# i2Nav-WHU/IC-GVINS

Measured on NVIDIA H100. Metric: frames/sec (KLT+BA) 1280x560 300-feat 10-KF window, higher is better.
Workload: dtype u8/int32 fixed point + f32 (KLT), f64 (BA)

## Files before the change

ic_gvins_b200/csrc/ba.cu:

```cuda
#include <cooperative_groups.h>
#include <math.h>
#include <string.h>

#include "ba_dev.cuh"
#include "geom_core.cuh"

namespace icg {
using namespace bam;
namespace cg = cooperative_groups;

constexpr int BA_CHOL_NB = 8;

__device__ __forceinline__ double *lin_Mp(const BaCaps &C, const BaDev &D, int b, int w) { return D.Mp[b] + (size_t) w * C.K * (C.K - 1) * 210; }
__device__ __forceinline__ double *lin_AW(const BaCaps &C, const BaDev &D, int b, int w) { return D.AW[b] + (size_t) w * C.LP * C.NCA; }
__device__ __forceinline__ double *lin_costf(const BaCaps &C, const BaDev &D, int b, int w) { return D.costf[b] + (size_t) w * C.F; }
__device__ __forceinline__ double *lin_hl(const BaCaps &C, const BaDev &D, int b, int w) { return D.hl[b] + (size_t) w * C.L; }
__device__ __forceinline__ double *lin_gl(const BaCaps &C, const BaDev &D, int b, int w) { return D.gl[b] + (size_t) w * C.L; }
__device__ __forceinline__ double *lin_Hc(const BaCaps &C, const BaDev &D, int b, int w) { return D.Hc[b] + (size_t) w * C.NS * C.NS; }
__device__ __forceinline__ double *lin_gc(const BaCaps &C, const BaDev &D, int b, int w) { return D.gc[b] + (size_t) w * C.NS; }

__device__ __forceinline__ int col_pose(int k) { return 6 * k; }
__device__ __forceinline__ int col_ext(int K) { return 6 * K; }
__device__ __forceinline__ int col_td(int K) { return 6 * K + 6; }
__device__ __forceinline__ int col_mix(int K, int k) { return 6 * K + 7 + 9 * k; }

__device__ __forceinline__ double block_sum(double v, double *s_red);
__device__ __forceinline__ double block_max(double v, double *s_red);
}
#include "ba_lm.cuh"
namespace icg {

__device__ __forceinline__ int jc_off(int a) { return a < 18 ? (a / 6) * 12 + (a % 6) : 36 + 2 * (a - 18); }
__device__ __forceinline__ int jc_row1(int a) { return a < 18 ? 6 : 1; }
__device__ __forceinline__ int tri20(int la, int lb) {
    return la * 20 - la * (la - 1) / 2 + (lb - la);
}
__device__ __forceinline__ void dmma884(double &c0, double &c1, double a, double b) {
    asm volatile("mma.sync.aligned.m8n8k4.row.col.f64.f64.f64.f64 {%0,%1}, {%2}, {%3}, {%0,%1};" : "+d"(c0), "+d"(c1) : "d"(a), "d"(b));
}
__global__ void __launch_bounds__(128, 4) ba_lin_vis(BaCaps C, BaDev D, int at_cand) {
    extern __shared__ double lv_sm[];
    __shared__ int s_ord[128], s_gbeg[BA_MAX_NODES], s_gend[BA_MAX_NODES], s_last, s_p0, s_np;
    double (*s_rec)[LV_LD] = (double (*)[LV_LD]) lv_sm;
    double (*s_frame)[NODE_FRAME_LD] = (double (*)[NODE_FRAME_LD]) (lv_sm + 128 * LV_LD);
    const int w = blockIdx.y;
    const LmState &st = D.st[w];
    if (st.done || !(at_cand ? st.step_valid : st.need_lin)) return;
    const int b = at_cand ? 1 - st.lin_buf : st.lin_buf;
    const double *pose = at_cand ? D.pose_c : D.pose, *xext = at_cand ? D.ext_c : D.ext, *rho = at_cand ? D.rho_c : D.rho;
    const int *vb = D.vb_lm0 + (size_t) w * C.NVB;
    if ((int) blockIdx.x >= vb[C.NVB - 1]) return;
    const WinDims dm = D.dims[w];
    const int tid = threadIdx.x;
    const int *off = D.lm_off + (size_t) w * (C.L + 1);
    const int pA = vb[blockIdx.x], pB = vb[blockIdx.x + 1];
    const int s0 = off[pA], nslot = off[pB] - s0;
    if (tid <= dm.K) node_frame(tid < dm.K ? pose + ((size_t) w * C.K + tid) * 7 : xext + (size_t) w * 8, s_frame[tid]);
    if (tid < BA_MAX_NODES) s_gbeg[tid] = s_gend[tid] = 0;
    if (tid == 0) s_np = 0;
    __syncthreads();
    if (tid < nslot) {
        const int q = s0 + tid;
        double r[2], Ji[12], Jj[12], Je[12], Jr[2], Jt[2], cost = 0;
        const int4 meta = ((const int4 *) D.f_meta_s)[(size_t) w * C.F + q];
        const int i = meta.y, j = meta.z, f = meta.w;
        if (D.f_active[(size_t) w * C.F + f] != 0) {
            const double *ext = xext + (size_t) w * 8;
            reproj_eval_frames(s_frame[i], s_frame[j], s_frame[dm.K], rho[(size_t) w * C.L + meta.x], ext[7],
                               D.f_const_s + ((size_t) w * C.F + q) * 14, dm.reproj_sinv, true, r, Ji, Jj, Je, Jr, Jt);
            if (dm.ext_const)
                for (int k = 0; k < 12; k++) Je[k] = 0;
            if (dm.td_const) Jt[0] = Jt[1] = 0;
            double sq = r[0] * r[0] + r[1] * r[1], sc = 1.0;
            if (dm.reproj_huber)
                huber(sq, cost, sc);
            else
                cost = 0.5 * sq;
            if (sc != 1.0) {
                for (int k = 0; k < 12; k++) Ji[k] *= sc, Jj[k] *= sc, Je[k] *= sc;
                Jr[0] *= sc, Jr[1] *= sc, Jt[0] *= sc, Jt[1] *= sc, r[0] *= sc, r[1] *= sc;
            }
        } else {
            for (int k = 0; k < 12; k++) Ji[k] = Jj[k] = Je[k] = 0;
            Jr[0] = Jr[1] = Jt[0] = Jt[1] = r[0] = r[1] = 0;
        }
        lin_costf(C, D, b, w)[f] = cost;
        double *sr = s_rec[tid];
#pragma unroll
        for (int k = 0; k < 12; k++) sr[k] = Ji[k], sr[12 + k] = Jj[k], sr[24 + k] = Je[k];
        sr[36] = Jt[0], sr[37] = Jt[1], sr[38] = r[0], sr[39] = r[1];
        sr[40] = Jr[0], sr[41] = Jr[1], sr[42] = (double) j, sr[43] = (double) i;
    }
    __syncthreads();
    const int lane = tid & 31, warp = tid >> 5;
    if (nslot > 0) {
        if (tid < nslot) {
            const int *ord = D.vis_ord + (size_t) w * C.F + s0;
            const int v = ord[tid], ob = (int) s_rec[v & 255][42];
            s_ord[tid] = v;
            if (tid == 0 || (int) s_rec[ord[tid - 1] & 255][42] != ob) s_gbeg[ob] = tid;
            if (tid == nslot - 1 || (int) s_rec[ord[tid + 1] & 255][42] != ob) s_gend[ob] = tid + 1;
        }
        __syncthreads();
        const int kk = lane & 3, g = lane >> 2;
        int o[3];
#pragma unroll
        for (int t = 0; t < 3; t++) {
            const int a = 8 * t + g;
            o[t] = a < 20 ? jc_off(a) + (kk & 1) * jc_row1(a) : -1;
        }
        for (int ob = warp; ob < dm.K; ob += 4) {
            const int beg = s_gbeg[ob], end = s_gend[ob];
            if (beg == end) continue;
            double c00[2] = {0, 0}, c01[2] = {0, 0}, c02[2] = {0, 0}, c11[2] = {0, 0}, c12[2] = {0, 0}, c22[2] = {0, 0};
            constexpr int UNR = 2;
            for (int base = beg; base < end; base += 2 * UNR) {
                double x[UNR][3];
#pragma unroll
                for (int u = 0; u < UNR; u++) {
                    const int q = base + 2 * u + (kk >> 1);
                    const bool ok = q < end;
                    const double *rec = s_rec[ok ? s_ord[q] & 255 : 0];
#pragma unroll
                    for (int t = 0; t < 3; t++) x[u][t] = (ok && o[t] >= 0) ? rec[o[t]] : 0.0;
                }
#pragma unroll
                for (int u = 0; u < UNR; u++) {
                    dmma884(c00[0], c00[1], x[u][0], x[u][0]);
                    dmma884(c01[0], c01[1], x[u][0], x[u][1]);
                    dmma884(c02[0], c02[1], x[u][0], x[u][2]);
                    dmma884(c11[0], c11[1], x[u][1], x[u][1]);
                    dmma884(c12[0], c12[1], x[u][1], x[u][2]);
                    dmma884(c22[0], c22[1], x[u][2], x[u][2]);
                }
            }
            double *pp = D.gpart + ((size_t) w * C.GQ + (s_ord[beg] >> 8)) * 210;
            auto put = [&](int ti, int tj, const double *c) {
#pragma unroll
                for (int e = 0; e < 2; e++) {
                    const int la = 8 * ti + g, lb = 8 * tj + 2 * kk + e;
                    if (la <= lb && lb < 20) pp[tri20(la, lb)] = c[e];
                }
            };
            put(0, 0, c00), put(0, 1, c01), put(0, 2, c02), put(1, 1, c11), put(1, 2, c12), put(2, 2, c22);
        }
        __threadfence();
    }
    const int *perm = D.lm_perm + (size_t) w * C.L;
    const int K = dm.K, NCV = 6 * K + 7, NCA = 4 * ((NCV + 1 + 3) / 4);
    const int grp = tid >> 3, sl = tid & 7;
    int o0[3], o1[3];
#pragma unroll
    for (int t = 0; t < 3; t++) {
        const int c = sl + 8 * t;
        o0[t] = c < 19 ? jc_off(c) : 38, o1[t] = c < 19 ? o0[t] + jc_row1(c) : 39;
    }
    for (int pl = pA + grp; pl < pB; pl += 16) {
        const int l = perm[pl], f0 = off[pl] - s0, nf = off[pl + 1] - off[pl];
        double *row = lin_AW(C, D, b, w) + (size_t) l * C.NCA;
        for (int c = sl; c < NCA; c += 8) row[c] = 0.0;
        __syncwarp(0xffu << (tid & 24));
        double acc[3] = {0, 0, 0};
        for (int q = 0; q < nf; q++) {
            const double *rec = s_rec[f0 + q];
            const double r0 = rec[40], r1 = rec[41];
            const int ob = (int) rec[42];
#pragma unroll
            for (int t = 0; t < 3; t++) {
                const int c = sl + 8 * t;
                if (c == 20) {
                    acc[t] += r0 * r0 + r1 * r1;
                } else if (c < 20) {
                    const double v = rec[o0[t]] * r0 + rec[o1[t]] * r1;
                    if (c >= 6 && c < 12)
                        row[col_pose(ob) + c - 6] = v;
                    else
                        acc[t] += v;
                }
            }
        }
        const int ref = nf > 0 ? (int) s_rec[f0][43] : 0;
#pragma unroll
        for (int t = 0; t < 3; t++) {
            const int c = sl + 8 * t;
            if (nf > 0) {
                if (c < 6) row[col_pose(ref) + c] = acc[t];
                else if (c >= 12 && c < 18) row[col_ext(K) + c - 12] = acc[t];
                else if (c == 18) row[col_td(K)] = acc[t];
            }
            if (c == 19) {
                row[NCV] = acc[t];
                lin_gl(C, D, b, w)[l] = acc[t];
            } else if (c == 20) {
                lin_hl(C, D, b, w)[l] = acc[t];
                if (st.first) D.scale_l[(size_t) w * C.L + l] = 1.0 / (1.0 + sqrt(acc[t]));
            }
        }
    }
    if (nslot == 0) return;
    const int rn = (int) s_rec[0][43];
    __syncthreads();
    if (tid == 0) s_last = atomicAdd(D.vis_cnt + (size_t) w * C.K + rn, 1) == D.ref_nrun[(size_t) w * C.K + rn] - 1;
    __syncthreads();
    if (!s_last) return;
    __threadfence();
    if (tid == 0) D.vis_cnt[(size_t) w * C.K + rn] = 0;
    const int PM = C.K * (C.K - 1), P = D.npairs[w];
    const int *pro = D.pair_ro + (size_t) w * PM, *poff = D.part_off + (size_t) w * (PM + 1);
    for (int p = tid; p < P; p += 128)
        if ((pro[p] >> 8) == rn) {
            atomicAdd(&s_np, 1);
            if (p == 0 || (pro[p - 1] >> 8) != rn) s_p0 = p;
        }
    __syncthreads();
    const double *part = D.gpart + (size_t) w * C.GQ * 210;
    double *Mp = lin_Mp(C, D, b, w);
    for (int p = s_p0 + warp; p < s_p0 + s_np; p += 4) {
        const int k0 = poff[p], k1 = poff[p + 1];
        double acc[7];
#pragma unroll
        for (int j = 0; j < 7; j++) acc[j] = lane + 32 * j < 210 ? __ldcg(part + (size_t) k0 * 210 + lane + 32 * j) : 0.0;
        for (int k = k0 + 1; k < k1; k++) {
            double v[7];
#pragma unroll
            for (int j = 0; j < 7; j++) v[j] = lane + 32 * j < 210 ? __ldcg(part + (size_t) k * 210 + lane + 32 * j) : 0.0;
#pragma unroll
            for (int j = 0; j < 7; j++) acc[j] += v[j];
        }
#pragma unroll
        for (int j = 0; j < 7; j++)
            if (lane + 32 * j < 210) Mp[(size_t) p * 210 + lane + 32 * j] = acc[j];
    }
}


__device__ __forceinline__ void gram2_slots(const BaCaps &C, const BaDev &D, int w, int K, short *s_slot) {
    const int PM = C.K * (C.K - 1), P = D.npairs[w];
    const int *pro = D.pair_ro + (size_t) w * PM;
    for (int e = threadIdx.x; e < K * K; e += blockDim.x) s_slot[e] = -1;
    __syncthreads();
    for (int p = threadIdx.x; p < P; p += blockDim.x) s_slot[(pro[p] >> 8) * K + (pro[p] & 255)] = (short) p;
    __syncthreads();
}
__device__ __forceinline__ double gram2_entry(const BaCaps &C, const BaDev &D, int buf, int w, int K, const short *s_slot, int A, int B) {
    const int P = D.npairs[w];
    const double *Mp = lin_Mp(C, D, buf, w);
    const int bA = A < 6 * K ? A / 6 : K, bB = B < 6 * K ? B / 6 : K;
    const int a = A - 6 * bA, b = B - 6 * bB;
    const int ga = 12 + a, gb = 12 + b;
    double sum = 0;
    if (bA == K) {
        const int idx = tri20(ga, gb);
        double s4[4] = {0, 0, 0, 0};
        int p = 0;
        for (; p + 16 <= P; p += 16) {
            double v[16];
#pragma unroll
            for (int u = 0; u < 16; u++) v[u] = Mp[(size_t) (p + u) * 210 + idx];
#pragma unroll
            for (int u = 0; u < 16; u++) s4[u & 3] += v[u];
        }
        for (; p < P; p++) s4[p & 3] += Mp[(size_t) p * 210 + idx];
        sum = (s4[0] + s4[1]) + (s4[2] + s4[3]);
    } else if (bB == K || bB == bA) {
        const int i1 = tri20(a, bB == K ? gb : b), i2 = tri20(6 + a, bB == K ? gb : 6 + b);
        for (int o0 = 0; o0 < K; o0 += 8) {
            double v1[8], v2[8];
#pragma unroll
            for (int u = 0; u < 8; u++) {
                const int o = o0 + u;
                const int p1 = o < K ? s_slot[bA * K + o] : -1, p2 = o < K ? s_slot[o * K + bA] : -1;
                v1[u] = p1 >= 0 ? Mp[(size_t) p1 * 210 + i1] : 0.0;
                v2[u] = p2 >= 0 ? Mp[(size_t) p2 * 210 + i2] : 0.0;
            }
#pragma unroll
            for (int u = 0; u < 8; u++) sum += v1[u], sum += v2[u];
        }
    } else {
        const int p1 = s_slot[bA * K + bB], p2 = s_slot[bB * K + bA];
        if (p1 >= 0) sum += Mp[(size_t) p1 * 210 + tri20(a, 6 + b)];
        if (p2 >= 0) sum += Mp[(size_t) p2 * 210 + tri20(b, 6 + a)];
    }
    return sum;
}

__device__ __forceinline__ double *x_inbox(const BaDev &D, int peer, int w, int from);
__device__ __forceinline__ int tri_idx(int A, int B, int ncv);

__device__ __forceinline__ void schur_store(const BaCaps &C, const BaDev &D, int buf, int w, int K, const short *s_slot, int A, int B, double cw) {
    const int NCV = 6 * K + 7;
    if (A == NCV) return;
    const size_t e = (size_t) w * C.NS * C.NS + (size_t) B * C.NS + A;
    const double hc = !D.S.split && B < NCV ? lin_Hc(C, D, buf, w)[(size_t) B * C.NS + A] : 0.0;
    const double cj = gram2_entry(C, D, buf, w, K, s_slot, A, B);
    if (D.S.split) {
        double *P = x_inbox(D, w % D.world, w, D.rank);
        const int TRI = NCV * (NCV + 1) / 2;
        if (B < NCV) {
            P[tri_idx(A, B, NCV)] = cj - cw;
            if (A == B) P[TRI + A] = cj;
        } else {
            P[TRI + NCV + A] = cj;
            P[TRI + 2 * NCV + A] = cw;
        }
    } else {
        double *V = D.visv + (size_t) w * 3 * C.NCV;
        if (B < NCV) {
            D.Hs[e] = hc + (cj - cw);
            if (A == B) V[A] = cj;
        } else {
            V[NCV + A] = cj, V[2 * NCV + A] = cw;
        }
    }
}

__device__ __forceinline__ void schur_scalars(const BaCaps &C, const BaDev &D, int w, const WinDims &dm, double *s_red) {
    const int tid = threadIdx.x;
    double c = 0, q = 0, gm = 0;
    const double *costf = lin_costf(C, D, 0, w), *gl = lin_gl(C, D, 0, w);
    for (int f = tid; f < dm.F; f += 256) c += costf[f];
    for (int l = tid; l < dm.L; l += 256) {
        const double r = D.rho[(size_t) w * C.L + l];
        q += r * r;
        gm = fmax(gm, fabs(gl[l]));
    }
    c = block_sum(c, s_red);
    q = block_sum(q, s_red);
    gm = block_max(gm, s_red);
    if (tid != 0) return;
    const int NCV = 6 * dm.K + 7, TRI = NCV * (NCV + 1) / 2;
    double *P = x_inbox(D, w % D.world, w, D.rank);
    P[TRI + 3 * NCV] = c, P[TRI + 3 * NCV + 1] = q, P[TRI + 3 * NCV + 2] = gm;
}

__global__ void __cluster_dims__(BA_SPLIT_W, 1, 1) __launch_bounds__(256) ba_schur_dmma(BaCaps C, BaDev D, int ld) {
    extern __shared__ double sA[];
    __shared__ short s_slot[32 * 32];
    __shared__ double s_red[40];
    cg::cluster_group cluster = cg::this_cluster();
    const int w = blockIdx.y, split = blockIdx.x;
    const LmState &st = D.st[w];
    if (st.done) return;
    const WinDims dm = D.dims[w];
    const int NCV = 6 * dm.K + 7, NCA = 4 * ((NCV + 1 + 3) / 4);
    const int T2 = (NCA + 15) / 16, nsuper = T2 * (T2 + 1) / 2;
    const int tid = threadIdx.x, lane = tid & 31, warp = tid >> 5, g = lane >> 2, kk = lane & 3;
    double *sphi = sA + (size_t) SCHUR_RCH * ld;
    const int b = st.lin_buf;
    const double *A = lin_AW(C, D, b, w), *hl = lin_hl(C, D, b, w);
    const double radius = st.radius;
    const int nsteps = (dm.L + 3) / 4;
    const int r_beg = 4 * (int) ((long long) nsteps * split / BA_SPLIT_W), r_end = min(dm.L, 4 * (int) ((long long) nsteps * (split + 1) / BA_SPLIT_W));
    const int npass = (nsuper + SCHUR_PASS - 1) / SCHUR_PASS;
    gram2_slots(C, D, w, dm.K, s_slot);
    for (int pass = 0; pass < npass; pass++) {
        if (pass > 0) cluster.barrier_wait();
        int si[2], sj[2];
        bool on[2];
#pragma unroll
        for (int h2 = 0; h2 < 2; h2++) {
            const int su = (2 * pass + h2) * 8 + warp;
            on[h2] = su < nsuper;
            int a = 0, e = on[h2] ? su : 0;
            while (e >= T2 - a) e -= T2 - a, a++;
            si[h2] = a, sj[h2] = a + e;
        }
        double acc[2][4][2];
#pragma unroll
        for (int h2 = 0; h2 < 2; h2++)
#pragma unroll
            for (int q = 0; q < 4; q++) acc[h2][q][0] = acc[h2][q][1] = 0;
        for (int r0 = r_beg; r0 < r_end; r0 += SCHUR_RCH) {
            const int nr = min(SCHUR_RCH, r_end - r0), nr4 = (nr + 3) & ~3;
            __syncthreads();
            for (int rb = warp; rb < nr4; rb += 8 * 4) {
                double v[4][3];
#pragma unroll
                for (int u = 0; u < 4; u++) {
                    const int rr = rb + 8 * u;
#pragma unroll
                    for (int cchunk = 0; cchunk < 3; cchunk++) {
                        const int c = lane + 32 * cchunk;
                        v[u][cchunk] = (rr < nr && c < NCA) ? A[(size_t) (r0 + rr) * C.NCA + c] : 0.0;
                    }
                }
#pragma unroll
                for (int u = 0; u < 4; u++) {
                    const int rr = rb + 8 * u;
#pragma unroll
                    for (int cchunk = 0; cchunk < 3; cchunk++) {
                        const int c = lane + 32 * cchunk;
                        if (rr < nr4 && c < ld) sA[(size_t) rr * ld + c] = v[u][cchunk];
                    }
                }
                for (int c = lane + 96; c < ld; c += 32)
                    for (int u = 0; u < 4; u++) {
                        const int rr = rb + 8 * u;
                        if (rr < nr4) sA[(size_t) rr * ld + c] = (rr < nr && c < NCA) ? A[(size_t) (r0 + rr) * C.NCA + c] : 0.0;
                    }
            }
            for (int rr = tid; rr < nr4; rr += 256) {
                double ph = 0;
                if (rr < nr) {
                    const int l = r0 + rr;
                    const double sl = D.scale_l[(size_t) w * C.L + l], hs = sl * sl * hl[l];
                    ph = sl * sl / (hs + lm_d2(hs, radius));
                }
                sphi[rr] = ph;
            }
            __syncthreads();
            for (int ks = 0; ks < nr4 / 4; ks++) {
                const double *row = sA + (size_t) (4 * ks + kk) * ld;
                const double ph = sphi[4 * ks + kk];
#pragma unroll
                for (int h2 = 0; h2 < 2; h2++) {
                    if (!on[h2]) continue;
                    const double xb0 = row[16 * sj[h2] + g], xb1 = row[16 * sj[h2] + 8 + g];
                    const double a0 = row[16 * si[h2] + g] * ph, a1 = row[16 * si[h2] + 8 + g] * ph;
                    dmma884(acc[h2][0][0], acc[h2][0][1], a0, xb0);
                    dmma884(acc[h2][1][0], acc[h2][1][1], a0, xb1);
                    dmma884(acc[h2][2][0], acc[h2][2][1], a1, xb0);
                    dmma884(acc[h2][3][0], acc[h2][3][1], a1, xb1);
                }
            }
        }
        __syncthreads();
#pragma unroll
        for (int h2 = 0; h2 < 2; h2++) {
            if (!on[h2]) continue;
#pragma unroll
            for (int q = 0; q < 4; q++)
#pragma unroll
                for (int e = 0; e < 2; e++) sA[(h2 * 8 + warp) * 256 + 64 * q + 32 * e + lane] = acc[h2][q][e];
        }
        cluster.sync();
        const int nslot = min(SCHUR_PASS, nsuper - SCHUR_PASS * pass);
        double cw[SCHUR_PASS / BA_SPLIT_W];
#pragma unroll
        for (int j = 0; j < SCHUR_PASS / BA_SPLIT_W; j++) {
            const int sl = split + BA_SPLIT_W * j;
            double p[BA_SPLIT_W];
#pragma unroll
            for (int k = 0; k < BA_SPLIT_W; k++) p[k] = sl < nslot ? cluster.map_shared_rank(sA, k)[sl * 256 + tid] : 0.0;
            cw[j] = 0;
#pragma unroll
            for (int k = 0; k < BA_SPLIT_W; k++) cw[j] += p[k];
        }
        cluster.barrier_arrive();
        const int q = tid >> 6, r_in = 8 * (q >> 1) + ((tid & 31) >> 2), c_in = 8 * (q & 1) + 2 * (tid & 3) + ((tid >> 5) & 1);
#pragma unroll
        for (int j = 0; j < SCHUR_PASS / BA_SPLIT_W; j++) {
            const int sl = split + BA_SPLIT_W * j;
            if (sl >= nslot) break;
            int a = 0, e = SCHUR_PASS * pass + sl;
            while (e >= T2 - a) e -= T2 - a, a++;
            const int r = 16 * a + r_in, cc = 16 * (a + e) + c_in;
            if (r <= cc && cc <= NCV) schur_store(C, D, b, w, dm.K, s_slot, r, cc, cw[j]);
        }
    }
    if (split == 0 && D.S.split) schur_scalars(C, D, w, dm, s_red);
    cluster.barrier_wait();
}

constexpr double IMU_GB_STD = 7200 / 3600.0 * 3.14159265358979323846 / 180.0;
constexpr double IMU_AB_STD = 2.0e4 * 1.0e-5;

__device__ void imu_factor_warp(const double *blob, const double *U, const double *pose0, const double *mix0, const double *pose1,
                                const double *mix1, bool want_j, double *rw, double *Jw, int lane) {
    __shared__ ImuMid s_mid[16];
    double *raw_r = rw + 15;
    const int wslot = (threadIdx.x >> 5) & 15;
    if (want_j)
        for (int e = lane; e < 450; e += 32) Jw[e] = 0;
    __syncwarp();
    if (lane == 0) {
        ImuMid M;
        imu_residual_raw(blob, pose0, mix0, pose1, mix1, raw_r, M);
        if (want_j) imu_jacobian_raw(blob, M, Jw);
        s_mid[wslot] = M;
    }
    __syncwarp();
    if (want_j && lane < 30) {
        for (int i = 0; i < 15; i++) {
            double s = 0;
            for (int k = i; k < 15; k++) s += U[i * 15 + k] * Jw[k * 30 + lane];
            Jw[i * 30 + lane] = s;
        }
    }
    if (lane < 15) {
        double s = 0;
        for (int k = lane; k < 15; k++) s += U[lane * 15 + k] * raw_r[k];
        rw[lane] = s;
    }
    __syncwarp();
}

__device__ void marg_dx(const BaCaps &C, const BaDev &D, int w, const WinDims &dm, const double *pose, const double *mix, const double *ext, double *dx,
                        int *colmap, int tid, int nthreads) {
    const int *type = D.marg_type + (size_t) w * BA_MARG_MAXB, *node = D.marg_node + (size_t) w * BA_MARG_MAXB;
    const double *x0 = D.marg_x0 + (size_t) w * BA_MARG_MAXB * 9;
    if (tid == 0) {
        int col = 0, xo = 0;
        for (int b = 0; b < dm.marg_nb; b++) {
            int t = type[b], nd = node[b];
            if (t == 0 || t == 2) {
                const double *x = t == 0 ? pose + nd * 7 : ext;
                const double *xl = x0 + xo;
                Q dq = qmul(qinv(pose_q(xl)), pose_q(x));
                V3 a = 2.0 * qv(dq);
                if (dq.w < 0) a = -a;
                for (int k = 0; k < 3; k++) dx[col + k] = x[k] - xl[k];
                dx[col + 3] = a.x, dx[col + 4] = a.y, dx[col + 5] = a.z;
                int base = t == 0 ? col_pose(nd) : col_ext(dm.K);
                for (int k = 0; k < 6; k++) colmap[col + k] = (t == 2 && dm.ext_const) ? -1 : base + k;
                col += 6, xo += 7;
            } else if (t == 1) {
                for (int k = 0; k < 9; k++) dx[col + k] = mix[nd * 9 + k] - x0[xo + k], colmap[col + k] = col_mix(dm.K, nd) + k;
                col += 9, xo += 9;
            } else {
                dx[col] = ext[7] - x0[xo];
                colmap[col] = dm.td_const ? -1 : col_td(dm.K);
                col += 1, xo += 1;
            }
        }
    }
}

__device__ __forceinline__ void red_add(double *p, double v) { asm volatile("red.global.add.f64 [%0], %1;" ::"l"(p), "d"(v) : "memory"); }

__device__ double cam_factors(const BaCaps &C, const BaDev &D, int w, const WinDims &dm, const double *pose, const double *mix, const double *ext,
                              bool lin, int b, double *smem) {
    const int tid = threadIdx.x, lane = tid & 31, warp = tid >> 5, nwarps = blockDim.x >> 5;
    const int K = dm.K, N = 15 * K + 7;
    double *Hc = lin_Hc(C, D, b, w), *gc = lin_gc(C, D, b, w);
    double *s_imu = smem;
    double *s_gnss = s_imu + (size_t) C.K * 480;
    double *s_misc = s_gnss + (size_t) C.G * 24;
    double *s_pp = s_misc, *s_mp = s_misc + 48, *s_dx = s_mp + 16, *s_y = s_dx + C.R, *s_cost = s_y + C.R;
    int *s_colmap = (int *) (s_cost + 8);
    __shared__ double s_total;
#ifdef ICG_BA_PHASE_CLOCKS
    unsigned long long cclk = D.clk ? clock64() : 0ull;
#define CAM_CLK(k)                                                 \
    if (D.clk && lin && w == 0 && tid == 0) {                      \
        const unsigned long long t_ = clock64();                   \
        atomicAdd(&D.clk[16 + (k)], t_ - cclk), atomicAdd(&D.clk[24 + (k)], 1ull); \
        cclk = t_;                                                 \
    }
#else
#define CAM_CLK(k)
#endif
    for (int k = warp; k < dm.n_imu; k += nwarps)
        imu_factor_warp(D.imu_blob + ((size_t) w * C.K + k) * ICG_IMU_BLOB_DOUBLES, D.imu_U + ((size_t) w * C.K + k) * 225, pose + k * 7, mix + k * 9,
                        pose + (k + 1) * 7, mix + (k + 1) * 9, lin, s_imu + (size_t) k * 480, s_imu + (size_t) k * 480 + 30, lane);
    if (tid < dm.n_gnss) {
        const int nd = D.gnss_node[(size_t) w * C.G + tid];
        double *o = s_gnss + tid * 24;
        gnss_eval(pose + nd * 7, D.gnss_blh + ((size_t) w * C.G + tid) * 3, D.gnss_std + ((size_t) w * C.G + tid) * 3, D.lever + (size_t) w * 3, lin, o, o + 3);
        double sq = o[0] * o[0] + o[1] * o[1] + o[2] * o[2], cost, sc = 1.0;
        if (dm.gnss_huber)
            huber(sq, cost, sc);
        else
            cost = 0.5 * sq;
        if (sc != 1.0) {
            for (int e = 0; e < 3; e++) o[e] *= sc;
            if (lin)
                for (int e = 0; e < 18; e++) o[3 + e] *= sc;
        }
        o[21] = cost;
    }
    if (tid == 64 && dm.has_pose_prior) pose_prior_eval(pose, D.pose_prior + (size_t) w * 7, D.pose_prior_sinfo + (size_t) w * 6, lin, s_pp, s_pp + 6);
    if (tid == 96 && dm.has_mix_prior)
        for (int k = 0; k < 9; k++) s_mp[k] = (mix[k] - D.mix_prior[(size_t) w * 9 + k]) / D.mix_prior_std[(size_t) w * 9 + k];
    if (dm.marg_r > 0) marg_dx(C, D, w, dm, pose, mix, ext, s_dx, s_colmap, tid, blockDim.x);
    __syncthreads();
    CAM_CLK(0)
    const double *H0 = D.marg_H0 + (size_t) w * C.R * C.R, *b0 = D.marg_b0 + (size_t) w * C.R;
    if (dm.marg_r > 0) {
        for (int i = tid; i < dm.marg_r; i += blockDim.x) {
            double s = 0;
            for (int k = 0; k < dm.marg_r; k++) s += H0[(size_t) i * dm.marg_r + k] * s_dx[k];
            s_y[i] = s;
        }
    }
    __syncthreads();
    if (tid == 0) {
        double c = 0;
        for (int k = 0; k < dm.n_imu; k++) {
            const double *r = s_imu + (size_t) k * 480;
            double sq = 0;
            for (int e = 0; e < 15; e++) sq += r[e] * r[e];
            c += 0.5 * sq;
        }
        for (int g = 0; g < dm.n_gnss; g++) c += s_gnss[g * 24 + 21];
        if (dm.has_imu_error) {
            const double *m = mix + dm.n_imu * 9;
            double sq = 0;
            for (int e = 0; e < 3; e++) sq += (m[3 + e] / IMU_GB_STD) * (m[3 + e] / IMU_GB_STD) + (m[6 + e] / IMU_AB_STD) * (m[6 + e] / IMU_AB_STD);
            c += 0.5 * sq;
        }
        if (dm.has_pose_prior) {
            double sq = 0;
            for (int e = 0; e < 6; e++) sq += s_pp[e] * s_pp[e];
            c += 0.5 * sq;
        }
        if (dm.has_mix_prior) {
            double sq = 0;
            for (int e = 0; e < 9; e++) sq += s_mp[e] * s_mp[e];
            c += 0.5 * sq;
        }
        if (dm.marg_r > 0) {
            double q = D.marg_c0[w];
            for (int i = 0; i < dm.marg_r; i++) q += (2.0 * b0[i] + s_y[i]) * s_dx[i];
            c += 0.5 * q;
        }
        s_total = c;
    }
    if (!lin) {
        __syncthreads();
        return s_total;
    }
    CAM_CLK(1)
    for (int e = tid; e < N * C.NS; e += blockDim.x) Hc[e] = 0;
    for (int e = tid; e < N; e += blockDim.x) gc[e] = 0;
    __syncthreads();
    CAM_CLK(2)
    if (dm.marg_r > 0) {
        const int r = dm.marg_r;
        for (int e = tid; e < r * r; e += blockDim.x) {
            int i = e / r, j = e - i * r;
            int ci = s_colmap[i], cj = s_colmap[j];
            if (ci >= 0 && cj >= 0) Hc[(size_t) ci * C.NS + cj] = H0[e];
        }
        for (int i = tid; i < r; i += blockDim.x)
            if (s_colmap[i] >= 0) gc[s_colmap[i]] = b0[i] + s_y[i];
    }
    __syncthreads();
    CAM_CLK(3)
    for (int parity = 0; parity < 2; parity++) {
        const int nf = (dm.n_imu - parity + 1) / 2;
        for (int e = tid; e < nf * 930; e += blockDim.x) {
            const int k = parity + 2 * (e / 930), q = e % 930;
            const double *rw = s_imu + (size_t) k * 480, *Jw = rw + 30;
            auto gcol = [&](int c) { return c < 6 ? col_pose(k) + c : c < 15 ? col_mix(K, k) + c - 6 : c < 21 ? col_pose(k + 1) + c - 15 : col_mix(K, k + 1) + c - 21; };
            if (q < 900) {
                int a = q / 30, b = q - a * 30;
                double s = 0;
                for (int m = 0; m < 15; m++) s += Jw[m * 30 + a] * Jw[m * 30 + b];
                red_add(&Hc[(size_t) gcol(a) * C.NS + gcol(b)], s);
            } else {
                int a = q - 900;
                double s = 0;
                for (int m = 0; m < 15; m++) s += Jw[m * 30 + a] * rw[m];
                red_add(&gc[gcol(a)], s);
            }
        }
        __syncthreads();
    }
    CAM_CLK(4)
    for (int e = tid; e < K * 42; e += blockDim.x) {
        const int k = e / 42, q = e % 42;
        double s = 0;
        if (q < 36) {
            const int a = q / 6, b = q % 6;
            for (int g = 0; g < dm.n_gnss; g++)
                if (D.gnss_node[(size_t) w * C.G + g] == k) {
                    const double *J = s_gnss + g * 24 + 3;
                    s += J[a] * J[b] + J[6 + a] * J[6 + b] + J[12 + a] * J[12 + b];
                }
            if (k == 0 && dm.has_pose_prior)
                for (int m = 0; m < 6; m++) s += s_pp[6 + m * 6 + a] * s_pp[6 + m * 6 + b];
            red_add(&Hc[(size_t) (col_pose(k) + a) * C.NS + col_pose(k) + b], s);
        } else {
            const int a = q - 36;
            for (int g = 0; g < dm.n_gnss; g++)
                if (D.gnss_node[(size_t) w * C.G + g] == k) {
                    const double *o = s_gnss + g * 24;
                    s += o[3 + a] * o[0] + o[9 + a] * o[1] + o[15 + a] * o[2];
                }
            if (k == 0 && dm.has_pose_prior)
                for (int m = 0; m < 6; m++) s += s_pp[6 + m * 6 + a] * s_pp[m];
            red_add(&gc[col_pose(k) + a], s);
        }
    }
    if (tid < 9) {
        if (dm.has_imu_error && tid >= 3) {
            const int k = dm.n_imu;
            const double sd = tid < 6 ? IMU_GB_STD : IMU_AB_STD;
            Hc[(size_t) (col_mix(K, k) + tid) * C.NS + col_mix(K, k) + tid] += 1.0 / (sd * sd);
            gc[col_mix(K, k) + tid] += mix[k * 9 + tid] / (sd * sd);
        }
    }
    __syncthreads();
    if (tid < 9 && dm.has_mix_prior) {
        const double sd = D.mix_prior_std[(size_t) w * 9 + tid];
        Hc[(size_t) (col_mix(K, 0) + tid) * C.NS + col_mix(K, 0) + tid] += 1.0 / (sd * sd);
        gc[col_mix(K, 0) + tid] += s_mp[tid] / sd;
    }
    __syncthreads();
    CAM_CLK(5)
#undef CAM_CLK
    return s_total;
}

__global__ void __launch_bounds__(CAM_THREADS) ba_lin_cam(BaCaps C, BaDev D, int at_cand) {
    extern __shared__ double smem[];
    const int w = blockIdx.x;
    LmState &st = D.st[w];
    if (st.done || !(at_cand ? st.step_valid : st.need_lin)) return;
    if (D.S.split && (w % D.world) != D.rank) return;
    const WinDims dm = D.dims[w];
    const int b = at_cand ? 1 - st.lin_buf : st.lin_buf;
    const double *pose = at_cand ? D.pose_c : D.pose, *mix = at_cand ? D.mix_c : D.mix, *ext = at_cand ? D.ext_c : D.ext;
    double c = cam_factors(C, D, w, dm, pose + (size_t) w * C.K * 7, mix + (size_t) w * C.K * 9, ext + (size_t) w * 8, true, b, smem);
    if (threadIdx.x == 0) st.cost_cam[b] = c;
}


__device__ __forceinline__ double block_sum(double v, double *s_red) {
    const int tid = threadIdx.x, lane = tid & 31, warp = tid >> 5;
    for (int o = 16; o > 0; o >>= 1) v += __shfl_down_sync(0xffffffffu, v, o);
    __syncthreads();
    if (lane == 0) s_red[warp] = v;
    __syncthreads();
    double t = 0;
    if (tid == 0) {
        for (int k = 0; k < (int) (blockDim.x >> 5); k++) t += s_red[k];
        s_red[32] = t;
    }
    __syncthreads();
    return s_red[32];
}
__device__ __forceinline__ double block_max(double v, double *s_red) {
    const int tid = threadIdx.x, lane = tid & 31, warp = tid >> 5;
    for (int o = 16; o > 0; o >>= 1) v = fmax(v, __shfl_down_sync(0xffffffffu, v, o));
    __syncthreads();
    if (lane == 0) s_red[warp] = v;
    __syncthreads();
    if (tid == 0) {
        double t = 0;
        for (int k = 0; k < (int) (blockDim.x >> 5); k++) t = fmax(t, s_red[k]);
        s_red[32] = t;
    }
    __syncthreads();
    return s_red[32];
}

__global__ void __launch_bounds__(SOLVE_THREADS, 2) ba_solve(BaCaps C, BaDev D) {
    extern __shared__ double sm[];
    const int w = blockIdx.x, tid = threadIdx.x;
    LmState &st = D.st[w];
    if (st.done) return;
#ifdef ICG_BA_PHASE_CLOCKS
    unsigned long long clk_prev = D.clk ? clock64() : 0ull;
#define SOLVE_CLK(k)                                              \
    if (D.clk && w == 0 && tid == 0) {                            \
        const unsigned long long t_ = clock64();                  \
        atomicAdd(&D.clk[k], t_ - clk_prev), atomicAdd(&D.clk[8 + (k)], 1ull); \
        clk_prev = t_;                                            \
    }
#define SOLVE_CLK_NOW() (D.clk ? clock64() : 0ull)
#define SOLVE_CLK_ADD(k, t0)                                      \
    if (D.clk && w == 0 && tid == 0) atomicAdd(&D.clk[k], clock64() - (t0)), atomicAdd(&D.clk[8 + (k)], 1ull);
#else
#define SOLVE_CLK(k)
#define SOLVE_CLK_NOW() 0ull
#define SOLVE_CLK_ADD(k, t0)
#endif
    const WinDims dm = D.dims[w];
    const int K = dm.K, L = dm.L, NCV = 6 * K + 7, N = 15 * K + 7;
    const int f_first = st.first, f_fresh = st.fresh_lin, f_last = st.last_success, f_iter = st.iter;
    const double f_gmax_old = st.gmax;
    (void) f_gmax_old;
    double *s_red = sm;
    double *s_scale = s_red + 40;
    double *s_g = s_scale + C.NS;
    double *s_rhs = s_g + C.NS;
    double *s_d2 = s_rhs + C.NS;
    double *s_diag = s_d2 + C.NS;
    double *S = s_diag + C.NS;
    const int b = st.lin_buf;
    const double *Hc = lin_Hc(C, D, b, w), *gcam = lin_gc(C, D, b, w), *Hs = D.Hs + (size_t) w * C.NS * C.NS;
    const double *V = D.visv + (size_t) (3 * C.NCV) * w;
    if (tid == 0 && st.need_lin) st.need_lin = 0;
    double *scale_c = D.scale_c + (size_t) w * C.NS;
    const double *hl = lin_hl(C, D, b, w), *gl = lin_gl(C, D, b, w), *scale_l = D.scale_l + (size_t) w * C.L;

    for (int a = tid; a < N; a += SOLVE_THREADS) {
        double g = gcam[a];
        if (a < NCV) g += V[NCV + a];
        s_g[a] = g;
        if (f_first) {
            double h = Hc[(size_t) a * C.NS + a] + (a < NCV ? V[a] : 0.0);
            scale_c[a] = 1.0 / (1.0 + sqrt(h));
        }
    }
    __syncthreads();
    for (int a = tid; a < N; a += SOLVE_THREADS) s_scale[a] = scale_c[a];
    double gmax_now = st.gmax;
    if (f_fresh) {
        double cs = 0, gq = 0;
        const double *costf = lin_costf(C, D, b, w);
        for (int f = tid; f < dm.F; f += SOLVE_THREADS) cs += costf[f];
        for (int l = tid; l < L; l += SOLVE_THREADS) gq = fmax(gq, fabs(gl[l]));
        const double c = block_sum(cs, s_red), gml = block_max(gq, s_red);
        double gm = 0;
        for (int a = tid; a < N; a += SOLVE_THREADS) gm = fmax(gm, fabs(s_g[a]));
        gm = fmax(block_max(gm, s_red), gml);
        gmax_now = gm;
        if (tid == 0) {
            st.x_cost = c + st.cost_cam[b];
            st.gmax = gm;
            if (f_first) st.initial_cost = st.x_cost;
            st.fresh_lin = 0;
        }
        __syncthreads();
    }
    if (f_first) {
        __syncthreads();
        if (tid == 0) st.first = 0;
    }
    {
        const int term = lm_term(f_iter, st.max_iter, f_last, gmax_now, st.radius);
        if (term) {
            __syncthreads();
            if (tid == 0) st.done = term, st.step_valid = 0;
            return;
        }
    }
    __syncthreads();
    if (tid == 0) st.iter++;
    const double radius = st.radius;
    SOLVE_CLK(0)

    constexpr bool async_fill = true;
    if (async_fill) {
        for (int i = tid >> 5; i < N; i += SOLVE_THREADS / 32) {
            const double *src = (i < NCV ? Hs : Hc) + (size_t) i * C.NS;
            const unsigned dst = (unsigned) __cvta_generic_to_shared(S + i * (i + 1) / 2);
            for (int j = tid & 31; j <= i; j += 32)
                asm volatile("cp.async.ca.shared.global [%0], [%1], 8;" ::"r"(dst + 8u * j), "l"(src + j) : "memory");
        }
        asm volatile("cp.async.commit_group;" ::: "memory");
    }
    for (int a = tid; a < N; a += SOLVE_THREADS) {
        double h = Hc[(size_t) a * C.NS + a] + (a < NCV ? V[a] : 0.0);
        double hs = s_scale[a] * s_scale[a] * h;
        s_d2[a] = lm_d2(hs, radius);
        double gw = a < NCV ? V[2 * NCV + a] : 0.0;
        s_rhs[a] = -s_scale[a] * (s_g[a] - gw);
    }
    if (async_fill) asm volatile("cp.async.wait_all;" ::: "memory");
    __syncthreads();
    if (async_fill) {
        for (int i = tid >> 5; i < N; i += SOLVE_THREADS / 32) {
            double *row = S + i * (i + 1) / 2;
            const double si = s_scale[i];
            for (int j = tid & 31; j <= i; j += 32) {
                double v = si * s_scale[j] * row[j];
                if (i == j) v += s_d2[i];
                row[j] = v;
            }
        }
    } else {
        for (int i = tid >> 5; i < N; i += SOLVE_THREADS / 32) {
            constexpr int MAXQ = 16;
            double hv[MAXQ];
            const int nq = i / 32 + 1;
#pragma unroll
            for (int q = 0; q < MAXQ; q++) {
                const int j = (tid & 31) + 32 * q;
                hv[q] = 0;
                if (q < nq && j <= i) hv[q] = (i < NCV ? Hs : Hc)[(size_t) i * C.NS + j];
            }
#pragma unroll
            for (int q = 0; q < MAXQ; q++) {
                const int j = (tid & 31) + 32 * q;
                if (q < nq && j <= i) {
                    double v = s_scale[i] * s_scale[j] * hv[q];
                    if (i == j) v += s_d2[i];
                    S[i * (i + 1) / 2 + j] = v;
                }
            }
        }
    }
    for (int a = tid; a < N; a += SOLVE_THREADS) S[N * (N + 1) / 2 + a] = s_rhs[a];
    __syncthreads();
    SOLVE_CLK(1)
    __shared__ int s_fail;
    if (tid == 0) s_fail = 0;
    __syncthreads();
    const int NR = N + 1;
    for (int J0 = 0; J0 < N; J0 += BA_CHOL_NB) {
        const int nb = min(BA_CHOL_NB, N - J0);
        const int lane = tid & 31, warp = tid >> 5, g = lane >> 2, kk = lane & 3;
        const int ntile = (NR - J0 + 7) / 8;
        const unsigned long long pc0 = SOLVE_CLK_NOW();
        (void) pc0;
        const int cb = J0 + g;
        const double *rb = S + (cb < NR ? cb * (cb + 1) / 2 : 0);
        const bool okb = cb < NR;
        if (warp == 0) {
            if (J0 > 0) {
                const double *ra = rb;
                double acc[8] = {0, 0, 0, 0, 0, 0, 0, 0};
                int k0 = 0;
                for (; k0 + 16 <= J0; k0 += 16) {
                    const double x0 = okb ? ra[k0 + kk] : 0.0, x1 = okb ? ra[k0 + 4 + kk] : 0.0, x2 = okb ? ra[k0 + 8 + kk] : 0.0, x3 = okb ? ra[k0 + 12 + kk] : 0.0;
                    dmma884(acc[0], acc[1], x0, x0);
                    dmma884(acc[2], acc[3], x1, x1);
                    dmma884(acc[4], acc[5], x2, x2);
                    dmma884(acc[6], acc[7], x3, x3);
                }
                for (; k0 + 8 <= J0; k0 += 8) {
                    const double x0 = okb ? ra[k0 + kk] : 0.0, x1 = okb ? ra[k0 + 4 + kk] : 0.0;
                    dmma884(acc[0], acc[1], x0, x0);
                    dmma884(acc[2], acc[3], x1, x1);
                }
                const double c0 = (acc[0] + acc[2]) + (acc[4] + acc[6]), c1 = (acc[1] + acc[3]) + (acc[5] + acc[7]);
                const int i = J0 + g;
                if (i < NR) {
                    const int ca = J0 + 2 * kk;
                    if (ca < J0 + nb && ca <= i) S[i * (i + 1) / 2 + ca] -= c0;
                    if (ca + 1 < J0 + nb && ca + 1 <= i) S[i * (i + 1) / 2 + ca + 1] -= c1;
                }
                __syncwarp();
            }
            double Ld[BA_CHOL_NB][BA_CHOL_NB], dinv[BA_CHOL_NB];
            bool bad = false;
#pragma unroll
            for (int a = 0; a < BA_CHOL_NB; a++)
#pragma unroll
                for (int b = 0; b < BA_CHOL_NB; b++) Ld[a][b] = (a < nb && b <= a) ? S[(J0 + a) * (J0 + a + 1) / 2 + J0 + b] : (a == b ? 1.0 : 0.0);
#pragma unroll
            for (int j = 0; j < BA_CHOL_NB; j++) {
                double d = Ld[j][j];
#pragma unroll
                for (int k = 0; k < j; k++) d -= Ld[j][k] * Ld[j][k];
                if (!(d > 0.0) || !isfinite(d)) bad = true;
                const double di = rsqrt(d);
                dinv[j] = di;
                Ld[j][j] = d * di;
#pragma unroll
                for (int a = j + 1; a < BA_CHOL_NB; a++) {
                    double sum = Ld[a][j];
#pragma unroll
                    for (int k = 0; k < j; k++) sum -= Ld[a][k] * Ld[j][k];
                    Ld[a][j] = sum * di;
                }
            }
            __syncwarp();
            if (bad && lane == 0) s_fail = 1;
#pragma unroll
            for (int a2 = 0; a2 < BA_CHOL_NB; a2++) {
                double *ri = S + (J0 + a2) * (J0 + a2 + 1) / 2 + J0;
#pragma unroll
                for (int b = 0; b <= a2; b++)
                    if (lane == ((a2 * 8 + b) & 31) && a2 < nb) ri[b] = Ld[a2][b];
                if (lane == 8 + a2 && a2 < nb) s_diag[J0 + a2] = dinv[a2];
            }
            SOLVE_CLK_ADD(6, pc0)
        } else if (J0 > 0 && warp != 4) {
            constexpr int TPW = 4, NWARP = 6;
            const int wslot = warp < 4 ? warp - 1 : warp - 2;
            for (int t0 = 1 + wslot; t0 < ntile; t0 += TPW * NWARP) {
                const double *ra[TPW];
                bool oka[TPW];
                double acc[TPW][4];
#pragma unroll
                for (int u = 0; u < TPW; u++) {
                    const int ia = J0 + 8 * (t0 + u * NWARP) + g;
                    oka[u] = (t0 + u * NWARP) < ntile && ia < NR;
                    ra[u] = S + (oka[u] ? ia * (ia + 1) / 2 : 0);
                    acc[u][0] = acc[u][1] = acc[u][2] = acc[u][3] = 0;
                }
                for (int k0 = 0; k0 + 8 <= J0; k0 += 8) {
                    const double b0 = okb ? rb[k0 + kk] : 0.0, b1 = okb ? rb[k0 + 4 + kk] : 0.0;
                    double a0[TPW], a1[TPW];
#pragma unroll
                    for (int u = 0; u < TPW; u++) a0[u] = oka[u] ? ra[u][k0 + kk] : 0.0, a1[u] = oka[u] ? ra[u][k0 + 4 + kk] : 0.0;
#pragma unroll
                    for (int u = 0; u < TPW; u++) {
                        dmma884(acc[u][0], acc[u][1], a0[u], b0);
                        dmma884(acc[u][2], acc[u][3], a1[u], b1);
                    }
                }
#pragma unroll
                for (int u = 0; u < TPW; u++) {
                    const double c0 = acc[u][0] + acc[u][2], c1 = acc[u][1] + acc[u][3];
                    const int i = J0 + 8 * (t0 + u * NWARP) + g;
                    if (oka[u]) {
                        const int ca = J0 + 2 * kk;
                        if (ca < J0 + nb && ca <= i) S[i * (i + 1) / 2 + ca] -= c0;
                        if (ca + 1 < J0 + nb && ca + 1 <= i) S[i * (i + 1) / 2 + ca + 1] -= c1;
                    }
                }
            }
        }
        __syncthreads();
        const unsigned long long pc1 = SOLVE_CLK_NOW();
        (void) pc1;
        if (s_fail) break;
        for (int i = J0 + nb + tid; i < NR; i += SOLVE_THREADS) {
            double *ri = S + i * (i + 1) / 2 + J0;
            double x[BA_CHOL_NB];
#pragma unroll
            for (int c = 0; c < BA_CHOL_NB; c++) x[c] = c < nb ? ri[c] : 0.0;
#pragma unroll
            for (int c = 0; c < BA_CHOL_NB; c++) {
                if (c < nb) {
                    const double *lc = S + (J0 + c) * (J0 + c + 1) / 2 + J0;
                    double sum = x[c];
#pragma unroll
                    for (int k = 0; k < c; k++) sum -= x[k] * lc[k];
                    x[c] = sum * s_diag[J0 + c];
                }
            }
#pragma unroll
            for (int c = 0; c < BA_CHOL_NB; c++)
                if (c < nb) ri[c] = x[c];
        }
        __syncthreads();
        SOLVE_CLK_ADD(7, pc1)
    }
    __syncthreads();
    bool valid = !s_fail;
    SOLVE_CLK(2)
    if (valid) {
        double *y = S + N * (N + 1) / 2;
        const int lane = tid & 31;
        for (int J0 = ((N - 1) / BA_CHOL_NB) * BA_CHOL_NB; J0 >= 0; J0 -= BA_CHOL_NB) {
            const int nb = min(BA_CHOL_NB, N - J0);
            if (tid < 32) {
                double x[BA_CHOL_NB];
#pragma unroll
                for (int c = BA_CHOL_NB - 1; c >= 0; c--) {
                    x[c] = 0.0;
                    if (c < nb) {
                        double sum = y[J0 + c];
#pragma unroll
                        for (int k = BA_CHOL_NB - 1; k > c; k--)
                            if (k < nb) sum -= S[(J0 + k) * (J0 + k + 1) / 2 + J0 + c] * x[k];
                        x[c] = sum * s_diag[J0 + c];
                    }
                }
#pragma unroll
                for (int c = 0; c < BA_CHOL_NB; c++)
                    if (c == lane && c < nb) s_rhs[J0 + c] = x[c];
            }
            __syncthreads();
            for (int i = tid; i < J0; i += SOLVE_THREADS) {
                double acc = y[i];
#pragma unroll
                for (int c = BA_CHOL_NB - 1; c >= 0; c--)
                    if (c < nb) acc -= S[(J0 + c) * (J0 + c + 1) / 2 + i] * s_rhs[J0 + c];
                y[i] = acc;
            }
            __syncthreads();
        }
    }
    __syncthreads();
    SOLVE_CLK(3)
    double *step_l = D.step_l + (size_t) w * C.L;
    const double *AW = lin_AW(C, D, b, w);
    double part = 0;
    bool finite = true;
    double *R2 = D.red2 + (size_t) w * 4;
    if (!valid) {
        if (tid == 0) {
            st.chol_ok = 0, st.step_valid = 0;
            R2[0] = 0, R2[1] = 0, R2[2] = 1;
        }
        return;
    }
    for (int a = tid; a < N; a += SOLVE_THREADS) {
        double sp = s_rhs[a];
        finite = finite && isfinite(sp);
        part += -0.5 * sp * (s_scale[a] * s_g[a]) + 0.5 * s_d2[a] * sp * sp;
    }
    double *s_sx = s_diag;
    __syncthreads();
    for (int a = tid; a < NCV; a += SOLVE_THREADS) s_sx[a] = s_scale[a] * s_rhs[a];
    __syncthreads();
    {
        const int lane = tid & 31, warp = tid >> 5;
        constexpr int LB = 8;
        const int lu = ((lane >> 4) & 1) * 4 + ((lane >> 3) & 1) * 2 + ((lane >> 2) & 1);
        for (int l0 = LB * warp; l0 < L; l0 += LB * (SOLVE_THREADS / 32)) {
            const int l = l0 + lu;
            const bool lok = l < L;
            const double sl = lok ? scale_l[l] : 0.0, hh = lok ? hl[l] : 0.0, gg = lok ? gl[l] : 0.0;
            double d[LB];
#pragma unroll
            for (int u = 0; u < LB; u++) d[u] = 0;
            for (int c = lane; c < NCV; c += 32) {
                const double sx = s_sx[c];
#pragma unroll
                for (int u = 0; u < LB; u++) d[u] += (l0 + u < L ? AW[(size_t) (l0 + u) * C.NCA + c] : 0.0) * sx;
            }
            const double hs = sl * sl * hh, d2 = lm_d2(hs, radius), den = hs + d2, sg = sl * gg;
            double e4[4], e2[2];
            {
                const bool hi = lane & 16;
#pragma unroll
                for (int u = 0; u < 4; u++) {
                    const double keep = hi ? d[u + 4] : d[u], send = hi ? d[u] : d[u + 4];
                    e4[u] = keep + __shfl_xor_sync(0xffffffffu, send, 16);
                }
            }
            {
                const bool hi = lane & 8;
#pragma unroll
                for (int u = 0; u < 2; u++) {
                    const double keep = hi ? e4[u + 2] : e4[u], send = hi ? e4[u] : e4[u + 2];
                    e2[u] = keep + __shfl_xor_sync(0xffffffffu, send, 8);
                }
            }
            double mine;
            {
                const bool hi = lane & 4;
                const double keep = hi ? e2[1] : e2[0], send = hi ? e2[0] : e2[1];
                mine = keep + __shfl_xor_sync(0xffffffffu, send, 4);
            }
            mine += __shfl_xor_sync(0xffffffffu, mine, 2);
            mine += __shfl_xor_sync(0xffffffffu, mine, 1);
            if ((lane & 3) == 0 && lok) {
                double sp = (-sg - sl * mine) / den;
                finite = finite && isfinite(sp);
                step_l[l] = sp;
                part += -0.5 * sp * sg + 0.5 * d2 * sp * sp;
            }
        }
    }
    __syncthreads();
    SOLVE_CLK(4)
    const double mcc = block_sum(part, s_red);
    const double nfin = block_sum(finite ? 0.0 : 1.0, s_red);
    const double *pose = D.pose + (size_t) w * C.K * 7, *mix = D.mix + (size_t) w * C.K * 9, *ext = D.ext + (size_t) w * 8, *rho = D.rho + (size_t) w * C.L;
    double *pose_c = D.pose_c + (size_t) w * C.K * 7, *mix_c = D.mix_c + (size_t) w * C.K * 9, *ext_c = D.ext_c + (size_t) w * 8, *rho_c = D.rho_c + (size_t) w * C.L;
    double sn = 0;
    for (int k = tid; k <= K; k += SOLVE_THREADS) {
        const bool is_ext = (k == K);
        const double *x = is_ext ? ext : pose + k * 7;
        double *xc = is_ext ? ext_c : pose_c + k * 7;
        if (is_ext && dm.ext_const) {
            for (int e = 0; e < 7; e++) xc[e] = x[e];
        } else {
            const int c0 = is_ext ? col_ext(K) : col_pose(k);
            double d[6];
            for (int e = 0; e < 6; e++) d[e] = s_rhs[c0 + e] * s_scale[c0 + e];
            pose_plus(x, d, xc);
            for (int e = 0; e < 7; e++) sn += (x[e] - xc[e]) * (x[e] - xc[e]);
        }
    }
    for (int e = tid; e < K * 9; e += SOLVE_THREADS) {
        int k = e / 9, q = e - 9 * k, c = col_mix(K, k) + q;
        double v = mix[e] + s_rhs[c] * s_scale[c];
        mix_c[e] = v;
        sn += (mix[e] - v) * (mix[e] - v);
    }
    if (tid == 0) {
        if (dm.td_const) {
            ext_c[7] = ext[7];
        } else {
            double v = ext[7] + s_rhs[col_td(K)] * s_scale[col_td(K)];
            ext_c[7] = v;
            sn += (ext[7] - v) * (ext[7] - v);
        }
    }
    for (int l = tid; l < L; l += SOLVE_THREADS) {
        double v = rho[l] + step_l[l] * scale_l[l];
        rho_c[l] = v;
        sn += (rho[l] - v) * (rho[l] - v);
    }
    sn = block_sum(sn, s_red);
    if (tid == 0) {
// ... 258 lines not shown
```

ic_gvins_b200/csrc/ba_dev.cuh:

```cuda
#pragma once
#include "ba_math.cuh"
#include "ba_slide.cuh"
#include "common.cuh"

namespace icg {

constexpr int BA_SPLIT_W = 4;
constexpr int BA_MARG_MAXB = 72;
constexpr int BA_MAX_NODES = 32;

struct BaCaps {
    int NW, K, L, F, G, R;
    int NCV, N, NS, NCA, RJ, LP, NVB;
    int GQ;
};

struct WinDims {
    int K, L, F, n_imu, n_gnss, marg_r, marg_nb;
    int ext_const, td_const, reproj_huber, gnss_huber, has_imu_error, has_pose_prior, has_mix_prior;
    double reproj_sinv;
};

struct LmState {
    double radius, decrease_factor, x_cost, x_norm, cand_cost, model_cost_change, step_norm, gmax, initial_cost;
    double cost_cam[2];
    int iter, n_success, n_invalid, done, need_lin, last_success, first, step_valid, fresh_lin, max_iter, chol_ok;
    int lin_buf;
};

struct ShardDev {
    int split;
    int PK, BS, RV;
    double *peer[8];
    size_t off_inbox, off_bcast, off_scal, off_flagA, off_flagB, off_flagC;
    size_t off_flagX, off_post, off_exp;
    double *redv;
    int *err;
    double *slm;
    int *slm_cnt;
};

struct BaDev {
    ShardDev S;
    WinDims *dims;
    LmState *st;
    double *pose, *mix, *ext, *rho;
    double *pose_c, *mix_c, *ext_c, *rho_c;
    double *pose_0, *mix_0, *ext_0, *rho_0;
    uint8_t *f_active_0;
    double *gnss_std_0;
    uint8_t *f_active;
    int *lm_off;
    int *lm_perm;
    int *vb_lm0;
    int *ref_nrun;
    int *f_meta_s;
    double *f_const_s;
    int *vis_ord;
    int *part_off, *pair_ro, *npairs;
    double *gpart;
    int *vis_cnt;
    double *Mp[2];
    double *AW[2];
    double *costf[2];
    double *hl[2], *gl[2];
    double *Hc[2], *gc[2];
    double *scale_l, *scale_c;
    double *Hs;
    double *visv;
    double *imu_blob, *imu_U;
    int *gnss_node;
    double *gnss_blh, *gnss_std, *lever;
    double *pose_prior, *pose_prior_sinfo, *mix_prior, *mix_prior_std;
    int *marg_type, *marg_node;
    double *marg_x0, *marg_H0, *marg_b0, *marg_c0;
    double *cost_part;
    double *red2;
    int rank, world;
    double *step_c, *step_l;
    double *Sglobal;
    unsigned long long *clk;
};

constexpr int LV_LD = 45;
constexpr size_t LV_SMEM = sizeof(double) * (128 * LV_LD + (BA_MAX_NODES + 1) * bam::NODE_FRAME_LD);
constexpr int SCHUR_RCH = 80;
constexpr int SCHUR_PASS = 16;
constexpr int CAM_THREADS = 320;
constexpr int SOLVE_THREADS = 256;

constexpr int SPLIT_CLUSTER = 4;
constexpr int SPLIT_HDR = 16;
constexpr int SPLIT_SCAL = 8;
constexpr int SPLIT_BS_ROWS = 32;
constexpr int STEP_SLICES = 4;
constexpr int MEXP_ROW = 16;
enum { XF_SUM = 0, XF_EXPORT = 1, XF_DONE = 2 };

__host__ __device__ inline size_t split_S_stride(const BaCaps &C) { return (size_t) (C.N + 1) * (C.N + 2) / 2 + (size_t) C.NS; }

constexpr int DSM_CL = 4;
static_assert(SOLVE_THREADS == 256 && DSM_CL == SPLIT_CLUSTER, "ba_solve_cam_dsm: warp r assembles row r of a tile row; one launch geometry for both forms");
__host__ __device__ constexpr int dsm_ntiles(int NR) { return (NR + 7) / 8; }
__host__ inline size_t dsm_smem_doubles(const BaCaps &C) {
    const int nt = dsm_ntiles(C.N + 1);
    int mx = 0;
    for (int cr = 0; cr < DSM_CL; cr++) {
        int s = 0;
        for (int T = cr; T < nt; T += DSM_CL) s += T;
        mx = s > mx ? s : mx;
    }
    return 40 + 8 * (size_t) nt * 8 + 64 + 8 + 8 * DSM_CL + 8 + 8 + (size_t) nt * 64 * 3 + (size_t) mx * 64;
}

constexpr int MARG_THREADS = 512;
constexpr int MARG_MAP_HDR = 8;

struct MargDev {
    int *map;
    int map_stride;
    double *H0, *b0;
    double *G1, *V1;
    double *G2, *V2;
    double *lam1, *lam2;
    double *Z;
    double *Hp, *bp;
    double *J0, *e0;
    int *flags;
    int n0cap, mcap, rcap;
};

constexpr int MARG_PAIR_MAXN = 160;
constexpr int MARG_CTA_MAXN = 118;
constexpr int MARG_CTA_THREADS = 512;
constexpr int MARG_CLUSTER_MAXN = 320;
constexpr int MARG_CLUSTER_CTAS = 8;
constexpr int MARG_CLUSTER_THREADS = 640;
constexpr int MARG_CLUSTER_SLOT = 3 * (MARG_CLUSTER_MAXN / 2);
__host__ __device__ constexpr int marg_cluster_rows(int n) { return (n + MARG_CLUSTER_CTAS - 1) / MARG_CLUSTER_CTAS; }
__host__ __device__ constexpr size_t marg_cluster_smem(int n) {
    return sizeof(double) * (2 * (size_t) marg_cluster_rows(n) * n + 2 * (size_t) MARG_CLUSTER_SLOT);
}

__global__ void ba_lin_vis(BaCaps C, BaDev D, int at_cand);
__global__ void ba_schur_dmma(BaCaps C, BaDev D, int ld);
__global__ void ba_lin_cam(BaCaps C, BaDev D, int at_cand);
__global__ void ba_solve(BaCaps C, BaDev D);
__global__ void ba_cost_cam(BaCaps C, BaDev D, int nblk_vis);
__global__ void ba_cost(BaCaps C, BaDev D, int nblk_vis);
__global__ void ba_accept(BaCaps C, BaDev D);
__global__ void ba_reset_state(BaDev D, LmState *save, int n, int max_iter);
__global__ void ba_chi2_cull(BaCaps C, BaDev D, int *counters);
__global__ void ba_set_gnss_huber(BaDev D, int n, int v);
__global__ void ba_residual_costs_kernel(BaCaps C, BaDev D, double *reproj_cost, double *gnss_cost);
__global__ void ba_reproj_eval_kernel(const double *in, double *out, int frames);
__global__ void ba_imu_eval_kernel(const double *blob, const double *U, const double *x, double *out);
__global__ void ba_small_factor_eval_kernel(int kind, const double *in, double *out);
__global__ void ba_marg_factor_eval_kernel(const double *in, double *out);
__global__ void ba_lm_ref_fill(const WinDims *dims, const SlideWin *win, const int *map, const double *old, const double *fc, const int *lm_off,
                               const int *lm_perm, double *out, int Lc, int Fc);

__global__ void ba_signal(BaDev D, unsigned long long epoch);
__global__ void ba_reduce(BaCaps C, BaDev D, unsigned long long epoch);
__global__ void ba_solve_cam(BaCaps C, BaDev D, unsigned long long epoch);
__global__ void ba_solve_cam_dsm(BaCaps C, BaDev D, unsigned long long epoch);
__global__ void ba_step_lm(BaCaps C, BaDev D, unsigned long long epoch);
__global__ void ba_exchange(BaCaps C, BaDev D, int n, int nblk_vis, unsigned long long epoch);
__global__ void ba_accept_split(BaCaps C, BaDev D, unsigned long long epoch);
__global__ void ba_xflag(BaDev D, int kind, unsigned long long epoch);
__global__ void ba_xsum(BaCaps C, BaDev D, int *v, int stride, int n, int nv, int op, int par, unsigned long long epoch);
__global__ void ba_marg_export(BaCaps C, BaDev D, const int *sel, const int *sel_off, const uint8_t *fmask, unsigned long long prev);
__global__ void ba_marg_heads(BaCaps C, BaDev D, int n_own, long long *heads, unsigned long long epoch);
__global__ void ba_marg_gather(BaCaps C, BaDev D, const long long *heads, const int *dst_row, double *dst);
__global__ void ba_marg_fill(BaCaps Cm, BaDev Dm, BaCaps C, BaDev D, const double *rows, const int *row0, const int *fidx);

__global__ void marg_prepare(BaDev D, MargDev M, int n, int restore);
__global__ void marg_assemble(BaCaps C, BaDev D, MargDev M);
__global__ void marg_jacobi(MargDev M, int which);
__global__ void marg_jacobi_pair(MargDev M, int which);
__global__ void marg_jacobi_cta(MargDev M, int which);
__global__ void marg_jacobi_cluster(MargDev M, int which);
__global__ void marg_schur(MargDev M);
__global__ void marg_finish(MargDev M);

}
```

ic_gvins_b200/csrc/ba_handle.cu:

```cuda
#include <unistd.h>

#include <string>
#include <thread>

#include "ba_handle.cuh"
#include "preint.cuh"

using namespace icg;

int dmalloc(icg_ba *h, double **p, size_t n) {
    if (cudaMalloc(p, sizeof(double) * n) != cudaSuccess) {
        set_error("icg_ba_create: cudaMalloc of %zu doubles failed", n);
        return ICG_ENOMEM;
    }
    cudaMemsetAsync(*p, 0, sizeof(double) * n, h->stream);
    h->dev_only.push_back(*p);
    return ICG_OK;
}

static int cam_threads(const icg_ba *h) { return h->D.world >= 4 ? CAM_THREADS : 160; }

static const char *PROF_NAMES[16] = {"(gap/other)", "lin_vis", "lin_lm", "lin at candidate", "","schur_dmma (+ epilogue)", "join lin_cam + lin_done",
                                     "signal", "solve", "cost (+cost_cam)", "exchange", "accept", "reduce", "join gram chain", "step_lm", ""};
static void prof_mark(icg_ba *h, int tag) {
    if (!h->prof) return;
    if (h->prof_used == h->prof_ev.size()) {
        cudaEvent_t e;
        cudaEventCreate(&e);
        h->prof_ev.push_back(e);
        h->prof_tag.push_back(0);
    }
    h->prof_tag[h->prof_used] = tag;
    cudaEventRecord(h->prof_ev[h->prof_used++], h->stream);
}
static void prof_collect(icg_ba *h) {
    if (!h->prof) return;
    if (h->prof_used && h->prof_skip > 0) {
        h->prof_skip--;
        h->prof_used = 0;
        return;
    }
    for (size_t i = 1; i < h->prof_used; i++) {
        float ms = 0;
        if (cudaEventElapsedTime(&ms, h->prof_ev[i - 1], h->prof_ev[i]) == cudaSuccess) {
            h->prof_ms[h->prof_tag[i]] += ms;
            h->prof_cnt[h->prof_tag[i]]++;
        }
    }
    h->prof_used = 0;
}
static void prof_print(icg_ba *h) {
    if (!h->prof) return;
    double tot = 0;
    for (int t = 0; t < 16; t++) tot += h->prof_ms[t];
    fprintf(stderr, "[icg_ba profile] handle %p, %d windows: stage totals over all recorded LM sequences (ms, mean us, share)\n", (void *) h, h->cur_windows);
    for (int t = 0; t < 16; t++)
        if (h->prof_cnt[t])
            fprintf(stderr, "  %-28s %9.3f ms  %8.1f us  %5.1f %%\n", PROF_NAMES[t], h->prof_ms[t], 1e3 * h->prof_ms[t] / h->prof_cnt[t], 100.0 * h->prof_ms[t] / tot);
    if (h->D.clk) {
        unsigned long long ck[48];
        if (cudaMemcpy(ck, h->D.clk, sizeof(ck), cudaMemcpyDeviceToHost) == cudaSuccess) {
            static const char *cn[6] = {"factor evaluation", "prior product + cost", "zero H_c", "prior blocks", "IMU J^T J", "GNSS / prior diagonals"};
            fprintf(stderr, "[icg_ba profile] ba_lin_cam phases of window 0 (SM cycles per call, mean):\n");
            for (int k = 0; k < 6; k++)
                if (ck[24 + k]) fprintf(stderr, "  %-28s %9.0f cycles\n", cn[k], (double) ck[16 + k] / (double) ck[24 + k]);
            if (h->D.S.split) {
                static const char *sn_l2[6] = {"per panel: stage B operand", "per panel: warp 0 tile + factor", "per panel: tiles + barrier 1", "per panel: row solve + barrier 2", "whole factorisation", ""};
                static const char *sn_dsm[6] = {"assembly", "per panel: warp 0 tile + factor", "per panel: until block barrier", "per panel: row solve + cl. barrier", "whole factorisation", "backward substitution"};
                const char **sn = h->solve_cam_dsm ? sn_dsm : sn_l2;
                fprintf(stderr, "[icg_ba profile] %s phases of window 0 (SM cycles, mean):\n", h->solve_cam_dsm ? "ba_solve_cam_dsm" : "ba_solve_cam");
                for (int k = 0; k < 6; k++)
                    if (ck[8 + k]) fprintf(stderr, "  %-34s %9.0f cycles\n", sn[k], (double) ck[k] / (double) ck[8 + k]);
                static const char *sn2[5] = {"(unused)", "(unused)", "per panel: warp 0 diagonal-tile update", "per panel: warp 0 loads + 8x8 factorisation", "per panel: warp 0 write-back"};
                for (int k = 0; k < 5 && h->solve_cam_dsm; k++)
                    if (ck[40 + k]) fprintf(stderr, "  %-50s %9.0f cycles\n", sn2[k], (double) ck[32 + k] / (double) ck[40 + k]);
            }
            static const char *nm[8] = {"gradient / cost / tests", "assembly", "Cholesky", "camera back-substitution", "landmark back-substitution", "candidate + reductions",
                                        "  per panel: warp 0 tile+factor", "  per panel: row solve phase"};
            if (!h->D.S.split) fprintf(stderr, "[icg_ba profile] ba_solve phases of window 0 (SM cycles per call, mean):\n");
            for (int k = 0; k < 8 && !h->D.S.split; k++)
                if (ck[8 + k]) fprintf(stderr, "  %-28s %9.0f cycles\n", nm[k], (double) ck[k] / (double) ck[8 + k]);
        }
    }
}

void retire(icg_ba *h, void *d, void *hp) {
    if (h->D.world > 1) {
        if (d) h->retired_d.push_back(d);
        if (hp) h->retired_h.push_back(hp);
        return;
    }
    if (d) cudaFree(d);
    if (hp) cudaFreeHost(hp);
}

static void split_release(icg_ba *h) {
    if (h->stream) cudaStreamSynchronize(h->stream);
    for (void *p : h->retired_d) cudaFree(p);
    for (void *p : h->retired_h) cudaFreeHost(p);
    for (icg_ba *m : h->retired_mx) icg_ba_destroy(m);
    h->retired_d.clear(), h->retired_h.clear(), h->retired_mx.clear();
    for (int r = 0; r < 8; r++)
        if (h->ipc_opened[r]) cudaIpcCloseMemHandle(h->ipc_opened[r]), h->ipc_opened[r] = nullptr;
    if (h->xbuf) cudaFree(h->xbuf), h->xbuf = nullptr;
    if (h->D.S.redv) cudaFree(h->D.S.redv), h->D.S.redv = nullptr;
    if (h->D.S.err) cudaFree(h->D.S.err), h->D.S.err = nullptr;
    if (h->D.S.slm) cudaFree(h->D.S.slm), h->D.S.slm = nullptr;
    if (h->D.S.slm_cnt) cudaFree(h->D.S.slm_cnt), h->D.S.slm_cnt = nullptr;
    if (h->D.Sglobal) cudaFree(h->D.Sglobal), h->D.Sglobal = nullptr;
    h->D.S.split = 0;
}

static int preload_group_kernels() {
    const void *k[] = {(const void *) ba_accept, (const void *) ba_accept_split, (const void *) ba_chi2_cull, (const void *) ba_cost, (const void *) ba_cost_cam,
                       (const void *) ba_exchange, (const void *) ba_lin_cam, (const void *) ba_lin_vis, (const void *) ba_marg_export, (const void *) ba_marg_fill,
                       (const void *) ba_marg_gather, (const void *) ba_marg_heads, (const void *) ba_reduce, (const void *) ba_reset_state,
                       (const void *) ba_schur_dmma, (const void *) ba_set_gnss_huber, (const void *) ba_signal, (const void *) ba_solve, (const void *) ba_solve_cam,
                       (const void *) ba_solve_cam_dsm, (const void *) ba_step_lm, (const void *) ba_xflag, (const void *) ba_xsum, (const void *) marg_assemble,
                       (const void *) marg_finish, (const void *) marg_jacobi, (const void *) marg_jacobi_cluster, (const void *) marg_jacobi_cta,
                       (const void *) marg_jacobi_pair, (const void *) marg_prepare, (const void *) marg_schur};
    cudaFuncAttributes a;
    for (const void *f : k) ICG_CUDA(cudaFuncGetAttributes(&a, f));
    ICG_CUDA(preload_update_cull());
    ICG_CUDA(preload_slide());
    ICG_CUDA(preload_preint_resident());
    return ICG_OK;
}

static int split_setup(icg_ba *h, int rank, int world) {
    if (world < 1 || world > 8 || rank < 0 || rank >= world) {
        set_error("split pipeline: rank %d / world %d out of range (<= 8 GPUs of one box)", rank, world);
        return ICG_EINVAL;
    }
    ICG_CUDA(cudaSetDevice(h->device));
    ICG_CUDA(cudaStreamSynchronize(h->stream));
    split_release(h);
    const BaCaps &C = h->C;
    ShardDev &S = h->D.S;
    const size_t NW = C.NW, G = world;
    const size_t TRI = (size_t) C.NCV * (C.NCV + 1) / 2;
    S.PK = (int) ((TRI + 3 * (size_t) C.NCV + 4 + 3) & ~(size_t) 3);
    S.BS = (SPLIT_HDR + C.NS + 3) & ~3;
    S.RV = (3 * C.NCV + 4 + 3) & ~3;
    const size_t NWo = (NW + G - 1) / G;
    size_t off = 0;
    S.off_inbox = off, off += NWo * G * S.PK;
    S.off_bcast = off, off += NW * S.BS;
    S.off_scal = off, off += NW * G * SPLIT_SCAL;
    S.off_flagA = off, off += 8;
    S.off_flagB = off, off += (NW + 3) & ~(size_t) 3;
    S.off_flagC = off, off += (NW * G + 3) & ~(size_t) 3;
    S.off_flagX = off, off += 3 * 8;
    S.off_post = off, off += 2 * NW * G * SPLIT_SCAL;
    S.off_exp = off;
    if (world > 1) off += 2 * NW + NW * (size_t) C.F * MEXP_ROW;
    h->xbuf_doubles = off;
    h->xs_calls = 0, h->exp_epoch = 0;
    if (world > 1) {
        const int rc = preload_group_kernels();
        if (rc != ICG_OK) return rc;
        if (!h->xs_v.d && h->xs_v.alloc(16) != ICG_OK) {
            set_error("split pipeline: allocation of the exchange word failed");
            return ICG_ENOMEM;
        }
    }
    if (cudaMalloc(&h->xbuf, sizeof(double) * off) != cudaSuccess || cudaMalloc(&S.redv, sizeof(double) * NW * S.RV) != cudaSuccess ||
        cudaMalloc(&S.err, sizeof(int) * 4) != cudaSuccess || cudaMalloc(&S.slm, sizeof(double) * NW * STEP_SLICES * 8) != cudaSuccess ||
        cudaMalloc(&S.slm_cnt, sizeof(int) * NW) != cudaSuccess ||
        cudaMalloc(&h->D.Sglobal, sizeof(double) * NWo * split_S_stride(C)) != cudaSuccess) {
        set_error("split pipeline: allocation of the exchange buffers failed (%zu doubles)", off);
        return ICG_ENOMEM;
    }
    ICG_CUDA(cudaMemset(h->xbuf, 0, sizeof(double) * off));
    ICG_CUDA(cudaMemset(S.redv, 0, sizeof(double) * NW * S.RV));
    ICG_CUDA(cudaMemset(S.err, 0, sizeof(int) * 4));
    ICG_CUDA(cudaMemset(S.slm, 0, sizeof(double) * NW * STEP_SLICES * 8));
    ICG_CUDA(cudaMemset(S.slm_cnt, 0, sizeof(int) * NW));
    for (int r = 0; r < 8; r++) S.peer[r] = nullptr;
    S.peer[rank] = h->xbuf;
    S.split = 1;
    h->D.rank = rank, h->D.world = world;
    h->x_world = world;
    h->epoch = 0;
    {
        const size_t ldbp = ((size_t) (C.N + 15) / 16) * 16 + 8;
        const size_t bs = (size_t) SPLIT_BS_ROWS * (C.NS + 1), base = 8 * ldbp + 64;
        h->smem_solve_cam = sizeof(double) * (40 + 4 * (size_t) C.NS + std::max(bs, base));
    }
    h->smem_step_lm = sizeof(double) * (40 + (size_t) C.NS);
    h->smem_solve_cam_dsm = sizeof(double) * dsm_smem_doubles(C);
    h->solve_cam_dsm = h->smem_solve_cam_dsm <= 227 * 1024 && C.N <= 32 * 11;
    if (h->solve_cam_dsm) ICG_CUDA(raise_dynamic_smem((const void *) ba_solve_cam_dsm, h->smem_solve_cam_dsm));
    ICG_CUDA(raise_dynamic_smem((const void *) ba_solve_cam, (size_t) (h->smem_solve_cam)));
    ICG_CUDA(cudaFuncSetAttribute(ba_solve_cam, cudaFuncAttributeNonPortableClusterSizeAllowed, 0));
    ICG_CUDA(raise_dynamic_smem((const void *) ba_step_lm, (size_t) (h->smem_step_lm)));
    return ICG_OK;
}

static int ba_create_body(icg_ba *h, int max_windows, int max_K, int max_L, int max_F, int max_gnss, int max_marg_r, void *stream) {
    if (stream) {
        h->stream = (cudaStream_t) stream;
    } else {
        ICG_CUDA(cudaStreamCreateWithFlags(&h->stream, cudaStreamNonBlocking));
        h->own_stream = true;
    }
    {
        int prio_lo = 0, prio_hi = 0;
        ICG_CUDA(cudaDeviceGetStreamPriorityRange(&prio_lo, &prio_hi));
        ICG_CUDA(cudaStreamCreateWithPriority(&h->stream_cam, cudaStreamNonBlocking, prio_hi));
    }
    ICG_CUDA(cudaEventCreateWithFlags(&h->ev_fork, cudaEventDisableTiming));
    ICG_CUDA(cudaEventCreateWithFlags(&h->ev_join, cudaEventDisableTiming));
    h->prof = getenv("ICG_BA_PROFILE") != nullptr;
    if (h->prof) {
        double *ck = nullptr;
        if (dmalloc(h, &ck, 48) != ICG_OK) return ICG_ENOMEM;
        h->D.clk = (unsigned long long *) ck;
    }
    if (getenv("ICG_BA_PROFILE_SKIP")) h->prof_skip = atoi(getenv("ICG_BA_PROFILE_SKIP"));
    BaCaps &C = h->C;
    max_L = std::max(1, max_L), max_F = std::max(1, max_F);
    C.NW = max_windows, C.K = max_K, C.L = max_L, C.F = max_F, C.G = std::max(1, max_gnss), C.R = std::max(1, max_marg_r);
    C.NCV = 6 * max_K + 7, C.N = 15 * max_K + 7, C.NS = (C.N + 3) & ~3, C.NCA = 4 * ((C.NCV + 1 + 3) / 4);
    C.RJ = (2 * max_F + 31) & ~31, C.LP = (max_L + 31) & ~31;
    C.NVB = (max_F + 127 - max_K) / (128 - max_K) + max_L / 128 + 4 + max_K;
    C.GQ = std::max(1, std::min(max_F, (C.NVB - 2) * (max_K - 1)));
    h->nblk_vis = (max_F + 255) / 256;
    const size_t NW = max_windows;
#define HD(field, count)                                                       \
    if (h->field.alloc(count) != ICG_OK) {                                     \
        set_error("icg_ba_create: allocation of " #field " failed");           \
        return ICG_ENOMEM;                                                     \
    }
    HD(dims, NW) HD(st, NW) HD(pose, NW * C.K * 7) HD(mix, NW * C.K * 9) HD(ext, NW * 8) HD(rho, NW * C.L)
    HD(imu_blob, NW * C.K * ICG_IMU_BLOB_DOUBLES) HD(imu_U, NW * C.K * 225) HD(gnss_blh, NW * C.G * 3) HD(gnss_std, NW * C.G * 3) HD(lever, NW * 3)
    HD(pose_prior, NW * 7) HD(pose_prior_sinfo, NW * 6) HD(mix_prior, NW * 9) HD(mix_prior_std, NW * 9) HD(marg_x0, NW * BA_MARG_MAXB * 9)
    HD(marg_H0, NW * C.R * C.R) HD(marg_b0, NW * C.R) HD(marg_c0, NW)
    HD(lm_off, NW * (C.L + 1)) HD(lm_perm, NW * C.L) HD(lm_fidx, NW * C.F) HD(gnss_node, NW * C.G) HD(marg_type, NW * BA_MARG_MAXB) HD(marg_node, NW * BA_MARG_MAXB) HD(f_active, NW * C.F)
    HD(scratch, 1024) HD(st_save, NW) HD(cull_counters, 2 * NW) HD(f_meta_s, NW * C.F * 4) HD(vb_lm0, NW * C.NVB) HD(ref_nrun, NW * C.K) HD(f_const_s, NW * C.F * 14)
    HD(part_off, NW * ((size_t) C.K * (C.K - 1) + 1)) HD(pair_ro, NW * (size_t) C.K * (C.K - 1)) HD(vis_ord, NW * C.F) HD(npairs, NW)
#undef HD
    ICG_CUDA(cudaMemsetAsync(h->st.d, 0, sizeof(LmState) * NW, h->stream));
    BaDev &D = h->D;
    D.rank = 0, D.world = 1;
    D.dims = h->dims.d, D.st = h->st.d, D.pose = h->pose.d, D.mix = h->mix.d, D.ext = h->ext.d, D.rho = h->rho.d;
    D.f_active = h->f_active.d;
    D.part_off = h->part_off.d, D.pair_ro = h->pair_ro.d, D.vis_ord = h->vis_ord.d, D.npairs = h->npairs.d;
    D.f_meta_s = h->f_meta_s.d, D.vb_lm0 = h->vb_lm0.d, D.ref_nrun = h->ref_nrun.d, D.f_const_s = h->f_const_s.d;
    D.lm_off = h->lm_off.d, D.lm_perm = h->lm_perm.d, D.imu_blob = h->imu_blob.d, D.imu_U = h->imu_U.d;
    D.gnss_node = h->gnss_node.d, D.gnss_blh = h->gnss_blh.d, D.gnss_std = h->gnss_std.d, D.lever = h->lever.d;
    D.pose_prior = h->pose_prior.d, D.pose_prior_sinfo = h->pose_prior_sinfo.d, D.mix_prior = h->mix_prior.d, D.mix_prior_std = h->mix_prior_std.d;
    D.marg_type = h->marg_type.d, D.marg_node = h->marg_node.d, D.marg_x0 = h->marg_x0.d, D.marg_H0 = h->marg_H0.d, D.marg_b0 = h->marg_b0.d, D.marg_c0 = h->marg_c0.d;
    int rc = ICG_OK;
#define DM(field, count) \
    if (rc == ICG_OK) rc = dmalloc(h, &D.field, count);
    DM(pose_c, NW * C.K * 7) DM(mix_c, NW * C.K * 9) DM(ext_c, NW * 8) DM(rho_c, NW * C.L)
    DM(pose_0, NW * C.K * 7) DM(mix_0, NW * C.K * 9) DM(ext_0, NW * 8) DM(rho_0, NW * C.L)
    DM(AW[0], NW * C.NCA * C.LP) DM(Mp[0], NW * (size_t) C.K * (C.K - 1) * 210) DM(visv, NW * 3 * C.NCV)
    DM(gpart, NW * (size_t) C.GQ * 210) DM(costf[0], NW * C.F) DM(hl[0], NW * C.L) DM(gl[0], NW * C.L) DM(scale_l, NW * C.L) DM(scale_c, NW * C.NS)
    DM(Hc[0], NW * C.NS * C.NS) DM(gc[0], NW * C.NS) DM(Hs, NW * C.NS * C.NS) DM(cost_part, NW * (h->nblk_vis + 1)) DM(red2, NW * 4) DM(step_c, NW * C.NS) DM(step_l, NW * C.L)
#undef DM
    if (rc == ICG_OK) rc = dmalloc(h, &D.gnss_std_0, NW * C.G * 3);
    if (rc == ICG_OK) {
        double *cnt = nullptr;
        rc = dmalloc(h, &cnt, (NW * C.K + 1) / 2);
        D.vis_cnt = (int *) cnt;
    }
    if (rc == ICG_OK) {
        double *fa0 = nullptr;
        rc = dmalloc(h, &fa0, (NW * C.F + 7) / 8 + 1);
        D.f_active_0 = (uint8_t *) fa0;
    }
    if (rc == ICG_OK) rc = dmalloc(h, &h->lm_ref, NW * C.L * 7);
    if (rc == ICG_OK) rc = dmalloc(h, &h->lm_ref_alt, NW * C.L * 7);
    if (rc != ICG_OK) return rc;
    h->smem_cam = sizeof(double) * ((size_t) C.K * 480 + (size_t) C.G * 24 + 48 + 16 + 2 * (size_t) C.R + 8) + sizeof(int) * (size_t) C.R + 64;
    size_t vec = sizeof(double) * (40 + 5 * (size_t) C.NS);
    size_t packed = sizeof(double) * ((size_t) (C.N + 1) * (C.N + 2) / 2);
    h->use_global_S = (vec + packed > 220 * 1024) ? 1 : 0;
    h->smem_solve = vec + (h->use_global_S ? 0 : packed);
    D.Sglobal = nullptr;
    memset(&D.S, 0, sizeof(D.S));
    if (h->use_global_S) {
        rc = split_setup(h, 0, 1);
        if (rc != ICG_OK) return rc;
    } else {
        ICG_CUDA(raise_dynamic_smem((const void *) ba_solve, (size_t) (h->smem_solve)));
    }
    h->ld_schur = 16 * ((C.NCA + 15) / 16) + 8;
    h->smem_schur = sizeof(double) * std::max((size_t) SCHUR_RCH * h->ld_schur + SCHUR_RCH, (size_t) SCHUR_PASS * 256);
    ICG_CUDA(raise_dynamic_smem((const void *) ba_schur_dmma, (size_t) (h->smem_schur)));
    ICG_CUDA(cudaFuncSetAttribute(ba_schur_dmma, cudaFuncAttributePreferredSharedMemoryCarveout, cudaSharedmemCarveoutMaxShared));
    ICG_CUDA(raise_dynamic_smem((const void *) ba_lin_cam, (size_t) (h->smem_cam)));
    ICG_CUDA(raise_dynamic_smem((const void *) ba_cost_cam, (size_t) (h->smem_cam)));
    ICG_CUDA(raise_dynamic_smem((const void *) ba_lin_vis, LV_SMEM));
    ICG_CUDA(cudaStreamSynchronize(h->stream));
    h->cur_windows = 0;
    return ICG_OK;
}

cudaError_t launch_lm_ref_fill(icg_ba *h, int n, const SlideWin *win, const int *map, const double *old, double *out) {
    const int gx = std::max(1, std::min(8, (h->C.L + 255) / 256));
    ba_lm_ref_fill<<<dim3(gx, n), 256, 0, h->stream>>>(h->D.dims, win, map, old, h->D.f_const_s, h->D.lm_off, h->D.lm_perm, out, h->C.L, h->C.F);
    count_launch();
    return cudaGetLastError();
}

#define PK_FAIL(code, ...)                          \
    do {                                            \
        char eb_[512];                              \
        snprintf(eb_, sizeof(eb_), __VA_ARGS__);    \
        err = eb_;                                  \
        return code;                                \
    } while (0)
static int pack_window(icg_ba *h, int w, const icg_ba_problem &p, bool values, std::string &err) {
        const BaCaps &C = h->C;
        if (p.K < 2 || p.K > C.K || p.L < 0 || p.L > C.L || p.F < 0 || p.F > C.F || p.n_imu < 0 || p.n_imu > p.K - 1 || p.n_gnss < 0 || p.n_gnss > C.G ||
            p.marg_r < 0 || p.marg_r > C.R || p.marg_nblocks < 0 || p.marg_nblocks > 2 * C.K + 2 || !p.pose || !p.mix || !p.ext || (p.L > 0 && !p.invdepth) ||
            (p.F > 0 && (!p.f_lm || !p.f_ref || !p.f_obs || !p.f_const))) {
            PK_FAIL(ICG_EINVAL, "icg_ba_upload: window %d exceeds the handle's capacity or has null parameter arrays (K=%d L=%d F=%d gnss=%d marg_r=%d)", w, p.K, p.L, p.F,
                      p.n_gnss, p.marg_r);
        }
        WinDims &d = h->dims.h[w];
        d.K = p.K, d.L = p.L, d.F = p.F, d.n_imu = p.n_imu, d.n_gnss = p.n_gnss, d.marg_r = p.marg_r, d.marg_nb = p.marg_nblocks;
        d.ext_const = p.ext_const != 0, d.td_const = p.td_const != 0, d.reproj_huber = p.reproj_huber != 0, d.gnss_huber = p.gnss_huber != 0;
        d.has_imu_error = p.has_imu_error != 0, d.has_pose_prior = p.has_pose_prior != 0, d.has_mix_prior = p.has_mix_prior != 0;
        d.reproj_sinv = 1.0 / p.reproj_std;
        if (values) {
            memcpy(h->pose.h + (size_t) w * C.K * 7, p.pose, sizeof(double) * 7 * p.K);
            memcpy(h->mix.h + (size_t) w * C.K * 9, p.mix, sizeof(double) * 9 * p.K);
        }
        memcpy(h->ext.h + (size_t) w * 8, p.ext, sizeof(double) * 8);
        if (values && p.L > 0) memcpy(h->rho.h + (size_t) w * C.L, p.invdepth, sizeof(double) * p.L);
        for (int f = 0; f < p.F; f++) {
            if (p.f_lm[f] < 0 || p.f_lm[f] >= p.L || p.f_ref[f] < 0 || p.f_ref[f] >= p.K || p.f_obs[f] < 0 || p.f_obs[f] >= p.K || p.f_ref[f] == p.f_obs[f]) {
                PK_FAIL(ICG_EINVAL, "icg_ba_upload: window %d factor %d has invalid indices", w, f);
            }
        }
        std::vector<int> refof(p.L, -1);
        {
            std::vector<unsigned> seen((size_t) p.L, 0u);
            for (int f = 0; f < p.F; f++) {
                const int l = p.f_lm[f];
                if (refof[l] < 0) refof[l] = p.f_ref[f];
                if (refof[l] != p.f_ref[f] || (seen[l] >> p.f_obs[f]) & 1u) {
                    PK_FAIL(ICG_EINVAL, "icg_ba_upload: window %d factor %d: landmark %d has two reference nodes or two observations in node %d", w, f, l, p.f_obs[f]);
                }
                seen[l] |= 1u << p.f_obs[f];
            }
        }
        if (p.f_active)
            memcpy(h->f_active.h + (size_t) w * C.F, p.f_active, p.F);
        else
            memset(h->f_active.h + (size_t) w * C.F, 1, p.F);
        int *perm = h->lm_perm.h + (size_t) w * C.L;
        std::vector<int> pos_of(p.L);
        {
            std::vector<int> kcur(p.K + 2, 0);
            for (int l = 0; l < p.L; l++) kcur[(refof[l] < 0 ? p.K : refof[l]) + 1]++;
            for (int k = 0; k <= p.K; k++) kcur[k + 1] += kcur[k];
            for (int l = 0; l < p.L; l++) pos_of[l] = kcur[refof[l] < 0 ? p.K : refof[l]]++, perm[pos_of[l]] = l;
        }
        int *off = h->lm_off.h + (size_t) w * (C.L + 1), *fidx = h->lm_fidx.h + (size_t) w * C.F;
        for (int l = 0; l <= p.L; l++) off[l] = 0;
        for (int f = 0; f < p.F; f++) off[pos_of[p.f_lm[f]] + 1]++;
        for (int l = 0; l < p.L; l++) off[l + 1] += off[l];
        int *vbh = h->vb_lm0.h + (size_t) w * C.NVB, *meta = h->f_meta_s.h + (size_t) w * C.F * 4;
        int nrun = 0;
        {
            std::vector<int> cur(off, off + p.L);
            for (int f = 0; f < p.F; f++) fidx[cur[pos_of[p.f_lm[f]]]++] = f;
            int *nrun_of = h->ref_nrun.h + (size_t) w * C.K;
            for (int k = 0; k < C.K; k++) nrun_of[k] = 0;
            int l0 = 0;
            while (l0 < p.L) {
                const int ref = refof[perm[l0]];
                int l1 = l0;
                while (l1 < p.L && refof[perm[l1]] == ref && off[l1 + 1] - off[l0] <= 128) l1++;
                if (l1 == l0 || nrun >= C.NVB - 2) PK_FAIL(ICG_EINVAL, "icg_ba_upload: window %d: landmark %d has more than 128 factors or the run table overflows", w, perm[l0]);
                if (ref >= 0) nrun_of[ref]++;
                vbh[nrun++] = l0;
                l0 = l1;
            }
            vbh[nrun] = p.L;
            vbh[C.NVB - 1] = nrun;
            double *fcs = h->f_const_s.h + (size_t) w * C.F * 14;
            for (int q = 0; q < p.F; q++) {
                const int f = fidx[q];
                meta[4 * q] = p.f_lm[f], meta[4 * q + 1] = p.f_ref[f], meta[4 * q + 2] = p.f_obs[f], meta[4 * q + 3] = f;
                if (values) memcpy(fcs + (size_t) q * 14, p.f_const + (size_t) f * 14, sizeof(double) * 14);
            }
        }
        {
            const int PM = C.K * (C.K - 1);
            int *poff = h->part_off.h + (size_t) w * (PM + 1), *pro = h->pair_ro.h + (size_t) w * PM, *ord = h->vis_ord.h + (size_t) w * C.F;
            std::vector<int> slot((size_t) p.K * p.K, -1);
            for (int f = 0; f < p.F; f++) slot[(size_t) p.f_ref[f] * p.K + p.f_obs[f]] = 0;
            int P = 0;
            for (int key = 0; key < p.K * p.K; key++)
                if (slot[key] == 0) slot[key] = P, pro[P++] = ((key / p.K) << 8) | (key % p.K);
            std::vector<int> npart(P, 0);
            for (int r = 0; r < nrun; r++) {
                unsigned seen = 0u;
                for (int q = off[vbh[r]]; q < off[vbh[r + 1]]; q++) seen |= 1u << meta[4 * q + 2];
                for (int k = 0; k < p.K; k++)
                    if ((seen >> k) & 1u) npart[slot[(size_t) refof[perm[vbh[r]]] * p.K + k]]++;
            }
            poff[0] = 0;
            for (int i = 0; i < P; i++) poff[i + 1] = poff[i] + npart[i];
            std::vector<int> cur(poff, poff + P), start(p.K), pidx(p.K);
            for (int r = 0; r < nrun; r++) {
                const int a = off[vbh[r]], b = off[vbh[r + 1]];
                if (a == b) continue;
                const int ref = meta[4 * a + 1];
                std::fill(start.begin(), start.end(), 0);
                for (int q = a; q < b; q++) start[meta[4 * q + 2]]++;
                for (int k = 0, t = 0; k < p.K; k++) {
                    const int c = start[k];
                    start[k] = t, t += c;
                    if (c) pidx[k] = cur[slot[(size_t) ref * p.K + k]]++;
                }
                for (int q = a; q < b; q++) {
                    const int k = meta[4 * q + 2];
                    ord[a + start[k]++] = (q - a) | (pidx[k] << 8);
                }
            }
            h->npairs.h[w] = P;
        }
        for (int k = 0; values && k < p.n_imu; k++) {
            const double *b = p.imu_blob + (size_t) k * ICG_IMU_BLOB_DOUBLES;
            memcpy(h->imu_blob.h + ((size_t) w * C.K + k) * ICG_IMU_BLOB_DOUBLES, b, sizeof(double) * ICG_IMU_BLOB_DOUBLES);
            if (!host_imu_sqrt_info(b + 252, h->imu_U.h + ((size_t) w * C.K + k) * 225)) {
                PK_FAIL(ICG_EINVAL, "icg_ba_upload: window %d IMU factor %d has a non positive-definite covariance", w, k);
            }
        }
        for (int g = 0; g < p.n_gnss; g++) {
            if (p.gnss_node[g] < 0 || p.gnss_node[g] >= p.K) {
                PK_FAIL(ICG_EINVAL, "icg_ba_upload: window %d GNSS factor %d has an invalid node", w, g);
            }
            h->gnss_node.h[(size_t) w * C.G + g] = p.gnss_node[g];
        }
        if (values && p.n_gnss) {
            memcpy(h->gnss_blh.h + (size_t) w * C.G * 3, p.gnss_blh, sizeof(double) * 3 * p.n_gnss);
            memcpy(h->gnss_std.h + (size_t) w * C.G * 3, p.gnss_std, sizeof(double) * 3 * p.n_gnss);
        }
        memcpy(h->lever.h + (size_t) w * 3, p.lever, sizeof(double) * 3);
        if (p.has_pose_prior) {
            memcpy(h->pose_prior.h + (size_t) w * 7, p.pose_prior, sizeof(double) * 7);
            for (int k = 0; k < 6; k++) h->pose_prior_sinfo.h[(size_t) w * 6 + k] = 1.0 / p.pose_prior_std[k];
        }
        if (p.has_mix_prior) {
            memcpy(h->mix_prior.h + (size_t) w * 9, p.mix_prior, sizeof(double) * 9);
            memcpy(h->mix_prior_std.h + (size_t) w * 9, p.mix_prior_std, sizeof(double) * 9);
        }
        if (p.marg_r > 0) {
            const int r = p.marg_r;
            int tot = 0, cols = 0;
            for (int b = 0; b < p.marg_nblocks; b++) {
                int t = p.marg_block_type[b];
                if (t < 0 || t > 3 || ((t == 0 || t == 1) && (p.marg_block_node[b] < 0 || p.marg_block_node[b] >= p.K))) {
                    PK_FAIL(ICG_EINVAL, "icg_ba_upload: window %d marginalization block %d invalid", w, b);
                }
                tot += (t == 0 || t == 2) ? 7 : t == 1 ? 9 : 1;
                cols += (t == 0 || t == 2) ? 6 : t == 1 ? 9 : 1;
                h->marg_type.h[(size_t) w * BA_MARG_MAXB + b] = t;
                h->marg_node.h[(size_t) w * BA_MARG_MAXB + b] = p.marg_block_node[b];
            }
            if (cols != r || tot > BA_MARG_MAXB * 9) {
                PK_FAIL(ICG_EINVAL, "icg_ba_upload: window %d marginalization prior size mismatch (blocks give %d columns, marg_r=%d)", w, cols, r);
            }
            memcpy(h->marg_x0.h + (size_t) w * BA_MARG_MAXB * 9, p.marg_x0, sizeof(double) * tot);
            if (!values) return ICG_OK;
            double *H0 = h->marg_H0.h + (size_t) w * C.R * C.R, *b0 = h->marg_b0.h + (size_t) w * C.R;
            for (int i = 0; i < r; i++) {
                for (int j = i; j < r; j++) {
                    double s = 0;
                    for (int k = 0; k < r; k++) s += p.marg_J0[(size_t) k * r + i] * p.marg_J0[(size_t) k * r + j];
                    H0[(size_t) i * r + j] = H0[(size_t) j * r + i] = s;
                }
                double s = 0;
                for (int k = 0; k < r; k++) s += p.marg_J0[(size_t) k * r + i] * p.marg_e0[k];
                b0[i] = s;
            }
            double c0 = 0;
            for (int k = 0; k < r; k++) c0 += p.marg_e0[k] * p.marg_e0[k];
            h->marg_c0.h[w] = c0;
        }
            return ICG_OK;
}
#undef PK_FAIL

int pack_windows(icg_ba *h, int n, const icg_ba_problem *P, bool values) {
    const int nthreads = std::max(1, std::min({n / 4, 16, (int) std::thread::hardware_concurrency()}));
    std::vector<int> rcs(nthreads, ICG_OK);
    std::vector<std::string> errs(nthreads);
    auto worker = [&](int t) {
        for (int w = t; w < n; w += nthreads) {
            const int rc = pack_window(h, w, P[w], values, errs[t]);
            if (rc != ICG_OK) {
                rcs[t] = rc;
                return;
            }
        }
    };
    std::vector<std::thread> th;
    for (int t = 1; t < nthreads; t++) th.emplace_back(worker, t);
    worker(0);
    for (auto &x : th) x.join();
    for (int t = 0; t < nthreads; t++)
        if (rcs[t] != ICG_OK) {
            set_error("%s", errs[t].c_str());
            return rcs[t];
        }
    return ICG_OK;
}

int upload_structure(icg_ba *h, int n) {
    const BaCaps &C = h->C;
    cudaStream_t s = h->stream;
    const size_t nn = (size_t) n, PM = (size_t) C.K * (C.K - 1);
#define UP(field, stride) ICG_CUDA(h->field.up(s, nn * (size_t) (stride)))
    UP(dims, 1); UP(ext, 8);
    UP(f_active, C.F);
    UP(f_meta_s, C.F * 4); UP(vb_lm0, C.NVB); UP(lm_off, C.L + 1); UP(lm_perm, C.L); UP(ref_nrun, C.K); UP(part_off, PM + 1); UP(pair_ro, PM); UP(vis_ord, C.F);
    UP(npairs, 1); UP(gnss_node, C.G); UP(lever, 3);
    UP(pose_prior, 7); UP(pose_prior_sinfo, 6); UP(mix_prior, 9); UP(mix_prior_std, 9);
    UP(marg_type, BA_MARG_MAXB); UP(marg_node, BA_MARG_MAXB); UP(marg_x0, BA_MARG_MAXB * 9);
#undef UP
    return ICG_OK;
}

int keep_pristine(icg_ba *h, int n) {
    const BaCaps &C = h->C;
    const BaDev &D = h->D;
    cudaStream_t s = h->stream;
    ICG_CUDA(cudaMemcpyAsync(D.pose_0, D.pose, sizeof(double) * (size_t) n * C.K * 7, cudaMemcpyDeviceToDevice, s));
    ICG_CUDA(cudaMemcpyAsync(D.mix_0, D.mix, sizeof(double) * (size_t) n * C.K * 9, cudaMemcpyDeviceToDevice, s));
    ICG_CUDA(cudaMemcpyAsync(D.ext_0, D.ext, sizeof(double) * (size_t) n * 8, cudaMemcpyDeviceToDevice, s));
    ICG_CUDA(cudaMemcpyAsync(D.rho_0, D.rho, sizeof(double) * (size_t) n * C.L, cudaMemcpyDeviceToDevice, s));
    ICG_CUDA(cudaMemcpyAsync(D.f_active_0, D.f_active, (size_t) n * C.F, cudaMemcpyDeviceToDevice, s));
    ICG_CUDA(cudaMemcpyAsync(D.gnss_std_0, D.gnss_std, sizeof(double) * (size_t) n * C.G * 3, cudaMemcpyDeviceToDevice, s));
    return ICG_OK;
}

static int alloc_lin_buf2(icg_ba *h) {
    BaDev &D = h->D;
    if (D.Mp[1]) return ICG_OK;
    const BaCaps &C = h->C;
    const size_t NW = C.NW;
    int rc = ICG_OK;
#define DM(field, count) \
    if (rc == ICG_OK) rc = dmalloc(h, &D.field, count);
    DM(AW[1], NW * C.NCA * C.LP) DM(Mp[1], NW * (size_t) C.K * (C.K - 1) * 210) DM(costf[1], NW * C.F) DM(hl[1], NW * C.L) DM(gl[1], NW * C.L)
    DM(Hc[1], NW * C.NS * C.NS) DM(gc[1], NW * C.NS)
#undef DM
    return rc;
}

static int launch_solve_cam(icg_ba *h, int n, unsigned long long epoch) {
    const ClusterLaunch L((unsigned) (n * SPLIT_CLUSTER), SOLVE_THREADS, h->solve_cam_dsm ? h->smem_solve_cam_dsm : h->smem_solve_cam, h->stream,
                          SPLIT_CLUSTER);
    if (h->solve_cam_dsm) ICG_CUDA(cudaLaunchKernelEx(&L.cfg, ba_solve_cam_dsm, h->C, h->D, epoch));
    else ICG_CUDA(cudaLaunchKernelEx(&L.cfg, ba_solve_cam, h->C, h->D, epoch));
    return ICG_OK;
}

static int enqueue_lm_split(icg_ba *h, int max_num_iterations) {
    const BaCaps &C = h->C;
    const BaDev &D = h->D;
    const int n = h->cur_windows;
    cudaStream_t s = h->stream;
    for (int r = 0; r < D.world; r++)
        if (!D.S.peer[r]) {
            set_error("landmark-sharded solve: peer %d is not connected (icg_ba_shard_connect)", r);
            return ICG_EINVAL;
        }
    const dim3 g_vis(C.NVB - 2, n), g_cost(h->nblk_vis, n), g_nn(((C.NCV + 1) * (C.NCV + 1) + 255) / 256, n);
    for (int it = 0; it <= max_num_iterations; it++) {
        const unsigned long long epoch = ++h->epoch;
        ICG_CUDA(cudaEventRecord(h->ev_fork, s));
        ICG_CUDA(cudaStreamWaitEvent(h->stream_cam, h->ev_fork, 0));
        ba_lin_cam<<<n, cam_threads(h), h->smem_cam, h->stream_cam>>>(C, D, 0);
        ICG_CUDA(cudaEventRecord(h->ev_join, h->stream_cam));
        prof_mark(h, 0);
        ba_lin_vis<<<g_vis, 128, LV_SMEM, s>>>(C, D, 0);
        prof_mark(h, 1);
        ba_schur_dmma<<<dim3(BA_SPLIT_W, n), 256, h->smem_schur, s>>>(C, D, h->ld_schur);
        prof_mark(h, 5);
        ba_signal<<<1, 32, 0, s>>>(D, epoch);
        prof_mark(h, 7);
        ICG_CUDA(cudaStreamWaitEvent(s, h->ev_join, 0));
        prof_mark(h, 6);
        ba_reduce<<<g_nn, 256, 0, s>>>(C, D, epoch);
        prof_mark(h, 12);
        int rc = launch_solve_cam(h, n, epoch);
        if (rc != ICG_OK) return rc;
        prof_mark(h, 8);
        ba_step_lm<<<dim3(n, STEP_SLICES), SOLVE_THREADS, h->smem_step_lm, s>>>(C, D, epoch);
        prof_mark(h, 14);
        count_launch(7);
        if (it == max_num_iterations) break;
        ICG_CUDA(cudaEventRecord(h->ev_fork, s));
        ICG_CUDA(cudaStreamWaitEvent(h->stream_cam, h->ev_fork, 0));
        ba_cost_cam<<<n, cam_threads(h), h->smem_cam, h->stream_cam>>>(C, D, h->nblk_vis);
        ICG_CUDA(cudaEventRecord(h->ev_join, h->stream_cam));
        ba_cost<<<g_cost, 256, 0, s>>>(C, D, h->nblk_vis);
        ICG_CUDA(cudaStreamWaitEvent(s, h->ev_join, 0));
        prof_mark(h, 9);
        ba_exchange<<<(n + 63) / 64, 64, 0, s>>>(C, D, n, h->nblk_vis, epoch);
        prof_mark(h, 10);
        ba_accept_split<<<n, 128, 0, s>>>(C, D, epoch);
        prof_mark(h, 11);
        count_launch(4);
    }
    ICG_CHECK_LAUNCH();
    return ICG_OK;
}

static int enqueue_lm(icg_ba *h, int max_num_iterations) {
    if (h->D.S.split) return enqueue_lm_split(h, max_num_iterations);
    int rc = alloc_lin_buf2(h);
    if (rc != ICG_OK) return rc;
    const BaCaps &C = h->C;
    const BaDev &D = h->D;
    const int n = h->cur_windows;
    cudaStream_t s = h->stream;
    const dim3 g_vis(C.NVB - 2, n);
    auto enqueue_lin = [&](int at_cand) -> int {
        ICG_CUDA(cudaEventRecord(h->ev_fork, s));
        ICG_CUDA(cudaStreamWaitEvent(h->stream_cam, h->ev_fork, 0));
        ba_lin_cam<<<n, cam_threads(h), h->smem_cam, h->stream_cam>>>(C, D, at_cand);
        ICG_CUDA(cudaEventRecord(h->ev_join, h->stream_cam));
        prof_mark(h, 0);
        ba_lin_vis<<<g_vis, 128, LV_SMEM, s>>>(C, D, at_cand);
        prof_mark(h, at_cand ? 3 : 1);
        ICG_CUDA(cudaStreamWaitEvent(s, h->ev_join, 0));
        prof_mark(h, at_cand ? 3 : 6);
        count_launch(2);
        return ICG_OK;
    };
    rc = enqueue_lin(0);
    if (rc != ICG_OK) return rc;
    for (int it = 0; it <= max_num_iterations; it++) {
        ba_schur_dmma<<<dim3(BA_SPLIT_W, n), 256, h->smem_schur, s>>>(C, D, h->ld_schur);
        prof_mark(h, 5);
        ba_solve<<<n, SOLVE_THREADS, h->smem_solve, s>>>(C, D);
        prof_mark(h, 8);
        count_launch(2);
        if (it == max_num_iterations) break;
        rc = enqueue_lin(1);
        if (rc != ICG_OK) return rc;
        ba_accept<<<n, 128, sizeof(double) * 8 * h->nblk_vis, s>>>(C, D);
        prof_mark(h, 11);
        count_launch();
    }
    ICG_CHECK_LAUNCH();
    return ICG_OK;
}

static int restore_params(icg_ba *h) {
    const BaCaps &C = h->C;
    const BaDev &D = h->D;
    const int n = h->cur_windows;
    cudaStream_t s = h->stream;
    ICG_CUDA(cudaMemcpyAsync(D.pose, D.pose_0, sizeof(double) * (size_t) n * C.K * 7, cudaMemcpyDeviceToDevice, s));
    ICG_CUDA(cudaMemcpyAsync(D.mix, D.mix_0, sizeof(double) * (size_t) n * C.K * 9, cudaMemcpyDeviceToDevice, s));
    ICG_CUDA(cudaMemcpyAsync(D.ext, D.ext_0, sizeof(double) * (size_t) n * 8, cudaMemcpyDeviceToDevice, s));
    ICG_CUDA(cudaMemcpyAsync(D.rho, D.rho_0, sizeof(double) * (size_t) n * C.L, cudaMemcpyDeviceToDevice, s));
    ICG_CUDA(cudaMemcpyAsync(D.f_active, D.f_active_0, (size_t) n * C.F, cudaMemcpyDeviceToDevice, s));
    ICG_CUDA(cudaMemcpyAsync(D.gnss_std, D.gnss_std_0, sizeof(double) * (size_t) n * C.G * 3, cudaMemcpyDeviceToDevice, s));
    ICG_CUDA(h->dims.up(s, n));
    return ICG_OK;
}

static void fill_summary(const LmState &st, icg_ba_summary &o) {
    o.iterations = st.iter, o.num_successful_steps = st.n_success;
    o.termination = st.done == 2 ? 1 : st.done == 3 ? 2 : 0;
    o.reserved = 0;
    o.initial_cost = st.initial_cost, o.final_cost = st.x_cost, o.final_radius = st.radius;
}

int shard_timed_out(icg_ba *h, const char *what) {
    if (icg_ba_shard_error(h) == 0) return ICG_OK;
    set_error("%s: a peer exchange of the shard group timed out (a rank did not make the same call)", what);
    return ICG_ECUDA;
}

int shard_xsum(icg_ba *h, int *v, int stride, int n, int nv, int op) {
    const unsigned long long epoch = ++h->epoch;
    const int par = (int) (h->xs_calls++ & 1);
    ba_xsum<<<1, 256, 0, h->stream>>>(h->C, h->D, v, stride, n, nv, op, par, epoch);
    ICG_CHECK_LAUNCH();
    count_launch();
    return ICG_OK;
}

int shard_xmax(icg_ba *h, int *v3, const char *fn) {
    int rc = hd_reserve(h, h->xs_v, 8, fn);
    if (rc != ICG_OK) return rc;
    memcpy(h->xs_v.h, v3, 3 * sizeof(int));
    ICG_CUDA(h->xs_v.up(h->stream, 3));
    rc = shard_xsum(h, h->xs_v.d, 3, 1, 3, 1);
    if (rc != ICG_OK) return rc;
    ICG_CUDA(h->xs_v.down(h->stream, 3));
    ICG_CUDA(cudaStreamSynchronize(h->stream));
    rc = shard_timed_out(h, fn);
    if (rc != ICG_OK) return rc;
    memcpy(v3, h->xs_v.h, 3 * sizeof(int));
    return ICG_OK;
}

int shard_agree(icg_ba *h, bool rejected, int fp, const char *fn) {
    int mx[3] = {rejected ? h->D.rank + 1 : 0, rejected ? 0 : fp, rejected ? 0 : -fp};
    const int rc = shard_xmax(h, mx, fn);
    if (rc != ICG_OK || rejected) return rc != ICG_OK ? rc : ICG_EINVAL;
    if (mx[0]) {
        set_error("%s: rank %d of the shard group rejected the call (see that rank's error); no rank changed its handle", fn, mx[0] - 1);
        return ICG_EINVAL;
    }
    if (mx[1] != -mx[2]) {
        set_error("%s: the ranks' camera sides differ (node, IMU and GNSS rows and maps, the prior's source and the integration's inputs must be "
                  "the same on every rank); no rank changed its handle", fn);
        return ICG_EINVAL;
    }
    return ICG_OK;
}

struct ShardBlob {
    uint64_t magic, pid, ptr, doubles;
    int32_t rank, world, device, pad;
    cudaIpcMemHandle_t ipc;
};
static_assert(sizeof(ShardBlob) <= ICG_SHARD_BLOB_BYTES, "ShardBlob size");

static int small_factor_eval(icg_ba *h, int kind, const double *in, int nin, double *out, int nout) {
    ICG_CUDA(cudaSetDevice(h->device));
    memcpy(h->scratch.h, in, sizeof(double) * nin);
    ICG_CUDA(cudaMemcpyAsync(h->scratch.d, h->scratch.h, sizeof(double) * nin, cudaMemcpyHostToDevice, h->stream));
    ba_small_factor_eval_kernel<<<1, 1, 0, h->stream>>>(kind, h->scratch.d, h->scratch.d + 128);
    count_launch();
    ICG_CUDA(cudaMemcpyAsync(h->scratch.h + 128, h->scratch.d + 128, sizeof(double) * nout, cudaMemcpyDeviceToHost, h->stream));
    ICG_CUDA(cudaStreamSynchronize(h->stream));
    memcpy(out, h->scratch.h + 128, sizeof(double) * nout);
    return ICG_OK;
}

extern "C" {

int icg_imu_preintegrate(const double *state16, const double *iewn3, const double *gravity3, const double *noise5, const double *imu, int n, double *blob,
                         double *end_state10) {
    if (!state16 || !gravity3 || !noise5 || !imu || !blob || n < 1) {
        set_error("icg_imu_preintegrate: bad arguments");
        return ICG_EINVAL;
    }
    gc::preintegrate_core(state16, iewn3, gravity3, noise5, imu, n, blob, end_state10);
    return ICG_OK;
}

int icg_ba_create(icg_ba **out, int max_windows, int max_K, int max_L, int max_F, int max_gnss, int max_marg_r, int device, void *stream) {
    if (!out || max_windows < 1 || max_K < 2 || max_K > 32 || max_L < 0 || max_F < 0 || max_gnss < 0 || max_marg_r < 0) {
        set_error("icg_ba_create: bad arguments");
        return ICG_EINVAL;
    }
    int ndev = 0;
    if (cudaGetDeviceCount(&ndev) != cudaSuccess || ndev == 0) {
        set_error("icg_ba_create: no CUDA device (this library has no CPU fallback)");
        return ICG_ENODEVICE;
    }
    if (device < 0 || device >= ndev) {
        set_error("icg_ba_create: device %d out of range", device);
        return ICG_EINVAL;
    }
    ICG_CUDA(cudaSetDevice(device));
    cudaDeviceProp prop;
    ICG_CUDA(cudaGetDeviceProperties(&prop, device));
    if (prop.major != 9 || prop.minor != 0) {
        set_error("icg_ba_create: device is sm_%d%d; this library is built for sm_90a only", prop.major, prop.minor);
        return ICG_ENODEVICE;
    }
    icg_ba *h = new icg_ba();
    h->device = device;
    const int rc_init = ba_create_body(h, max_windows, max_K, max_L, max_F, max_gnss, max_marg_r, stream);
    if (rc_init != ICG_OK) {
        icg_ba_destroy(h);
        return rc_init;
    }
    *out = h;
    return ICG_OK;
}

void icg_ba_destroy(icg_ba *h) {
    if (!h) return;
    cudaSetDevice(h->device);
    if (h->stream) cudaStreamSynchronize(h->stream);
    prof_collect(h);
    prof_print(h);
    for (cudaEvent_t e : h->prof_ev) cudaEventDestroy(e);
    split_release(h);
    if (h->mx_h) icg_ba_destroy(h->mx_h);
    if (h->mx_rows) cudaFree(h->mx_rows);
    for (double *p : {h->M.H0, h->M.b0, h->M.G1, h->M.V1, h->M.lam1, h->M.Z})
        if (p) cudaFree(p);
    if (h->slide_old) cudaFree(h->slide_old);
    for (double *p : {h->store_d[0], h->store_d[1], h->cut_rows})
        if (p) cudaFree(p);
    if (h->ins_ev) cudaEventDestroy(h->ins_ev);
    if (h->fc_alt) cudaFree(h->fc_alt);
    if (h->slide_ev) cudaEventDestroy(h->slide_ev);
    for (void *p : h->dev_only) cudaFree(p);
    if (h->stream_cam) cudaStreamSynchronize(h->stream_cam), cudaStreamDestroy(h->stream_cam);
    if (h->ev_fork) cudaEventDestroy(h->ev_fork);
    if (h->ev_join) cudaEventDestroy(h->ev_join);
    if (h->own_stream && h->stream) cudaStreamDestroy(h->stream);
    delete h;
}

int icg_ba_upload(icg_ba *h, int n, const icg_ba_problem *P) {
    if (!h || !P || n < 1 || n > h->C.NW) {
        set_error("icg_ba_upload: bad arguments (n=%d, capacity %d)", n, h ? h->C.NW : 0);
        return ICG_EINVAL;
    }
    ICG_CUDA(cudaSetDevice(h->device));
    const BaCaps &C = h->C;
    h->marg_res_n = 0;
    h->cull_res_n = 0;
    h->lists_n = 0;
    h->store_valid = false;
    int rc = pack_windows(h, n, P, true);
    if (rc != ICG_OK) return rc;
    rc = upload_structure(h, n);
    if (rc != ICG_OK) return rc;
    cudaStream_t s = h->stream;
    const size_t nn = (size_t) n;
#define UP(field, stride) ICG_CUDA(h->field.up(s, nn * (size_t) (stride)))
    UP(pose, C.K * 7); UP(mix, C.K * 9); UP(rho, C.L); UP(f_const_s, C.F * 14); UP(imu_blob, C.K * ICG_IMU_BLOB_DOUBLES); UP(imu_U, C.K * 225);
    UP(gnss_blh, C.G * 3); UP(gnss_std, C.G * 3); UP(marg_H0, (size_t) C.R * C.R); UP(marg_b0, C.R); UP(marg_c0, 1);
#undef UP
    ICG_CUDA(launch_lm_ref_fill(h, n, nullptr, nullptr, nullptr, h->lm_ref));
    rc = keep_pristine(h, n);
    if (rc != ICG_OK) return rc;
    h->cur_windows = n;
    return ICG_OK;
}

int icg_ba_run(icg_ba *h, int max_num_iterations, int restart) {
    if (!h || h->cur_windows < 1 || max_num_iterations < 0) {
        set_error("icg_ba_run: no problems uploaded");
        return ICG_EINVAL;
    }
    ICG_CUDA(cudaSetDevice(h->device));
    const int n = h->cur_windows;
    if (restart) {
        int rc = restore_params(h);
        if (rc != ICG_OK) return rc;
    }
    ba_reset_state<<<(n + 127) / 128, 128, 0, h->stream>>>(h->D, nullptr, n, max_num_iterations);
    count_launch();
    return enqueue_lm(h, max_num_iterations);
// ... 419 lines not shown
```

ic_gvins_b200/csrc/ba_split.cuh:

```cuda
#pragma once
#include <cooperative_groups.h>

namespace icg {
namespace cg = cooperative_groups;

__device__ __forceinline__ unsigned long long ld_acquire_sys(const unsigned long long *p) {
    unsigned long long v;
    asm volatile("ld.acquire.sys.global.u64 %0, [%1];" : "=l"(v) : "l"(p) : "memory");
    return v;
}
__device__ __forceinline__ void st_release_sys(unsigned long long *p, unsigned long long v) {
    asm volatile("st.release.sys.global.u64 [%0], %1;" ::"l"(p), "l"(v) : "memory");
}
__device__ __forceinline__ void wait_flag(const unsigned long long *f, unsigned long long epoch, int *err) {
    const long long t0 = clock64();
    while (ld_acquire_sys(f) < epoch) {
        if (clock64() - t0 > 4000000000ll) {
            atomicExch(err, 1);
            break;
        }
        __nanosleep(64);
    }
}

__device__ __forceinline__ double *x_inbox(const BaDev &D, int peer, int w, int from) {
    const ShardDev &S = D.S;
    return S.peer[peer] + S.off_inbox + ((size_t) (w / D.world) * D.world + from) * S.PK;
}
__device__ __forceinline__ double *x_bcast(const BaDev &D, int peer, int w) { return D.S.peer[peer] + D.S.off_bcast + (size_t) w * D.S.BS; }
__device__ __forceinline__ double *x_scal(const BaDev &D, int peer, int w, int from) {
    return D.S.peer[peer] + D.S.off_scal + ((size_t) w * D.world + from) * SPLIT_SCAL;
}
__device__ __forceinline__ unsigned long long *x_flagA(const BaDev &D, int peer, int from) {
    return (unsigned long long *) (D.S.peer[peer] + D.S.off_flagA) + from;
}
__device__ __forceinline__ unsigned long long *x_flagB(const BaDev &D, int peer, int w) {
    return (unsigned long long *) (D.S.peer[peer] + D.S.off_flagB) + w;
}
__device__ __forceinline__ unsigned long long *x_flagC(const BaDev &D, int peer, int w, int from) {
    return (unsigned long long *) (D.S.peer[peer] + D.S.off_flagC) + (size_t) w * D.world + from;
}
__device__ __forceinline__ int tri_idx(int A, int B, int ncv) { return A * ncv - A * (A - 1) / 2 + (B - A); }

__global__ void ba_signal(BaDev D, unsigned long long epoch) {
    const int q = threadIdx.x;
    if (q >= D.world) return;
    __threadfence_system();
    st_release_sys(x_flagA(D, q, D.rank), epoch);
}

__global__ void __launch_bounds__(256) ba_reduce(BaCaps C, BaDev D, unsigned long long epoch) {
    const int w = blockIdx.y, tid = threadIdx.x;
    if (w % D.world != D.rank) return;
    if (D.st[w].done) return;
    const int K = D.dims[w].K, NCV = 6 * K + 7, nn = NCV + 1, TRI = NCV * (NCV + 1) / 2;
    if ((int) blockIdx.x * 256 >= nn * nn) return;
    if (tid < D.world) wait_flag(x_flagA(D, D.rank, tid), epoch, D.S.err);
    __syncthreads();
    const int t = blockIdx.x * 256 + tid;
    if (t >= nn * nn) return;
    const int A = t / nn, B = t - A * nn;
    if (B < A) return;
    const double *P0 = x_inbox(D, D.rank, w, 0);
    const size_t PK = D.S.PK;
    auto rsum = [&](int e) {
        double s = 0;
        for (int r = 0; r < D.world; r++) s += __ldcg(P0 + (size_t) r * PK + e);
        return s;
    };
    double *rv = D.S.redv + (size_t) w * D.S.RV;
    if (A < NCV && B < NCV) {
        D.Hs[(size_t) w * C.NS * C.NS + (size_t) B * C.NS + A] = lin_Hc(C, D, 0, w)[(size_t) B * C.NS + A] + rsum(tri_idx(A, B, NCV));
        if (A == B) rv[A] = rsum(TRI + A);
    } else if (A < NCV) {
        rv[NCV + A] = rsum(TRI + NCV + A);
        rv[2 * NCV + A] = rsum(TRI + 2 * NCV + A);
    } else {
        rv[3 * NCV] = rsum(TRI + 3 * NCV);
        rv[3 * NCV + 1] = rsum(TRI + 3 * NCV + 1);
        double m = 0;
        for (int r = 0; r < D.world; r++) m = fmax(m, __ldcg(P0 + (size_t) r * PK + TRI + 3 * NCV + 2));
        rv[3 * NCV + 2] = m;
    }
}


__device__ __forceinline__ void split_col(const BaCaps &C, const BaDev &D, int w, int NCV, int a, const LmState &s0, double &g, double &sc, double &d2,
                                          double &rh) {
    const double *rv = D.S.redv + (size_t) w * D.S.RV;
    const double gv = lin_gc(C, D, 0, w)[a] + (a < NCV ? rv[NCV + a] : 0.0);
    const double h = lin_Hc(C, D, 0, w)[(size_t) a * C.NS + a] + (a < NCV ? rv[a] : 0.0);
    const double sv = s0.first ? 1.0 / (1.0 + sqrt(h)) : D.scale_c[(size_t) w * C.NS + a];
    g = gv, sc = sv, d2 = lm_d2(sv * sv * h, s0.radius), rh = -sv * (gv - (a < NCV ? rv[2 * NCV + a] : 0.0));
}

__device__ __forceinline__ void split_hdr(double *BC, int term, bool valid, double x_cost, double gmax, double init, double mcc) {
    BC[0] = (double) term, BC[1] = valid ? 1.0 : 0.0, BC[2] = x_cost, BC[3] = gmax, BC[4] = init, BC[5] = mcc;
}

__device__ __forceinline__ void split_bcast(const BaDev &D, int w, int N, bool valid, double nfin, const double *x, const double *s_scale, double x_cost,
                                            double gmax, double init, double mcc, unsigned long long epoch) {
    const int tid = threadIdx.x;
    for (int q = 0; q < D.world; q++) {
        double *BC = x_bcast(D, q, w);
        if (valid)
            for (int a = tid; a < N; a += SOLVE_THREADS) BC[SPLIT_HDR + a] = x[a] * s_scale[a];
        if (tid == 0) split_hdr(BC, 0, valid && nfin == 0.0, x_cost, gmax, init, mcc);
    }
    __threadfence_system();
    __syncthreads();
    for (int q = tid; q < D.world; q += SOLVE_THREADS) st_release_sys(x_flagB(D, q, w), epoch);
}

__global__ void __launch_bounds__(SOLVE_THREADS) ba_solve_cam(BaCaps C, BaDev D, unsigned long long epoch) {
    extern __shared__ double sm[];
    cg::cluster_group cluster = cg::this_cluster();
    const int CL = (int) cluster.num_blocks(), cr = (int) cluster.block_rank();
    const int w = blockIdx.x / CL, tid = threadIdx.x, lane = tid & 31, warp = tid >> 5;
    if (w % D.world != D.rank) return;
    LmState &st = D.st[w];
    if (st.done) return;
    const WinDims dm = D.dims[w];
    const int K = dm.K, NCV = 6 * K + 7, N = 15 * K + 7, NR = N + 1;
    const int CT = CL * SOLVE_THREADS, ctid = cr * SOLVE_THREADS + tid, cwarp = ctid >> 5, ncwarps = CT / 32;
    const LmState s0 = st;
    double *s_red = sm;
    double *s_scale = s_red + 40;
    double *s_g = s_scale + C.NS;
    double *s_rhs = s_g + C.NS;
    double *s_d2 = s_rhs + C.NS;
    double *s_blk = s_d2 + C.NS;
    double *S = D.Sglobal + (size_t) (w / D.world) * split_S_stride(C);
    const double *Hc = lin_Hc(C, D, 0, w), *Hs = D.Hs + (size_t) w * C.NS * C.NS;
    for (int a = tid; a < N; a += SOLVE_THREADS) split_col(C, D, w, NCV, a, s0, s_g[a], s_scale[a], s_d2[a], s_rhs[a]);
    __syncthreads();
    double x_cost = s0.x_cost, gmax = s0.gmax;
    if (s0.fresh_lin) {
        const double *rv = D.S.redv + (size_t) w * D.S.RV;
        double gm = 0;
        for (int a = tid; a < N; a += SOLVE_THREADS) gm = fmax(gm, fabs(s_g[a]));
        gmax = fmax(block_max(gm, s_red), rv[3 * NCV + 2]);
        x_cost = rv[3 * NCV] + s0.cost_cam[0];
    }
    const int term = lm_term(s0.iter, s0.max_iter, s0.last_success, gmax, s0.radius);
    cluster.sync();
    if (cr == 0 && tid == 0) lm_begin(st, x_cost, gmax, s0.first ? x_cost : s0.initial_cost, term);
    if (cr == 0 && s0.first)
        for (int a = tid; a < N; a += SOLVE_THREADS) D.scale_c[(size_t) w * C.NS + a] = s_scale[a];
    if (term) {
        if (cr == 0) {
            __syncthreads();
            for (int q = tid; q < D.world; q += SOLVE_THREADS) {
                split_hdr(x_bcast(D, q, w), term, false, x_cost, gmax, s0.first ? x_cost : s0.initial_cost, 0.0);
                __threadfence_system();
                st_release_sys(x_flagB(D, q, w), epoch);
            }
        }
        return;
    }
    for (int i = cwarp; i < N; i += ncwarps) {
        const double *src = (i < NCV ? Hs : Hc) + (size_t) i * C.NS;
        double *dst = S + (size_t) i * (i + 1) / 2;
        const double si = s_scale[i];
        for (int j = lane; j <= i; j += 32) {
            double v = si * s_scale[j] * src[j];
            if (i == j) v += s_d2[i];
            dst[j] = v;
        }
    }
    for (int a = ctid; a < N; a += CT) S[(size_t) N * (N + 1) / 2 + a] = s_rhs[a];
    cluster.sync();
    double *dinvg = S + (size_t) (C.N + 1) * (C.N + 2) / 2;
    double *s_b = s_blk;
    const int ldbp = ((C.N + 15) / 16) * 16 + 8;
    int fail = 0;
#ifdef ICG_BA_PHASE_CLOCKS
#define CAMS_CLK(k, t0)                                                                                             \
    if (D.clk && w == 0 && ctid == 0) atomicAdd(&D.clk[k], clock64() - (t0)), atomicAdd(&D.clk[8 + (k)], 1ull);
#define CAMS_NOW() clock64()
#else
#define CAMS_CLK(k, t0)
#define CAMS_NOW() 0ull
#endif
    const unsigned long long tc_all = CAMS_NOW();
    (void) tc_all;
    for (int J0 = 0; J0 < N; J0 += BA_CHOL_NB) {
        const int nb = min(BA_CHOL_NB, N - J0);
        const int g = lane >> 2, kk = lane & 3;
        const int ntile = (NR - J0 + 7) / 8;
        const unsigned long long tc0 = CAMS_NOW();
        (void) tc0;
        if (J0 > 0) {
            for (int e = tid; e < 8 * J0; e += SOLVE_THREADS) {
                const int r = e / J0, c = e - r * J0, row = J0 + r;
                s_b[r * ldbp + c] = row < NR ? S[(size_t) row * (row + 1) / 2 + c] : 0.0;
            }
            __syncthreads();
        }
        CAMS_CLK(0, tc0)
        const unsigned long long tc1 = CAMS_NOW();
        (void) tc1;
        auto tile_update = [&](int tI) {
            const int ia = J0 + 8 * tI + g;
            const bool oka = ia < NR;
            const double *ra = S + (oka ? (size_t) ia * (ia + 1) / 2 : 0);
            const double *sb = s_b + g * ldbp;
            double c0 = 0, c1 = 0, d0 = 0, d1 = 0, e0 = 0, e1 = 0, f0 = 0, f1 = 0;
            for (int k0 = 0; k0 < J0; k0 += 64) {
                double a[16];
#pragma unroll
                for (int u = 0; u < 16; u++) a[u] = (oka && k0 + 4 * u < J0) ? ra[k0 + 4 * u + kk] : 0.0;
#pragma unroll
                for (int u = 0; u < 16; u += 4) {
                    if (k0 + 4 * u < J0) {
                        const double b0 = sb[k0 + 4 * u + kk], b1 = k0 + 4 * u + 4 < J0 ? sb[k0 + 4 * u + 4 + kk] : 0.0;
                        const double b2 = k0 + 4 * u + 8 < J0 ? sb[k0 + 4 * u + 8 + kk] : 0.0, b3 = k0 + 4 * u + 12 < J0 ? sb[k0 + 4 * u + 12 + kk] : 0.0;
                        dmma884(c0, c1, a[u], b0);
                        dmma884(d0, d1, a[u + 1], b1);
                        dmma884(e0, e1, a[u + 2], b2);
                        dmma884(f0, f1, a[u + 3], b3);
                    }
                }
            }
            c0 += d0 + (e0 + f0), c1 += d1 + (e1 + f1);
            if (oka) {
                const int ca = J0 + 2 * kk;
                double *ri = S + (size_t) ia * (ia + 1) / 2;
                if (ca < J0 + nb && ca <= ia) ri[ca] -= c0;
                if (ca + 1 < J0 + nb && ca + 1 <= ia) ri[ca + 1] -= c1;
            }
        };
        if (cwarp == 0) {
            double *s_jj = s_b + 8 * ldbp;
            {
                const int ia = J0 + g;
                const bool oka = ia < NR;
                const int ca = J0 + 2 * kk;
                double v0 = 0, v1 = 0;
                if (oka && ca <= ia && ca < J0 + nb) v0 = S[(size_t) ia * (ia + 1) / 2 + ca];
                if (oka && ca + 1 <= ia && ca + 1 < J0 + nb) v1 = S[(size_t) ia * (ia + 1) / 2 + ca + 1];
                if (J0 > 0) {
                    const double *sa = s_b + g * ldbp;
                    double c0 = 0, c1 = 0, d0 = 0, d1 = 0, e0 = 0, e1 = 0, f0 = 0, f1 = 0;
                    int k0 = 0;
                    for (; k0 + 16 <= J0; k0 += 16) {
                        const double x0 = sa[k0 + kk], x1 = sa[k0 + 4 + kk], x2 = sa[k0 + 8 + kk], x3 = sa[k0 + 12 + kk];
                        dmma884(c0, c1, x0, x0);
                        dmma884(d0, d1, x1, x1);
                        dmma884(e0, e1, x2, x2);
                        dmma884(f0, f1, x3, x3);
                    }
                    for (; k0 + 4 <= J0; k0 += 4) {
                        const double x0 = sa[k0 + kk];
                        dmma884(c0, c1, x0, x0);
                    }
                    v0 -= c0 + d0 + (e0 + f0), v1 -= c1 + d1 + (e1 + f1);
                }
                s_jj[g * 8 + 2 * kk] = v0, s_jj[g * 8 + 2 * kk + 1] = v1;
                if (oka && ia >= J0 + nb) {
                    if (ca < J0 + nb) S[(size_t) ia * (ia + 1) / 2 + ca] = v0;
                    if (ca + 1 < J0 + nb) S[(size_t) ia * (ia + 1) / 2 + ca + 1] = v1;
                }
                __syncwarp();
            }
            double Ld[BA_CHOL_NB][BA_CHOL_NB], dinv[BA_CHOL_NB];
            bool bad = false;
#pragma unroll
            for (int a = 0; a < BA_CHOL_NB; a++)
#pragma unroll
                for (int b = 0; b < BA_CHOL_NB; b++) Ld[a][b] = (a < nb && b <= a) ? s_jj[a * 8 + b] : (a == b ? 1.0 : 0.0);
#pragma unroll
            for (int j = 0; j < BA_CHOL_NB; j++) {
                double d = Ld[j][j];
#pragma unroll
                for (int k = 0; k < j; k++) d -= Ld[j][k] * Ld[j][k];
                if (!(d > 0.0) || !isfinite(d)) bad = true;
                const double di = rsqrt(d);
                dinv[j] = di;
                Ld[j][j] = d * di;
#pragma unroll
                for (int a = j + 1; a < BA_CHOL_NB; a++) {
                    double sum = Ld[a][j];
#pragma unroll
                    for (int k = 0; k < j; k++) sum -= Ld[a][k] * Ld[j][k];
                    Ld[a][j] = sum * di;
                }
            }
            __syncwarp();
#pragma unroll
            for (int a2 = 0; a2 < BA_CHOL_NB; a2++) {
                double *ri = S + (size_t) (J0 + a2) * (J0 + a2 + 1) / 2 + J0;
#pragma unroll
                for (int b = 0; b <= a2; b++)
                    if (lane == ((a2 * 8 + b) & 31) && a2 < nb) ri[b] = Ld[a2][b];
                if (lane == 8 + a2 && a2 < nb) dinvg[J0 + a2] = bad ? -1.0 : dinv[a2];
            }
            CAMS_CLK(1, tc1)
        } else if (J0 > 0) {
            for (int tI = cwarp; tI < ntile; tI += ncwarps - 1) tile_update(tI);
        }
        cluster.sync();
        CAMS_CLK(2, tc1)
        const unsigned long long tc2 = CAMS_NOW();
        (void) tc2;
        fail = dinvg[J0] < 0.0;
        if (fail) break;
        for (int i = J0 + nb + ctid; i < NR; i += CT) {
            double *ri = S + (size_t) i * (i + 1) / 2 + J0;
            double x[BA_CHOL_NB], Lb[BA_CHOL_NB * (BA_CHOL_NB - 1) / 2], dv[BA_CHOL_NB];
#pragma unroll
            for (int c = 0; c < BA_CHOL_NB; c++) {
                x[c] = c < nb ? ri[c] : 0.0;
                dv[c] = c < nb ? dinvg[J0 + c] : 1.0;
#pragma unroll
                for (int k = 0; k < c; k++) Lb[c * (c - 1) / 2 + k] = c < nb ? S[(size_t) (J0 + c) * (J0 + c + 1) / 2 + J0 + k] : 0.0;
            }
#pragma unroll
            for (int c = 0; c < BA_CHOL_NB; c++) {
                double sum = x[c];
#pragma unroll
                for (int k = 0; k < c; k++) sum -= x[k] * Lb[c * (c - 1) / 2 + k];
                x[c] = sum * dv[c];
            }
#pragma unroll
            for (int c = 0; c < BA_CHOL_NB; c++)
                if (c < nb) ri[c] = x[c];
        }
        cluster.sync();
        CAMS_CLK(3, tc2)
    }
    CAMS_CLK(4, tc_all)
    if (cr != 0) return;
    const bool valid = !fail;
    double *y = s_rhs;
    __syncthreads();
    if (valid) {
        for (int a = tid; a < N; a += SOLVE_THREADS) y[a] = S[(size_t) N * (N + 1) / 2 + a];
        __syncthreads();
        const int ldb = C.NS + 1;
        for (int j1 = N; j1 > 0; j1 -= SPLIT_BS_ROWS) {
            const int j0 = max(0, j1 - SPLIT_BS_ROWS), nr = j1 - j0;
            for (int e = tid; e < nr * j1; e += SOLVE_THREADS) {
                const int r = e / j1, c = e - r * j1;
                const int row = j0 + r;
                s_blk[r * ldb + c] = c <= row ? S[(size_t) row * (row + 1) / 2 + c] : 0.0;
            }
            __syncthreads();
            if (warp == 0) {
                double xv = lane < nr ? y[j0 + lane] : 0.0;
                for (int r = nr - 1; r >= 0; r--) {
                    const double xj = __shfl_sync(0xffffffffu, xv, r) / s_blk[r * ldb + j0 + r];
                    if (lane == r) xv = xj;
                    if (lane < r) xv -= s_blk[r * ldb + j0 + lane] * xj;
                }
                if (lane < nr) y[j0 + lane] = xv;
            }
            __syncthreads();
            for (int c = tid; c < j0; c += SOLVE_THREADS) {
                double acc = y[c];
                for (int r = 0; r < nr; r++) acc -= s_blk[r * ldb + c] * y[j0 + r];
                y[c] = acc;
            }
            __syncthreads();
        }
    }
    double part = 0;
    bool finite = true;
    if (valid)
        for (int a = tid; a < N; a += SOLVE_THREADS) {
            const double sp = y[a];
            finite = finite && isfinite(sp);
            part += -0.5 * sp * (s_scale[a] * s_g[a]) + 0.5 * s_d2[a] * sp * sp;
        }
    const double mcc = block_sum(part, s_red);
    const double nfin = block_sum(finite ? 0.0 : 1.0, s_red);
    split_bcast(D, w, N, valid, nfin, y, s_scale, x_cost, gmax, s0.first ? x_cost : s0.initial_cost, mcc, epoch);
}

__host__ __device__ inline int dsm_tile_off(int cr, int m) { return m * cr + 2 * m * (m - 1); }

__device__ __forceinline__ unsigned mapa_u32(unsigned addr, unsigned rank) {
    unsigned r;
    asm volatile("mapa.shared::cluster.u32 %0, %1, %2;" : "=r"(r) : "r"(addr), "r"(rank));
    return r;
}
__device__ __forceinline__ void dsm_mbar_init(unsigned bar, unsigned count) { asm volatile("mbarrier.init.shared::cta.b64 [%0], %1;" ::"r"(bar), "r"(count) : "memory"); }
__device__ __forceinline__ void dsm_mbar_arrive_local(unsigned bar) { asm volatile("mbarrier.arrive.release.cta.shared::cta.b64 _, [%0];" ::"r"(bar) : "memory"); }
__device__ __forceinline__ void dsm_mbar_arrive_expect_tx_remote(unsigned bar_cluster, unsigned tx) {
    asm volatile("mbarrier.arrive.expect_tx.release.cluster.shared::cluster.b64 _, [%0], %1;" ::"r"(bar_cluster), "r"(tx) : "memory");
}
__device__ __forceinline__ void st_async_f64(unsigned dst_cluster, double a, unsigned bar_cluster) {
    asm volatile("st.async.weak.shared::cluster.mbarrier::complete_tx::bytes.f64 [%0], %1, [%2];" ::"r"(dst_cluster), "d"(a), "r"(bar_cluster) : "memory");
}
__device__ __forceinline__ bool dsm_mbar_try_wait(unsigned bar, unsigned parity) {
    unsigned ok;
    asm volatile("{\n\t.reg .pred p;\n\tmbarrier.try_wait.parity.acquire.cluster.shared::cta.b64 p, [%1], %2;\n\tselp.u32 %0, 1, 0, p;\n\t}" : "=r"(ok) : "r"(bar), "r"(parity) : "memory");
    return ok != 0;
}
__device__ __forceinline__ void dsm_mbar_wait(unsigned bar, unsigned parity, volatile int *s_dead, int *err) {
    if (dsm_mbar_try_wait(bar, parity)) return;
    const long long t0 = clock64();
    while (!dsm_mbar_try_wait(bar, parity)) {
        if (*s_dead) return;
        if (clock64() - t0 > 400000000ll) {
            *s_dead = 1;
            atomicExch(err, 1);
            return;
        }
    }
}

__global__ void __launch_bounds__(SOLVE_THREADS, 1) ba_solve_cam_dsm(BaCaps C, BaDev D, unsigned long long epoch) {
    extern __shared__ double sm[];
    cg::cluster_group cluster = cg::this_cluster();
    constexpr int CL = DSM_CL;
    const int cr = (int) cluster.block_rank();
    const int w = blockIdx.x / CL, tid = threadIdx.x, lane = tid & 31, warp = tid >> 5;
    if (w % D.world != D.rank) return;
    LmState &st = D.st[w];
    if (st.done) return;
    const WinDims dm = D.dims[w];
    const int K = dm.K, NCV = 6 * K + 7, N = 15 * K + 7, NR = N + 1;
    const int ntc = dsm_ntiles(C.N + 1), VL = ntc * 8;
    const int nt = dsm_ntiles(NR), npan = (N + 7) / 8;
    const int Tn = N >> 3, rn = N & 7;
    const LmState s0 = st;
    double *s_red = sm;
    double *s_scale = s_red + 40;
    double *s_g = s_scale + VL;
    double *s_rhs = s_g + VL;
    double *s_d2 = s_rhs + VL;
    double *s_y = s_d2 + VL;
    double *s_contrib = s_y + VL;
    double *s_x = s_contrib + VL;
    double *s_dinv = s_x + VL;
    double *s_Lf = s_dinv + VL;
    double *s_dv = s_Lf + 64;
    double *s_inbox = s_dv + 8;
    double *s_xT = s_inbox + 8 * CL;
    int *s_fail = (int *) (s_xT + 8);
    unsigned long long *s_bar = (unsigned long long *) (s_xT + 12);
    double *s_dg = s_xT + 16;
    double *s_P = s_dg + (size_t) ntc * 64;
    double *s_tiles = s_P + (size_t) 2 * ntc * 64;
    const double *Hc = lin_Hc(C, D, 0, w), *Hs = D.Hs + (size_t) w * C.NS * C.NS;
    for (int a = tid; a < VL; a += SOLVE_THREADS) {
        double g = 0, sc = 0, d2 = 0, rh = 0;
        if (a < N) split_col(C, D, w, NCV, a, s0, g, sc, d2, rh);
        s_g[a] = g, s_scale[a] = sc, s_d2[a] = d2, s_rhs[a] = rh;
        s_y[a] = 0, s_contrib[a] = 0, s_x[a] = 0, s_dinv[a] = 0;
    }
    if (tid < 8 * CL) s_inbox[tid] = 0;
    if (tid == 0) {
        s_fail[0] = 0, s_fail[1] = 0;
        dsm_mbar_init(smem_u32(s_bar), CL - 1);
        asm volatile("fence.mbarrier_init.release.cluster;" ::: "memory");
    }
    __syncthreads();
    double x_cost = s0.x_cost, gmax = s0.gmax;
    if (s0.fresh_lin) {
        const double *rv = D.S.redv + (size_t) w * D.S.RV;
        double gm = 0;
        for (int a = tid; a < N; a += SOLVE_THREADS) gm = fmax(gm, fabs(s_g[a]));
        gmax = fmax(block_max(gm, s_red), rv[3 * NCV + 2]);
        x_cost = rv[3 * NCV] + s0.cost_cam[0];
    }
    const int term = lm_term(s0.iter, s0.max_iter, s0.last_success, gmax, s0.radius);
    cluster.sync();
    if (cr == 0 && tid == 0) lm_begin(st, x_cost, gmax, s0.first ? x_cost : s0.initial_cost, term);
    if (cr == 0 && s0.first)
        for (int a = tid; a < N; a += SOLVE_THREADS) D.scale_c[(size_t) w * C.NS + a] = s_scale[a];
    if (term) {
        if (cr == 0) {
            __syncthreads();
            for (int q = tid; q < D.world; q += SOLVE_THREADS) {
                split_hdr(x_bcast(D, q, w), term, false, x_cost, gmax, s0.first ? x_cost : s0.initial_cost, 0.0);
                __threadfence_system();
                st_release_sys(x_flagB(D, q, w), epoch);
            }
        }
        return;
    }
#ifdef ICG_BA_PHASE_CLOCKS
#define DSM_CLK(k, t0)                                                                                             \
    if (D.clk && w == 0 && cr == 0 && tid == 0) atomicAdd(&D.clk[k], clock64() - (t0)), atomicAdd(&D.clk[8 + (k)], 1ull);
#define DSM_CLK2(k, t0)                                                                                            \
    if (D.clk && w == 0 && cr == 0 && tid == 0) atomicAdd(&D.clk[32 + (k)], clock64() - (t0)), atomicAdd(&D.clk[40 + (k)], 1ull);
#define DSM_NOW() clock64()
#else
#define DSM_CLK(k, t0)
#define DSM_CLK2(k, t0)
#define DSM_NOW() 0ull
#endif
    const unsigned long long tq0 = DSM_NOW();
    (void) tq0;
    for (int m = 0, T = cr; T < nt; m += 2, T += 2 * CL) {
        constexpr int NCH = (15 * 22 + 7 + 31) / 32;
        double v[2][NCH];
#pragma unroll
        for (int h = 0; h < 2; h++) {
            const int Th = T + h * CL, i = 8 * Th + warp, ncol = 8 * Th;
            const double *src = (i < NCV ? Hs : Hc) + (size_t) (i < N ? i : 0) * C.NS;
#pragma unroll
            for (int u = 0; u < NCH; u++) {
                const int j = 32 * u + lane;
                v[h][u] = (Th < nt && j < ncol && i < N) ? __ldcg(src + j) : 0.0;
            }
        }
#pragma unroll
        for (int h = 0; h < 2; h++) {
            const int Th = T + h * CL, i = 8 * Th + warp, ncol = 8 * Th;
            if (Th >= nt) continue;
            double *trow = s_tiles + (size_t) dsm_tile_off(cr, m + h) * 64 + warp * 8;
            const double si = i < N ? s_scale[i] : 0.0;
#pragma unroll
            for (int u = 0; u < NCH; u++) {
                const int j = 32 * u + lane;
                if (j < ncol) trow[(j >> 3) * 64 + (j & 7)] = i < N ? si * s_scale[j] * v[h][u] : (i == N ? s_rhs[j] : 0.0);
            }
        }
    }
    {
        constexpr int NDG = (dsm_ntiles(15 * 22 + 8) * 64 + SOLVE_THREADS - 1) / SOLVE_THREADS;
        double v[NDG];
#pragma unroll
        for (int u = 0; u < NDG; u++) {
            const int e = tid + u * SOLVE_THREADS, T = e >> 6, r = (e >> 3) & 7, c = e & 7, i = 8 * T + r, j = 8 * T + c;
            v[u] = (e < nt * 64 && c <= r && i < N) ? __ldcg((i < NCV ? Hs : Hc) + (size_t) i * C.NS + j) : 0.0;
        }
#pragma unroll
        for (int u = 0; u < NDG; u++) {
            const int e = tid + u * SOLVE_THREADS, T = e >> 6, r = (e >> 3) & 7, c = e & 7, i = 8 * T + r, j = 8 * T + c;
            if (e >= nt * 64) continue;
            double x = 0;
            if (c <= r) {
                if (i < N) x = s_scale[i] * s_scale[j] * v[u] + (i == j ? s_d2[i] : 0.0);
                else if (i == N && j < N) x = s_rhs[j];
            }
            s_dg[e] = x;
        }
    }
    volatile int *s_dead = s_fail + 1;
    __syncthreads();
    DSM_CLK(0, tq0)
    const int wi = warp < 4 ? warp - 1 : warp - 2;
    const bool worker = warp != 0 && warp != 4;
    int fail = 0;
    const unsigned long long tc_all = DSM_NOW();
    (void) tc_all;
    for (int J = 0; J < npan; J++) {
        const int nb = min(8, N - 8 * J);
        const double *PJ = s_P + (size_t) ((J - 1) & 1) * ntc * 64;
        if (J > 0 && tid < 8 && Tn > J - 1) s_y[8 * (J - 1) + tid] = PJ[(size_t) Tn * 64 + rn * 8 + tid];
        const unsigned long long tc1 = DSM_NOW();
        (void) tc1;
        if (J > 0 && worker) {
            const int Jp = J - 1;
            auto run = [&](double a0, double a1, bool diag, const double *pb, double *pc, int n) {
                for (; n > 0; n -= 4, pb += 256, pc += 256) {
                    double2 bq[4], cq[4];
#pragma unroll
                    for (int u = 0; u < 4; u++)
                        if (u < n) bq[u] = *(const double2 *) (pb + 64 * u), cq[u] = *(double2 *) (pc + 64 * u);
#pragma unroll
                    for (int u = 0; u < 4; u++)
                        if (u < n) dmma884(cq[u].x, cq[u].y, diag ? -bq[u].x : a0, bq[u].x);
#pragma unroll
                    for (int u = 0; u < 4; u++)
                        if (u < n) dmma884(cq[u].x, cq[u].y, diag ? -bq[u].y : a1, bq[u].y);
#pragma unroll
                    for (int u = 0; u < 4; u++)
                        if (u < n) *(double2 *) (pc + 64 * u) = cq[u];
                }
            };
            auto run2 = [&](double a10, double a11, double a20, double a21, const double *pb, double *pc1, double *pc2, int n) {
                for (; n > 0; n -= 4, pb += 256, pc1 += 256, pc2 += 256) {
                    double2 bq[4], c1[4], c2[4];
#pragma unroll
                    for (int u = 0; u < 4; u++)
                        if (u < n) bq[u] = *(const double2 *) (pb + 64 * u), c1[u] = *(double2 *) (pc1 + 64 * u), c2[u] = *(double2 *) (pc2 + 64 * u);
#pragma unroll
                    for (int u = 0; u < 4; u++)
                        if (u < n) dmma884(c1[u].x, c1[u].y, a10, bq[u].x), dmma884(c2[u].x, c2[u].y, a20, bq[u].x);
#pragma unroll
                    for (int u = 0; u < 4; u++)
                        if (u < n) dmma884(c1[u].x, c1[u].y, a11, bq[u].y), dmma884(c2[u].x, c2[u].y, a21, bq[u].y);
#pragma unroll
                    for (int u = 0; u < 4; u++)
                        if (u < n) *(double2 *) (pc1 + 64 * u) = c1[u], *(double2 *) (pc2 + 64 * u) = c2[u];
                }
            };
            if (wi < 5) {
                const int m_lo = (Jp + 2 - cr + CL - 1) / CL, m_hi = cr < nt ? (nt - 1 - cr) / CL : -1;
                for (int i = wi; m_lo + i <= m_hi - i; i += 5) {
                    const int m1 = m_lo + i, m2 = m_hi - i, T1 = cr + CL * m1, T2 = cr + CL * m2;
                    const double2 pa1 = *(const double2 *) (PJ + (size_t) T1 * 64 + 2 * lane);
                    double *t1 = s_tiles + (size_t) dsm_tile_off(cr, m1) * 64 + 2 * lane;
                    const double *pb0 = PJ + (size_t) (Jp + 1) * 64 + 2 * lane;
                    if (m1 == m2) {
                        run(-pa1.x, -pa1.y, false, pb0, t1 + (size_t) (Jp + 1) * 64, T1 - (Jp + 1));
                    } else {
                        const double2 pa2 = *(const double2 *) (PJ + (size_t) T2 * 64 + 2 * lane);
                        double *t2 = s_tiles + (size_t) dsm_tile_off(cr, m2) * 64 + 2 * lane;
                        run2(-pa1.x, -pa1.y, -pa2.x, -pa2.y, pb0, t1 + (size_t) (Jp + 1) * 64, t2 + (size_t) (Jp + 1) * 64, T1 - (Jp + 1));
                        run(-pa2.x, -pa2.y, false, PJ + (size_t) T1 * 64 + 2 * lane, t2 + (size_t) T1 * 64, T2 - T1);
                    }
                }
            } else {
                run(0.0, 0.0, true, PJ + (size_t) (Jp + 2) * 64 + 2 * lane, s_dg + (size_t) (Jp + 2) * 64 + 2 * lane, nt - (Jp + 2));
            }
        }
        if (warp == 0) {
            const unsigned long long tf0 = DSM_NOW();
            (void) tf0;
            double *dg = s_dg + (size_t) J * 64;
            if (J > 0) {
                const double2 p = *(const double2 *) (PJ + (size_t) J * 64 + 2 * lane);
                double2 c = *(double2 *) (dg + 2 * lane);
                dmma884(c.x, c.y, -p.x, p.x);
                dmma884(c.x, c.y, -p.y, p.y);
                *(double2 *) (dg + 2 * lane) = c;
                __syncwarp();
            }
            DSM_CLK2(2, tf0)
            const unsigned long long tf1 = DSM_NOW();
            (void) tf1;
            double Ld[8][8], dinv[8];
            bool bad = false;
#pragma unroll
            for (int a = 0; a < 8; a++)
#pragma unroll
                for (int b = 0; b < 8; b++) Ld[a][b] = (a < nb && b <= a) ? dg[a * 8 + b] : (a == b ? 1.0 : 0.0);
#pragma unroll
            for (int j = 0; j < 8; j++) {
                double d = Ld[j][j];
#pragma unroll
                for (int k = 0; k < j; k++) d -= Ld[j][k] * Ld[j][k];
                if (!(d > 0.0) || !isfinite(d)) bad = true;
                const double di = rsqrt(d);
                dinv[j] = di;
                Ld[j][j] = d * di;
#pragma unroll
                for (int a = j + 1; a < 8; a++) {
                    double sum = Ld[a][j];
#pragma unroll
                    for (int k = 0; k < j; k++) sum -= Ld[a][k] * Ld[j][k];
                    Ld[a][j] = sum * di;
                }
            }
#ifdef ICG_BA_PHASE_CLOCKS
            if (Ld[7][7] == 12345.678) bad = true;
#endif
            DSM_CLK2(3, tf1)
            const unsigned long long tf2 = DSM_NOW();
            (void) tf2;
            __syncwarp();
#pragma unroll
            for (int a2 = 0; a2 < 8; a2++) {
#pragma unroll
                for (int b = 0; b <= a2; b++)
                    if (lane == ((a2 * 8 + b) & 31) && a2 < nb) dg[a2 * 8 + b] = Ld[a2][b];
                if (lane == 8 + a2) s_dv[a2] = dinv[a2];
                if (lane == 16 + a2 && a2 < nb) s_dinv[8 * J + a2] = dinv[a2];
            }
            if (lane == 0 && bad) s_fail[0] = 1;
            DSM_CLK2(4, tf2)
            DSM_CLK(1, tf0)
        }
        __syncthreads();
        DSM_CLK(2, tc1)
        const unsigned long long tc2 = DSM_NOW();
        (void) tc2;
        fail = s_fail[0];
        if (fail) break;
        {
            const int m0 = (J + 1 - cr + CL - 1) / CL;
            const int m = m0 + (tid >> 3), r = tid & 7, T = cr + CL * m;
            if (T < nt) {
                double *tp = s_tiles + ((size_t) dsm_tile_off(cr, m) + J) * 64 + r * 8;
                const double *s_Ljj = s_dg + (size_t) J * 64;
                double x[8];
#pragma unroll
                for (int c = 0; c < 8; c += 2) {
                    const double2 t2 = *(const double2 *) (tp + c);
                    x[c] = t2.x, x[c + 1] = t2.y;
                }
#pragma unroll
                for (int c = 0; c < 8; c++) {
                    double sum = x[c];
#pragma unroll
                    for (int k = 0; k < c; k++) sum -= x[k] * s_Ljj[c * 8 + k];
                    x[c] = sum * s_dv[c];
                }
                double *dstP = s_P + (size_t) (J & 1) * ntc * 64 + (size_t) T * 64 + r * 8;
#pragma unroll
                for (int c = 0; c < 8; c += 2) *(double2 *) (tp + c) = make_double2(x[c], x[c + 1]);
#pragma unroll
                for (int q = 0; q < CL; q++) {
                    double *rp = cluster.map_shared_rank(dstP, q);
#pragma unroll
                    for (int c = 0; c < 8; c += 2) *(double2 *) (rp + c) = make_double2(x[c], x[c + 1]);
                }
            }
            cluster.sync();
        }
        DSM_CLK(3, tc2)
    }
    DSM_CLK(4, tc_all)
    const bool valid = !fail;
    const unsigned long long tb0 = DSM_NOW();
    (void) tb0;
    if (valid) {
        {
            const int J = npan - 1;
            if (tid < 8 && Tn > J) s_y[8 * J + tid] = s_P[(size_t) (J & 1) * ntc * 64 + (size_t) Tn * 64 + rn * 8 + tid];
        }
        if (rn > 0 && tid == 0) {
            double x[8];
            for (int c = 0; c < rn; c++) {
                double sum = s_dg[(size_t) Tn * 64 + rn * 8 + c];
                for (int k = 0; k < c; k++) sum -= x[k] * s_dg[(size_t) Tn * 64 + c * 8 + k];
                x[c] = sum * s_dv[c];
                s_y[8 * Tn + c] = x[c];
            }
        }
        __syncthreads();
        double *rX0 = cluster.map_shared_rank(s_x, 0);
        for (int T = npan - 1; T >= 0; T--) {
            if (cr == T % CL) {
                const int nbT = min(8, N - 8 * T), m = T / CL;
                const double *trow = s_tiles + (size_t) dsm_tile_off(cr, m) * 64;
                const int c0 = max(0, 8 * (T - 3)), ncrit = 8 * T - c0;
                if (warp == 0) {
                    const int c = lane & 7, col = c0 + lane;
                    double lcol[8], tcr[8], acc = 0;
#pragma unroll
                    for (int r = 0; r < 8; r++) lcol[r] = s_dg[(size_t) T * 64 + r * 8 + c];
                    if (lane < ncrit) {
                        const double *tp = trow + (col >> 3) * 64 + (col & 7);
#pragma unroll
                        for (int r = 0; r < 8; r++) tcr[r] = tp[r * 8];
                        acc = s_contrib[col];
                    } else {
#pragma unroll
                        for (int r = 0; r < 8; r++) tcr[r] = 0;
                    }
                    const int nmiss = max(0, 3 - (npan - 1 - T));
                    if (lane < nmiss) dsm_mbar_arrive_local(smem_u32(s_bar));
                    dsm_mbar_wait(smem_u32(s_bar), ((npan - 1 - T) / CL) & 1, s_dead, D.S.err);
                    double v = 0;
                    if (lane < nbT) {
                        v = s_y[8 * T + c] - s_contrib[8 * T + c];
#pragma unroll
                        for (int q = 0; q < CL; q++)
                            if (q != cr) v -= s_inbox[q * 8 + c];
                    }
#pragma unroll
                    for (int r = 7; r >= 0; r--) {
                        const double xr = __shfl_sync(0xffffffffu, v, r) * s_dinv[8 * T + r];
                        if (lane == r) v = xr;
                        else if (lane < r) v -= lcol[r] * xr;
                    }
                    if (lane < 8) s_xT[lane] = v, rX0[8 * T + lane] = v;
#pragma unroll
                    for (int r = 0; r < 8; r++) acc += tcr[r] * __shfl_sync(0xffffffffu, v, r);
                    if (lane < ncrit) {
                        s_contrib[col] = acc;
                        const int q = (col >> 3) % CL;
                        const unsigned abar = mapa_u32(smem_u32(s_bar), q);
                        st_async_f64(mapa_u32(smem_u32(s_inbox + cr * 8 + (col & 7)), q), acc, abar);
                        if ((col & 7) == 0) dsm_mbar_arrive_expect_tx_remote(abar, 64u);
                    }
                }
                __syncthreads();
                for (int col = tid; col < c0; col += SOLVE_THREADS) {
                    const double *tp = trow + (col >> 3) * 64 + (col & 7);
                    double acc = s_contrib[col];
#pragma unroll
                    for (int r = 0; r < 8; r++) acc += tp[r * 8] * s_xT[r];
                    s_contrib[col] = acc;
                }
                __syncthreads();
            }
        }
    }
    cluster.sync();
    DSM_CLK(5, tb0)
    if (cr != 0) return;
    double part = 0;
    bool finite = true;
    if (valid)
        for (int a = tid; a < N; a += SOLVE_THREADS) {
            const double sp = s_x[a];
            finite = finite && isfinite(sp);
            part += -0.5 * sp * (s_scale[a] * s_g[a]) + 0.5 * s_d2[a] * sp * sp;
        }
    const double mcc = block_sum(part, s_red);
    const double nfin = block_sum(finite ? 0.0 : 1.0, s_red);
    split_bcast(D, w, N, valid, nfin, s_x, s_scale, x_cost, gmax, s0.first ? x_cost : s0.initial_cost, mcc, epoch);
}

__global__ void __launch_bounds__(SOLVE_THREADS) ba_step_lm(BaCaps C, BaDev D, unsigned long long epoch) {
    extern __shared__ double sm[];
    __shared__ int s_last;
    const int w = blockIdx.x, sl_id = blockIdx.y, tid = threadIdx.x;
    LmState &st = D.st[w];
    const WinDims dm = D.dims[w];
    const int K = dm.K, L = dm.L, NCV = 6 * K + 7, N = 15 * K + 7;
    const bool owner = (w % D.world) == D.rank;
    double *s_red = sm, *s_dl = s_red + 40;
    if (st.done) return;
    const double *BC = x_bcast(D, D.rank, w);
    if (tid == 0) wait_flag(x_flagB(D, D.rank, w), epoch, D.S.err);
    __syncthreads();
    const int term = (int) __ldcg(BC + 0), valid = (int) __ldcg(BC + 1);
    double *R3 = D.red2 + (size_t) w * 4;
    if (!owner && tid == 0 && sl_id == 0) lm_begin(st, __ldcg(BC + 2), __ldcg(BC + 3), __ldcg(BC + 4), term);
    if (term) return;
    if (!valid) {
        if (tid == 0 && sl_id == 0) {
            st.chol_ok = 0, st.step_valid = 0;
            R3[0] = 0, R3[1] = 0, R3[2] = 1, R3[3] = 0;
        }
        return;
    }
    for (int a = tid; a < N; a += SOLVE_THREADS) s_dl[a] = __ldcg(BC + SPLIT_HDR + a);
    __syncthreads();
    const double radius = st.radius;
    const double *hl = lin_hl(C, D, 0, w), *gl = lin_gl(C, D, 0, w), *scale_l = D.scale_l + (size_t) w * C.L;
    double *step_l = D.step_l + (size_t) w * C.L;
    const double *AW = lin_AW(C, D, 0, w);
// ... 254 lines not shown
```

Baseline: 24590.

## Store camera Hessian as block-tridiagonal band plus prior index instead of dense

Replaces the dense NS x NS camera Hessian Hc with a compact block-tridiagonal band of 15x15 node blocks. The marginalization prior H0 is now read through an inverse column map instead of being scattered into Hc. Diagonal blocks are accumulated in shared memory rather than with global atomics. The solve and split paths gather entries through hc_ptr lookups and no longer add Hc into Hs during the Schur store. This cuts zeroing, atomic traffic and memory footprint, in exchange for more indexing logic and scattered cp.async gathers when a prior is present.

```diff
diff --git a/ic_gvins_b200/csrc/ba.cu b/ic_gvins_b200/csrc/ba.cu
--- a/ic_gvins_b200/csrc/ba.cu
+++ b/ic_gvins_b200/csrc/ba.cu
@@ -16,13 +16,42 @@
 __device__ __forceinline__ double *lin_costf(const BaCaps &C, const BaDev &D, int b, int w) { return D.costf[b] + (size_t) w * C.F; }
 __device__ __forceinline__ double *lin_hl(const BaCaps &C, const BaDev &D, int b, int w) { return D.hl[b] + (size_t) w * C.L; }
 __device__ __forceinline__ double *lin_gl(const BaCaps &C, const BaDev &D, int b, int w) { return D.gl[b] + (size_t) w * C.L; }
-__device__ __forceinline__ double *lin_Hc(const BaCaps &C, const BaDev &D, int b, int w) { return D.Hc[b] + (size_t) w * C.NS * C.NS; }
+__device__ __forceinline__ double *lin_Hband(const BaCaps &C, const BaDev &D, int b, int w) { return D.Hc_band[b] + (size_t) w * hc_band_stride(C.K); }
+__device__ __forceinline__ int *lin_Hinv(const BaCaps &C, const BaDev &D, int b, int w) { return D.Hc_inv[b] + (size_t) w * C.NS; }
 __device__ __forceinline__ double *lin_gc(const BaCaps &C, const BaDev &D, int b, int w) { return D.gc[b] + (size_t) w * C.NS; }
 
 __device__ __forceinline__ int col_pose(int k) { return 6 * k; }
 __device__ __forceinline__ int col_ext(int K) { return 6 * K; }
 __device__ __forceinline__ int col_td(int K) { return 6 * K + 6; }
 __device__ __forceinline__ int col_mix(int K, int k) { return 6 * K + 7 + 9 * k; }
+
+__device__ __forceinline__ int hc_node(int K, int c) {
+    if (c < 6 * K) return (c / 6) << 4 | (c % 6);
+    if (c < 6 * K + 7) return -1;
+    const int m = c - 6 * K - 7;
+    return (m / 9) << 4 | (6 + m % 9);
+}
+__device__ __forceinline__ const double *hc_ptr_in(const double *band, const int *inv, const double *H0, int CK, int K, int r, int i, int j) {
+    const int ni = hc_node(K, i), nj = hc_node(K, j);
+    if (ni >= 0 && nj >= 0) {
+        const int ki = ni >> 4, kj = nj >> 4, ai = ni & 15, aj = nj & 15;
+        if (ki == kj) return band + ki * HC_BLK + ai * HC_NODE + aj;
+        if (ki == kj + 1) return band + (CK + kj) * HC_BLK + ai * HC_NODE + aj;
+        if (kj == ki + 1) return band + (CK + ki) * HC_BLK + aj * HC_NODE + ai;
+    }
+    if (r > 0) {
+        const int pi = inv[i], pj = pi >= 0 ? inv[j] : -1;
+        if (pj >= 0) return H0 + pi * r + pj;
+    }
+    return nullptr;
+}
+__device__ __forceinline__ const double *hc_ptr(const BaCaps &C, const BaDev &D, int b, int w, int K, int r, int i, int j) {
+    return hc_ptr_in(lin_Hband(C, D, b, w), lin_Hinv(C, D, b, w), D.marg_H0 + (size_t) w * C.R * C.R, C.K, K, r, i, j);
+}
+__device__ __forceinline__ double hc_at(const BaCaps &C, const BaDev &D, int b, int w, int K, int r, int i, int j) {
+    const double *p = hc_ptr(C, D, b, w, K, r, i, j);
+    return p ? *p : 0.0;
+}
 
 __device__ __forceinline__ double block_sum(double v, double *s_red);
 __device__ __forceinline__ double block_max(double v, double *s_red);
@@ -291,7 +320,6 @@
     const int NCV = 6 * K + 7;
     if (A == NCV) return;
     const size_t e = (size_t) w * C.NS * C.NS + (size_t) B * C.NS + A;
-    const double hc = !D.S.split && B < NCV ? lin_Hc(C, D, buf, w)[(size_t) B * C.NS + A] : 0.0;
     const double cj = gram2_entry(C, D, buf, w, K, s_slot, A, B);
     if (D.S.split) {
         double *P = x_inbox(D, w % D.world, w, D.rank);
@@ -306,7 +334,7 @@
     } else {
         double *V = D.visv + (size_t) w * 3 * C.NCV;
         if (B < NCV) {
-            D.Hs[e] = hc + (cj - cw);
+            D.Hs[e] = cj - cw;
             if (A == B) V[A] = cj;
         } else {
             V[NCV + A] = cj, V[2 * NCV + A] = cw;
@@ -532,12 +560,14 @@
                               bool lin, int b, double *smem) {
     const int tid = threadIdx.x, lane = tid & 31, warp = tid >> 5, nwarps = blockDim.x >> 5;
     const int K = dm.K, N = 15 * K + 7;
-    double *Hc = lin_Hc(C, D, b, w), *gc = lin_gc(C, D, b, w);
+    double *Hband = lin_Hband(C, D, b, w), *gc = lin_gc(C, D, b, w);
     double *s_imu = smem;
     double *s_gnss = s_imu + (size_t) C.K * 480;
     double *s_misc = s_gnss + (size_t) C.G * 24;
     double *s_pp = s_misc, *s_mp = s_misc + 48, *s_dx = s_mp + 16, *s_y = s_dx + C.R, *s_cost = s_y + C.R;
-    int *s_colmap = (int *) (s_cost + 8);
+    double *s_hd = s_cost + 8;
+    int *s_colmap = (int *) (s_hd + (size_t) C.K * HC_BLK);
+    int *s_inv = s_colmap + C.R;
     __shared__ double s_total;
 #ifdef ICG_BA_PHASE_CLOCKS
     unsigned long long cclk = D.clk ? clock64() : 0ull;
@@ -621,8 +651,10 @@
         return s_total;
     }
     CAM_CLK(1)
-    for (int e = tid; e < N * C.NS; e += blockDim.x) Hc[e] = 0;
+    for (int e = tid; e < K * HC_BLK; e += blockDim.x) s_hd[e] = 0;
     for (int e = tid; e < N; e += blockDim.x) gc[e] = 0;
+    if (dm.marg_r > 0)
+        for (int c = tid; c < N; c += blockDim.x) s_inv[c] = -1;
     __syncthreads();
     CAM_CLK(2)
     if (dm.marg_r > 0) {
@@ -630,12 +662,21 @@
         for (int e = tid; e < r * r; e += blockDim.x) {
             int i = e / r, j = e - i * r;
             int ci = s_colmap[i], cj = s_colmap[j];
-            if (ci >= 0 && cj >= 0) Hc[(size_t) ci * C.NS + cj] = H0[e];
+            const int ni = ci >= 0 ? hc_node(K, ci) : -1, nj = cj >= 0 ? hc_node(K, cj) : -1;
+            if (ni >= 0 && nj >= 0 && (ni >> 4) == (nj >> 4)) s_hd[(ni >> 4) * HC_BLK + (ni & 15) * HC_NODE + (nj & 15)] = H0[e];
         }
         for (int i = tid; i < r; i += blockDim.x)
-            if (s_colmap[i] >= 0) gc[s_colmap[i]] = b0[i] + s_y[i];
-    }
-    __syncthreads();
+            if (s_colmap[i] >= 0) gc[s_colmap[i]] = b0[i] + s_y[i], s_inv[s_colmap[i]] = i;
+    }
+    __syncthreads();
+    if (dm.marg_r > 0) {
+        int *inv = lin_Hinv(C, D, b, w);
+        for (int c = tid; c < N; c += blockDim.x) inv[c] = s_inv[c];
+    }
+    auto prior_at = [&](int ci, int cj) {
+        const int pi = dm.marg_r > 0 ? s_inv[ci] : -1, pj = pi >= 0 ? s_inv[cj] : -1;
+        return pj >= 0 ? H0[(size_t) pi * dm.marg_r + pj] : 0.0;
+    };
     CAM_CLK(3)
     for (int parity = 0; parity < 2; parity++) {
         const int nf = (dm.n_imu - parity + 1) / 2;
@@ -644,10 +685,14 @@
             const double *rw = s_imu + (size_t) k * 480, *Jw = rw + 30;
             auto gcol = [&](int c) { return c < 6 ? col_pose(k) + c : c < 15 ? col_mix(K, k) + c - 6 : c < 21 ? col_pose(k + 1) + c - 15 : col_mix(K, k + 1) + c - 21; };
             if (q < 900) {
-                int a = q / 30, b = q - a * 30;
+                const int a = q / 30, b = q - a * 30, na = a >= 15, nb = b >= 15;
+                if (!na && nb) continue;
                 double s = 0;
                 for (int m = 0; m < 15; m++) s += Jw[m * 30 + a] * Jw[m * 30 + b];
-                red_add(&Hc[(size_t) gcol(a) * C.NS + gcol(b)], s);
+                if (na == nb)
+                    s_hd[(k + na) * HC_BLK + (a - 15 * na) * HC_NODE + b - 15 * nb] += s;
+                else
+                    Hband[(C.K + k) * HC_BLK + (a - 15) * HC_NODE + b] = prior_at(gcol(a), gcol(b)) + s;
             } else {
                 int a = q - 900;
                 double s = 0;
@@ -658,6 +703,11 @@
         __syncthreads();
     }
     CAM_CLK(4)
+    for (int e = dm.n_imu * HC_BLK + tid; e < (K - 1) * HC_BLK; e += blockDim.x) {
+        const int k = e / HC_BLK, a = (e - k * HC_BLK) / HC_NODE, c = e - k * HC_BLK - a * HC_NODE;
+        Hband[(C.K + k) * HC_BLK + a * HC_NODE + c] =
+            prior_at(a < 6 ? col_pose(k + 1) + a : col_mix(K, k + 1) + a - 6, c < 6 ? col_pose(k) + c : col_mix(K, k) + c - 6);
+    }
     for (int e = tid; e < K * 42; e += blockDim.x) {
         const int k = e / 42, q = e % 42;
         double s = 0;
@@ -670,7 +720,7 @@
                 }
             if (k == 0 && dm.has_pose_prior)
                 for (int m = 0; m < 6; m++) s += s_pp[6 + m * 6 + a] * s_pp[6 + m * 6 + b];
-            red_add(&Hc[(size_t) (col_pose(k) + a) * C.NS + col_pose(k) + b], s);
+            s_hd[k * HC_BLK + a * HC_NODE + b] += s;
         } else {
             const int a = q - 36;
             for (int g = 0; g < dm.n_gnss; g++)
@@ -687,17 +737,18 @@
         if (dm.has_imu_error && tid >= 3) {
             const int k = dm.n_imu;
             const double sd = tid < 6 ? IMU_GB_STD : IMU_AB_STD;
-            Hc[(size_t) (col_mix(K, k) + tid) * C.NS + col_mix(K, k) + tid] += 1.0 / (sd * sd);
+            s_hd[k * HC_BLK + (6 + tid) * (HC_NODE + 1)] += 1.0 / (sd * sd);
             gc[col_mix(K, k) + tid] += mix[k * 9 + tid] / (sd * sd);
         }
     }
     __syncthreads();
     if (tid < 9 && dm.has_mix_prior) {
         const double sd = D.mix_prior_std[(size_t) w * 9 + tid];
-        Hc[(size_t) (col_mix(K, 0) + tid) * C.NS + col_mix(K, 0) + tid] += 1.0 / (sd * sd);
+        s_hd[(6 + tid) * (HC_NODE + 1)] += 1.0 / (sd * sd);
         gc[col_mix(K, 0) + tid] += s_mp[tid] / sd;
     }
     __syncthreads();
+    for (int e = tid; e < K * HC_BLK; e += blockDim.x) Hband[e] = s_hd[e];
     CAM_CLK(5)
 #undef CAM_CLK
     return s_total;
@@ -744,6 +795,53 @@
     }
     __syncthreads();
     return s_red[32];
+}
+
+__device__ __noinline__ void solve_fill_mix(const double *band, const int *inv, const double *H0, int CK, int K, int marg_r, double *S) {
+    const int tid = threadIdx.x, NCV = 6 * K + 7, N = 15 * K + 7;
+    for (int e = NCV * (NCV + 1) / 2 + tid; e < N * (N + 1) / 2; e += SOLVE_THREADS) S[e] = 0.0;
+    __syncthreads();
+    const unsigned s0 = (unsigned) __cvta_generic_to_shared(S);
+    for (int e = tid; e < (N - NCV) * 36; e += SOLVE_THREADS) {
+        const int i = NCV + e / 36, s = e % 36, k = (i - NCV) / 9;
+        const int j = s < 18 ? 6 * (k - 1) + s : col_mix(K, k - 1) + s - 18;
+        if (s < 18 ? (j >= 0 && j < 6 * K) : (k > 0 || s >= 27) && j <= i)
+            asm volatile("cp.async.ca.shared.global [%0], [%1], 8;" ::"r"(s0 + 8u * (i * (i + 1) / 2 + j)), "l"(hc_ptr_in(band, inv, H0, CK, K, 0, i, j)) : "memory");
+    }
+    if (marg_r > 0) {
+        const double *band_end = band + hc_band_stride(CK);
+        for (int i = NCV + (tid >> 5); i < N; i += SOLVE_THREADS / 32) {
+            if (inv[i] < 0) continue;
+            for (int j = tid & 31; j <= i; j += 32) {
+                const double *src = hc_ptr_in(band, inv, H0, CK, K, marg_r, i, j);
+                if (src && (src < band || src >= band_end))
+                    asm volatile("cp.async.ca.shared.global [%0], [%1], 8;" ::"r"(s0 + 8u * (i * (i + 1) / 2 + j)), "l"(src) : "memory");
+            }
+        }
+    }
+}
+
+__device__ __noinline__ void solve_scale_vis(double *S, const double *s_scale, const double *s_d2, const double *s_hv, const double *band,
+                                             const int *inv, const double *H0, int CK, int K, int marg_r) {
+    const int tid = threadIdx.x, NCV = 6 * K + 7;
+    for (int i = tid >> 5; i < NCV; i += SOLVE_THREADS / 32) {
+        double *row = S + i * (i + 1) / 2;
+        const double si = s_scale[i];
+        const int ki = i < 6 * K ? i / 6 : -2;
+        for (int j = tid & 31; j <= i; j += 32) {
+            const int kj = j / 6;
+            double hc = 0.0;
+            if (ki - kj <= 1 && ki >= 0)
+                hc = s_hv[(ki == kj ? ki : CK + kj) * 36 + (i - 6 * ki) * 6 + j - 6 * kj];
+            else if (marg_r > 0) {
+                const double *p = hc_ptr_in(band, inv, H0, CK, K, marg_r, i, j);
+                hc = p ? *p : 0.0;
+            }
+            double v = si * s_scale[j] * (hc + row[j]);
+            if (i == j) v += s_d2[i];
+            row[j] = v;
+        }
+    }
 }
 
 __global__ void __launch_bounds__(SOLVE_THREADS, 2) ba_solve(BaCaps C, BaDev D) {
@@ -779,8 +877,10 @@
     double *s_d2 = s_rhs + C.NS;
     double *s_diag = s_d2 + C.NS;
     double *S = s_diag + C.NS;
+    double *s_hv = S + (size_t) (C.N + 1) * (C.N + 2) / 2;
     const int b = st.lin_buf;
-    const double *Hc = lin_Hc(C, D, b, w), *gcam = lin_gc(C, D, b, w), *Hs = D.Hs + (size_t) w * C.NS * C.NS;
+    const double *gcam = lin_gc(C, D, b, w), *Hs = D.Hs + (size_t) w * C.NS * C.NS;
+    const int marg_r = dm.marg_r;
     const double *V = D.visv + (size_t) (3 * C.NCV) * w;
     if (tid == 0 && st.need_lin) st.need_lin = 0;
     double *scale_c = D.scale_c + (size_t) w * C.NS;
@@ -791,7 +891,7 @@
         if (a < NCV) g += V[NCV + a];
         s_g[a] = g;
         if (f_first) {
-            double h = Hc[(size_t) a * C.NS + a] + (a < NCV ? V[a] : 0.0);
+            double h = hc_at(C, D, b, w, K, marg_r, a, a) + (a < NCV ? V[a] : 0.0);
             scale_c[a] = 1.0 / (1.0 + sqrt(h));
         }
     }
@@ -835,16 +935,26 @@
 
     constexpr bool async_fill = true;
     if (async_fill) {
-        for (int i = tid >> 5; i < N; i += SOLVE_THREADS / 32) {
-            const double *src = (i < NCV ? Hs : Hc) + (size_t) i * C.NS;
+        for (int i = tid >> 5; i < NCV; i += SOLVE_THREADS / 32) {
+            const double *src = Hs + (size_t) i * C.NS;
             const unsigned dst = (unsigned) __cvta_generic_to_shared(S + i * (i + 1) / 2);
             for (int j = tid & 31; j <= i; j += 32)
                 asm volatile("cp.async.ca.shared.global [%0], [%1], 8;" ::"r"(dst + 8u * j), "l"(src + j) : "memory");
         }
+        solve_fill_mix(lin_Hband(C, D, b, w), lin_Hinv(C, D, b, w), D.marg_H0 + (size_t) w * C.R * C.R, C.K, K, marg_r, S);
+        {
+            const double *band = lin_Hband(C, D, b, w);
+            const unsigned dst = (unsigned) __cvta_generic_to_shared(s_hv);
+            for (int e = tid; e < (2 * K - 1) * 36; e += SOLVE_THREADS) {
+                const int blk = e / 36, q = e - 36 * blk, bk = blk < K ? blk : C.K + blk - K;
+                asm volatile("cp.async.ca.shared.global [%0], [%1], 8;" ::"r"(dst + 8u * (bk * 36 + q)), "l"(band + bk * HC_BLK + (q / 6) * HC_NODE + q % 6)
+                             : "memory");
+            }
+        }
         asm volatile("cp.async.commit_group;" ::: "memory");
     }
     for (int a = tid; a < N; a += SOLVE_THREADS) {
-        double h = Hc[(size_t) a * C.NS + a] + (a < NCV ? V[a] : 0.0);
+        double h = hc_at(C, D, b, w, K, marg_r, a, a) + (a < NCV ? V[a] : 0.0);
         double hs = s_scale[a] * s_scale[a] * h;
         s_d2[a] = lm_d2(hs, radius);
         double gw = a < NCV ? V[2 * NCV + a] : 0.0;
@@ -853,7 +963,8 @@
     if (async_fill) asm volatile("cp.async.wait_all;" ::: "memory");
     __syncthreads();
     if (async_fill) {
-        for (int i = tid >> 5; i < N; i += SOLVE_THREADS / 32) {
+        solve_scale_vis(S, s_scale, s_d2, s_hv, lin_Hband(C, D, b, w), lin_Hinv(C, D, b, w), D.marg_H0 + (size_t) w * C.R * C.R, C.K, K, marg_r);
+        for (int i = NCV + (tid >> 5); i < N; i += SOLVE_THREADS / 32) {
             double *row = S + i * (i + 1) / 2;
             const double si = s_scale[i];
             for (int j = tid & 31; j <= i; j += 32) {
@@ -871,7 +982,7 @@
             for (int q = 0; q < MAXQ; q++) {
                 const int j = (tid & 31) + 32 * q;
                 hv[q] = 0;
-                if (q < nq && j <= i) hv[q] = (i < NCV ? Hs : Hc)[(size_t) i * C.NS + j];
+                if (q < nq && j <= i) hv[q] = i < NCV ? hc_at(C, D, b, w, K, marg_r, i, j) + Hs[(size_t) i * C.NS + j] : hc_at(C, D, b, w, K, marg_r, i, j);
             }
 #pragma unroll
             for (int q = 0; q < MAXQ; q++) {
diff --git a/ic_gvins_b200/csrc/ba_dev.cuh b/ic_gvins_b200/csrc/ba_dev.cuh
--- a/ic_gvins_b200/csrc/ba_dev.cuh
+++ b/ic_gvins_b200/csrc/ba_dev.cuh
@@ -8,6 +8,9 @@
 constexpr int BA_SPLIT_W = 4;
 constexpr int BA_MARG_MAXB = 72;
 constexpr int BA_MAX_NODES = 32;
+constexpr int HC_NODE = 15;
+constexpr int HC_BLK = HC_NODE * HC_NODE;
+__host__ __device__ inline size_t hc_band_stride(int K) { return (size_t) (2 * K - 1) * HC_BLK; }
 
 struct BaCaps {
     int NW, K, L, F, G, R;
@@ -64,7 +67,8 @@
     double *AW[2];
     double *costf[2];
     double *hl[2], *gl[2];
-    double *Hc[2], *gc[2];
+    double *Hc_band[2], *gc[2];
+    int *Hc_inv[2];
     double *scale_l, *scale_c;
     double *Hs;
     double *visv;
diff --git a/ic_gvins_b200/csrc/ba_handle.cu b/ic_gvins_b200/csrc/ba_handle.cu
--- a/ic_gvins_b200/csrc/ba_handle.cu
+++ b/ic_gvins_b200/csrc/ba_handle.cu
@@ -16,6 +16,13 @@
     cudaMemsetAsync(*p, 0, sizeof(double) * n, h->stream);
     h->dev_only.push_back(*p);
     return ICG_OK;
+}
+
+static int alloc_hc_inv(icg_ba *h, int b) {
+    double *p = nullptr;
+    const int rc = dmalloc(h, &p, ((size_t) h->C.NW * h->C.NS + 1) / 2);
+    h->D.Hc_inv[b] = (int *) p;
+    return rc;
 }
 
 static int cam_threads(const icg_ba *h) { return h->D.world >= 4 ? CAM_THREADS : 160; }
@@ -60,7 +67,7 @@
     if (h->D.clk) {
         unsigned long long ck[48];
         if (cudaMemcpy(ck, h->D.clk, sizeof(ck), cudaMemcpyDeviceToHost) == cudaSuccess) {
-            static const char *cn[6] = {"factor evaluation", "prior product + cost", "zero H_c", "prior blocks", "IMU J^T J", "GNSS / prior diagonals"};
+            static const char *cn[6] = {"factor evaluation", "prior product + cost", "zero H_c diagonal blocks", "prior blocks", "IMU J^T J", "GNSS / prior diagonals"};
             fprintf(stderr, "[icg_ba profile] ba_lin_cam phases of window 0 (SM cycles per call, mean):\n");
             for (int k = 0; k < 6; k++)
                 if (ck[24 + k]) fprintf(stderr, "  %-28s %9.0f cycles\n", cn[k], (double) ck[16 + k] / (double) ck[24 + k]);
@@ -258,9 +265,10 @@
     DM(pose_0, NW * C.K * 7) DM(mix_0, NW * C.K * 9) DM(ext_0, NW * 8) DM(rho_0, NW * C.L)
     DM(AW[0], NW * C.NCA * C.LP) DM(Mp[0], NW * (size_t) C.K * (C.K - 1) * 210) DM(visv, NW * 3 * C.NCV)
     DM(gpart, NW * (size_t) C.GQ * 210) DM(costf[0], NW * C.F) DM(hl[0], NW * C.L) DM(gl[0], NW * C.L) DM(scale_l, NW * C.L) DM(scale_c, NW * C.NS)
-    DM(Hc[0], NW * C.NS * C.NS) DM(gc[0], NW * C.NS) DM(Hs, NW * C.NS * C.NS) DM(cost_part, NW * (h->nblk_vis + 1)) DM(red2, NW * 4) DM(step_c, NW * C.NS) DM(step_l, NW * C.L)
+    DM(Hc_band[0], NW * hc_band_stride(C.K)) DM(gc[0], NW * C.NS) DM(Hs, NW * C.NS * C.NS) DM(cost_part, NW * (h->nblk_vis + 1)) DM(red2, NW * 4) DM(step_c, NW * C.NS) DM(step_l, NW * C.L)
 #undef DM
     if (rc == ICG_OK) rc = dmalloc(h, &D.gnss_std_0, NW * C.G * 3);
+    if (rc == ICG_OK) rc = alloc_hc_inv(h, 0);
     if (rc == ICG_OK) {
         double *cnt = nullptr;
         rc = dmalloc(h, &cnt, (NW * C.K + 1) / 2);
@@ -274,11 +282,12 @@
     if (rc == ICG_OK) rc = dmalloc(h, &h->lm_ref, NW * C.L * 7);
     if (rc == ICG_OK) rc = dmalloc(h, &h->lm_ref_alt, NW * C.L * 7);
     if (rc != ICG_OK) return rc;
-    h->smem_cam = sizeof(double) * ((size_t) C.K * 480 + (size_t) C.G * 24 + 48 + 16 + 2 * (size_t) C.R + 8) + sizeof(int) * (size_t) C.R + 64;
+    h->smem_cam = sizeof(double) * ((size_t) C.K * 480 + (size_t) C.G * 24 + 48 + 16 + 2 * (size_t) C.R + 8 + (size_t) C.K * HC_BLK) +
+                  sizeof(int) * ((size_t) C.R + C.NS) + 64;
     size_t vec = sizeof(double) * (40 + 5 * (size_t) C.NS);
     size_t packed = sizeof(double) * ((size_t) (C.N + 1) * (C.N + 2) / 2);
     h->use_global_S = (vec + packed > 220 * 1024) ? 1 : 0;
-    h->smem_solve = vec + (h->use_global_S ? 0 : packed);
+    h->smem_solve = vec + (h->use_global_S ? 0 : packed + sizeof(double) * (2 * (size_t) C.K - 1) * 36);
     D.Sglobal = nullptr;
     memset(&D.S, 0, sizeof(D.S));
     if (h->use_global_S) {
@@ -552,8 +561,9 @@
 #define DM(field, count) \
     if (rc == ICG_OK) rc = dmalloc(h, &D.field, count);
     DM(AW[1], NW * C.NCA * C.LP) DM(Mp[1], NW * (size_t) C.K * (C.K - 1) * 210) DM(costf[1], NW * C.F) DM(hl[1], NW * C.L) DM(gl[1], NW * C.L)
-    DM(Hc[1], NW * C.NS * C.NS) DM(gc[1], NW * C.NS)
+    DM(Hc_band[1], NW * hc_band_stride(C.K)) DM(gc[1], NW * C.NS)
 #undef DM
+    if (rc == ICG_OK) rc = alloc_hc_inv(h, 1);
     return rc;
 }
 
diff --git a/ic_gvins_b200/csrc/ba_split.cuh b/ic_gvins_b200/csrc/ba_split.cuh
--- a/ic_gvins_b200/csrc/ba_split.cuh
+++ b/ic_gvins_b200/csrc/ba_split.cuh
@@ -70,7 +70,7 @@
     };
     double *rv = D.S.redv + (size_t) w * D.S.RV;
     if (A < NCV && B < NCV) {
-        D.Hs[(size_t) w * C.NS * C.NS + (size_t) B * C.NS + A] = lin_Hc(C, D, 0, w)[(size_t) B * C.NS + A] + rsum(tri_idx(A, B, NCV));
+        D.Hs[(size_t) w * C.NS * C.NS + (size_t) B * C.NS + A] = hc_at(C, D, 0, w, K, D.dims[w].marg_r, B, A) + rsum(tri_idx(A, B, NCV));
         if (A == B) rv[A] = rsum(TRI + A);
     } else if (A < NCV) {
         rv[NCV + A] = rsum(TRI + NCV + A);
@@ -85,11 +85,12 @@
 }
 
 
-__device__ __forceinline__ void split_col(const BaCaps &C, const BaDev &D, int w, int NCV, int a, const LmState &s0, double &g, double &sc, double &d2,
-                                          double &rh) {
+__device__ __forceinline__ void split_col(const BaCaps &C, const BaDev &D, int w, const WinDims &dm, int a, const LmState &s0, double &g, double &sc,
+                                          double &d2, double &rh) {
+    const int NCV = 6 * dm.K + 7;
     const double *rv = D.S.redv + (size_t) w * D.S.RV;
     const double gv = lin_gc(C, D, 0, w)[a] + (a < NCV ? rv[NCV + a] : 0.0);
-    const double h = lin_Hc(C, D, 0, w)[(size_t) a * C.NS + a] + (a < NCV ? rv[a] : 0.0);
+    const double h = hc_at(C, D, 0, w, dm.K, dm.marg_r, a, a) + (a < NCV ? rv[a] : 0.0);
     const double sv = s0.first ? 1.0 / (1.0 + sqrt(h)) : D.scale_c[(size_t) w * C.NS + a];
     g = gv, sc = sv, d2 = lm_d2(sv * sv * h, s0.radius), rh = -sv * (gv - (a < NCV ? rv[2 * NCV + a] : 0.0));
 }
@@ -131,8 +132,8 @@
     double *s_d2 = s_rhs + C.NS;
     double *s_blk = s_d2 + C.NS;
     double *S = D.Sglobal + (size_t) (w / D.world) * split_S_stride(C);
-    const double *Hc = lin_Hc(C, D, 0, w), *Hs = D.Hs + (size_t) w * C.NS * C.NS;
-    for (int a = tid; a < N; a += SOLVE_THREADS) split_col(C, D, w, NCV, a, s0, s_g[a], s_scale[a], s_d2[a], s_rhs[a]);
+    const double *Hs = D.Hs + (size_t) w * C.NS * C.NS;
+    for (int a = tid; a < N; a += SOLVE_THREADS) split_col(C, D, w, dm, a, s0, s_g[a], s_scale[a], s_d2[a], s_rhs[a]);
     __syncthreads();
     double x_cost = s0.x_cost, gmax = s0.gmax;
     if (s0.fresh_lin) {
@@ -159,11 +160,10 @@
         return;
     }
     for (int i = cwarp; i < N; i += ncwarps) {
-        const double *src = (i < NCV ? Hs : Hc) + (size_t) i * C.NS;
         double *dst = S + (size_t) i * (i + 1) / 2;
         const double si = s_scale[i];
         for (int j = lane; j <= i; j += 32) {
-            double v = si * s_scale[j] * src[j];
+            double v = si * s_scale[j] * (i < NCV ? Hs[(size_t) i * C.NS + j] : hc_at(C, D, 0, w, K, dm.marg_r, i, j));
             if (i == j) v += s_d2[i];
             dst[j] = v;
         }
@@ -443,10 +443,10 @@
     double *s_dg = s_xT + 16;
     double *s_P = s_dg + (size_t) ntc * 64;
     double *s_tiles = s_P + (size_t) 2 * ntc * 64;
-    const double *Hc = lin_Hc(C, D, 0, w), *Hs = D.Hs + (size_t) w * C.NS * C.NS;
+    const double *Hs = D.Hs + (size_t) w * C.NS * C.NS;
     for (int a = tid; a < VL; a += SOLVE_THREADS) {
         double g = 0, sc = 0, d2 = 0, rh = 0;
-        if (a < N) split_col(C, D, w, NCV, a, s0, g, sc, d2, rh);
+        if (a < N) split_col(C, D, w, dm, a, s0, g, sc, d2, rh);
         s_g[a] = g, s_scale[a] = sc, s_d2[a] = d2, s_rhs[a] = rh;
         s_y[a] = 0, s_contrib[a] = 0, s_x[a] = 0, s_dinv[a] = 0;
     }
@@ -500,11 +500,11 @@
 #pragma unroll
         for (int h = 0; h < 2; h++) {
             const int Th = T + h * CL, i = 8 * Th + warp, ncol = 8 * Th;
-            const double *src = (i < NCV ? Hs : Hc) + (size_t) (i < N ? i : 0) * C.NS;
 #pragma unroll
             for (int u = 0; u < NCH; u++) {
                 const int j = 32 * u + lane;
-                v[h][u] = (Th < nt && j < ncol && i < N) ? __ldcg(src + j) : 0.0;
+                const double *src = Th < nt && j < ncol && i < N ? (i < NCV ? Hs + (size_t) i * C.NS + j : hc_ptr(C, D, 0, w, K, dm.marg_r, i, j)) : nullptr;
+                v[h][u] = src ? __ldcg(src) : 0.0;
             }
         }
 #pragma unroll
@@ -526,7 +526,8 @@
 #pragma unroll
         for (int u = 0; u < NDG; u++) {
             const int e = tid + u * SOLVE_THREADS, T = e >> 6, r = (e >> 3) & 7, c = e & 7, i = 8 * T + r, j = 8 * T + c;
-            v[u] = (e < nt * 64 && c <= r && i < N) ? __ldcg((i < NCV ? Hs : Hc) + (size_t) i * C.NS + j) : 0.0;
+            const double *src = e < nt * 64 && c <= r && i < N ? (i < NCV ? Hs + (size_t) i * C.NS + j : hc_ptr(C, D, 0, w, K, dm.marg_r, i, j)) : nullptr;
+            v[u] = src ? __ldcg(src) : 0.0;
         }
 #pragma unroll
         for (int u = 0; u < NDG; u++) {
```

Result: no change. 24570, median of 6 (-0.0%).
